# luosiallen/Diff-Foley

Hardware: AMD Instinct MI355X
Metric: UNet denoise steps/sec (8s audio latent, 25-step DDIM, CFG 4.5), aggregate over GPUs (higher is better)
Workload: dtype f16; 1 GPU; BASELINE.json configs[1]: single MI355X, batch=4 (UNet batch 8), 25-step DDIM, fp16 (16-bit MFMA operands at the bf16 rate; the operand type that meets mel MAE < 1e-3 -- the bf16 build is timed in `modes`) UNet, 32 CAVP context frames, latent 4x16x64, guidance 4.5; batch_per_gpu=4, global_batch=4, parallelism=batch-shard x1, no step-loop collectives

## Files before the change

### diff_foley_amd/csrc/attention.hip

```cpp
#include <stdlib.h>
#include "common.h"
#include "kernels.h"

namespace {

template <int KS> struct AttnGeo {
  static constexpr int KT = 32 * KS;
  static constexpr int VROW = KT + 4;
};

template <int D, int NW, int KS = 1>
__global__ __launch_bounds__(NW * 64) void attention_kernel(const bf16_t* __restrict__ Q, int ldq,
                                                            const bf16_t* __restrict__ K, int ldk,
                                                            const bf16_t* __restrict__ Vt, int ldvt, int heads, int Tq,
                                                            int Tk, float scale_log2e, bf16_t* __restrict__ O, int ldo) {
  constexpr int DKC = (D + 15) / 16;
  constexpr int DKP = DKC * 16;
  constexpr int DT = (D + 31) / 32;
  constexpr int KROW = DKP + 8;
  constexpr int KT = AttnGeo<KS>::KT, VROW = AttnGeo<KS>::VROW;
  constexpr bool ONES = (D % 32) != 0;
  constexpr int ONE_T = D / 32, ONE_R = ((D % 32) / 8) * 4 + (D % 4);
  static_assert(!ONES || (D % 8) == 0, "row D sits in half-wave 0");
  __shared__ __attribute__((aligned(16))) bf16_t sK[2 * KT * KROW];
  __shared__ __attribute__((aligned(16))) bf16_t sV[2 * DT * 32 * VROW];

  const int tid = threadIdx.x, lane = tid & 63, wid = tid >> 6;
  const int l31 = lane & 31, lh = lane >> 5;
  const int n = blockIdx.z, h = blockIdx.y;
  const int q0 = (blockIdx.x * NW + wid) * 32;
  const int q = q0 + l31;
  const bool qv = q < Tq;

  bf16x8 qf[DKC];
  {
    const bf16_t* qr = Q + ((long)n * Tq + (qv ? q : 0)) * ldq + h * D;
#pragma unroll
    for (int c = 0; c < DKC; ++c) {
      const int d0 = 16 * c + 8 * lh;
      const bool ok = qv && d0 < D;
      uint4 v = *reinterpret_cast<const uint4*>(qr + (ok ? d0 : 0));
      if (!ok) v = make_uint4(0, 0, 0, 0);
      qf[c] = *reinterpret_cast<bf16x8*>(&v);
    }
  }

  f32x16 o[DT];
#pragma unroll
  for (int t = 0; t < DT; ++t)
#pragma unroll
    for (int r = 0; r < 16; ++r) o[t][r] = 0.f;
  float m_run = -INFINITY, l_run = 0.f;

  const bf16_t* Kb = K + (long)n * Tk * ldk + h * D;
  const bf16_t* Vb = Vt + ((long)n * heads + h) * D * ldvt;
  const int ntiles = (Tk + KT - 1) / KT;

  constexpr int NT = NW * 64;
  constexpr int KCH = (KT * (DKP / 8) + NT - 1) / NT;
  constexpr int VCR = KT / 4;
  constexpr int VCH = (DT * 32 * VCR + NT - 1) / NT;
  uint4 kreg[KCH];
  uint2 vreg[VCH];
  constexpr unsigned OOB = 0x80000000u;
  const __amdgpu_buffer_rsrc_t rsK =
      __builtin_amdgcn_make_buffer_rsrc((void*)Kb, 0, (int)(((long)(Tk - 1) * ldk + D) * 2), 0x00020000);
  const __amdgpu_buffer_rsrc_t rsV =
      __builtin_amdgcn_make_buffer_rsrc((void*)Vb, 0, (int)(((long)(D - 1) * ldvt + ldvt) * 2), 0x00020000);
  unsigned k_off[KCH], v_off[VCH];
#pragma unroll
  for (int i = 0; i < KCH; ++i) {
    const int c = tid + i * NT;
    const int key = c / (DKP / 8), ch = c - key * (DKP / 8);
    const bool ok = (c < KT * (DKP / 8)) && (ch * 8 < D);
    k_off[i] = ok ? (unsigned)((key * ldk + ch * 8) * 2) : OOB;
  }
#pragma unroll
  for (int i = 0; i < VCH; ++i) {
    const int c = tid + i * NT;
    const int d = c / VCR, ch = c - d * VCR;
    const bool ok = (c < DT * 32 * VCR) && (d < D);
    v_off[i] = ok ? (unsigned)((d * ldvt + ch * 4) * 2) : OOB;
  }
  auto gfetch = [&](int k0) {
#pragma unroll
    for (int i = 0; i < KCH; ++i) {
      const u32x4 v = __builtin_amdgcn_raw_buffer_load_b128(rsK, (int)k_off[i], k0 * ldk * 2, 0);
      kreg[i] = make_uint4(v[0], v[1], v[2], v[3]);
    }
#pragma unroll
    for (int i = 0; i < VCH; ++i) {
      typedef __attribute__((ext_vector_type(2))) unsigned int u32x2;
      const u32x2 v = __builtin_amdgcn_raw_buffer_load_b64(rsV, (int)v_off[i], k0 * 2, 0);
      vreg[i] = make_uint2(v[0], v[1]);
    }
    if (k0 + KT > Tk) {
#pragma unroll
      for (int i = 0; i < VCH; ++i) {
        const int ch = (tid + i * NT) % VCR;
        const int nvalid = Tk - (k0 + ch * 4);
        uint2 v = vreg[i];
        if (nvalid < 4) {
          if (nvalid < 3) v.y = 0; else v.y &= 0xFFFFu;
          if (nvalid < 2) v.x &= 0xFFFFu;
          if (nvalid < 1) v.x = 0;
        }
        vreg[i] = v;
      }
    }
  };
  auto sstore = [&](int buf) {
    bf16_t* k_ = sK + buf * (KT * KROW);
    bf16_t* v_ = sV + buf * (DT * 32 * VROW);
#pragma unroll
    for (int i = 0; i < KCH; ++i) {
      const int c = tid + i * NT;
      const int key = c / (DKP / 8), ch = c - key * (DKP / 8);
      if (c < KT * (DKP / 8)) *reinterpret_cast<uint4*>(&k_[key * KROW + ch * 8]) = kreg[i];
    }
#pragma unroll
    for (int i = 0; i < VCH; ++i) {
      const int c = tid + i * NT;
      const int d = c / VCR, ch = c - d * VCR;
      if (c < DT * 32 * VCR && !(ONES && d == D)) *reinterpret_cast<uint2*>(&v_[d * VROW + ch * 4]) = vreg[i];
    }
  };

  gfetch(0);
  DfTouch code_touch = DfTouch();
  if constexpr (D >= 128) code_touch = df_entry_touch(0);
  sstore(0);
  if (ONES) {
#if defined(DF_OPERAND_F16)
    constexpr uint32_t ONE2 = 0x3C003C00u;
#else
    constexpr uint32_t ONE2 = 0x3F803F80u;
#endif
    for (int i = tid; i < 2 * (KT / 2); i += NT) {
      const int b = i / (KT / 2), k2 = i - b * (KT / 2);
      *reinterpret_cast<uint32_t*>(&sV[b * (DT * 32 * VROW) + D * VROW + 2 * k2]) = ONE2;
    }
  }
  __syncthreads();

  for (int kt = 0; kt < ntiles; ++kt) {
    const int k0 = kt * KT;
    const int buf = kt & 1;
    const bf16_t* cK = sK + buf * (KT * KROW);
    const bf16_t* cV = sV + buf * (DT * 32 * VROW);
    if (kt + 1 < ntiles) gfetch(k0 + KT);

    f32x16 s[KS];
#pragma unroll
    for (int u = 0; u < KS; ++u)
#pragma unroll
      for (int r = 0; r < 16; ++r) s[u][r] = 0.f;
#pragma unroll
    for (int c = 0; c < DKC; ++c)
#pragma unroll
      for (int u = 0; u < KS; ++u) {
        const bf16x8 kf = *reinterpret_cast<const bf16x8*>(&cK[(u * 32 + l31) * KROW + 16 * c + 8 * lh]);
        s[u] = DF_MFMA_32x32x16(kf, qf[c], s[u]);
      }
    if (k0 + KT > Tk) {
#pragma unroll
      for (int u = 0; u < KS; ++u)
#pragma unroll
        for (int r = 0; r < 16; ++r) {
          const int key = k0 + u * 32 + (r & 3) + 8 * (r >> 2) + 4 * lh;
          s[u][r] = (key < Tk) ? s[u][r] : -INFINITY;
        }
    }
    float mxu[KS];
#pragma unroll
    for (int u = 0; u < KS; ++u) {
      mxu[u] = -INFINITY;
#pragma unroll
      for (int r = 0; r < 16; ++r) mxu[u] = fmaxf(mxu[u], s[u][r]);
    }
    float mx = mxu[0];
#pragma unroll
    for (int u = 1; u < KS; ++u) mx = fmaxf(mx, mxu[u]);
    mx = half_max(mx) * scale_log2e;
    const float m_new = fmaxf(m_run, mx);
    float psu[KS];
    uint32_t pk[KS][8];
#pragma unroll
    for (int u = 0; u < KS; ++u) {
      psu[u] = 0.f;
#pragma unroll
      for (int r = 0; r < 16; r += 2) {
        const float p0 = __builtin_amdgcn_exp2f(__builtin_fmaf(s[u][r], scale_log2e, -m_new)),
                    p1 = __builtin_amdgcn_exp2f(__builtin_fmaf(s[u][r + 1], scale_log2e, -m_new));
        if (!ONES) psu[u] += p0 + p1;
        pk[u][r >> 1] = pack_bf2_bounded(p0, p1);
      }
    }
    float ps = psu[0];
#pragma unroll
    for (int u = 1; u < KS; ++u) ps += psu[u];
    if (__any(m_new != m_run)) {
      const float alpha = __builtin_amdgcn_exp2f(m_run - m_new);
      if (!ONES) l_run *= alpha;
#pragma unroll
      for (int t = 0; t < DT; ++t)
#pragma unroll
        for (int r = 0; r < 16; ++r) o[t][r] *= alpha;
      m_run = m_new;
    }
    if (!ONES) l_run += ps;
#pragma unroll
    for (int u = 0; u < KS; ++u)
#pragma unroll
      for (int c = 0; c < 2; ++c) {
        uint4 pv = make_uint4(pk[u][4 * c], pk[u][4 * c + 1], pk[u][4 * c + 2], pk[u][4 * c + 3]);
        const bf16x8 pf = *reinterpret_cast<bf16x8*>(&pv);
#pragma unroll
        for (int t = 0; t < DT; ++t) {
          const bf16_t* vr = &cV[(t * 32 + l31) * VROW + u * 32 + 16 * c + 4 * lh];
          const uint2 v0 = *reinterpret_cast<const uint2*>(vr);
          const uint2 v1 = *reinterpret_cast<const uint2*>(vr + 8);
          uint4 vv = make_uint4(v0.x, v0.y, v1.x, v1.y);
          const bf16x8 vf = *reinterpret_cast<bf16x8*>(&vv);
          o[t] = DF_MFMA_32x32x16(vf, pf, o[t]);
        }
      }
    if (kt + 1 < ntiles) sstore(buf ^ 1);
    __syncthreads();
  }

  float l_tot;
  if (ONES) {
    const float mine = o[ONE_T][ONE_R];
    const float other = __shfl_xor(mine, 32);
    l_tot = lh == 0 ? mine : other;
  } else {
    l_tot = l_run + __shfl_xor(l_run, 32);
  }
  const float inv = 1.0f / l_tot;
  if (qv) {
    bf16_t* orow = O + ((long)n * Tq + q) * ldo + h * D;
#pragma unroll
    for (int t = 0; t < DT; ++t)
#pragma unroll
      for (int g = 0; g < 4; ++g) {
        const int d0 = 32 * t + 8 * g + 4 * lh;
        if (d0 < D) {
          uint2 w;
          w.x = pack_bf2(o[t][4 * g] * inv, o[t][4 * g + 1] * inv);
          w.y = pack_bf2(o[t][4 * g + 2] * inv, o[t][4 * g + 3] * inv);
          *reinterpret_cast<uint2*>(orow + d0) = w;
        }
      }
  }
  if constexpr (D >= 128) df_entry_touch_end(code_touch);
}

template <int D>
hipError_t launch_d(const uint16_t* Q, int ldq, const uint16_t* K, int ldk, const uint16_t* Vt, int ldvt,
                    uint16_t* O, int ldo, int N, int heads, int Tq, int Tk, float scale, hipStream_t s) {
  const float sl2 = scale * 1.4426950408889634f;
  const int form = attention_form(D, Tq, Tk), nw = form >> 4;
  if (nw < 1) return hipErrorInvalidValue;
  const dim3 grid((Tq + 32 * nw - 1) / (32 * nw), heads, N), block(64 * nw);
#define DF_ATTN(...) hipLaunchKernelGGL((attention_kernel<D, __VA_ARGS__>), grid, block, 0, s, Q, ldq, K, ldk, Vt, ldvt, heads, Tq, Tk, sl2, O, ldo)
  switch (form) {
    case 4 * 16 + 2:
      if constexpr (D <= 80) { DF_ATTN(4, 2); break; }
      return hipErrorInvalidValue;
    case 4 * 16 + 1: DF_ATTN(4); break;
    case 2 * 16 + 1: DF_ATTN(2); break;
    case 1 * 16 + 1: DF_ATTN(1); break;
    default: return hipErrorInvalidValue;
  }
#undef DF_ATTN
  return hipGetLastError();
}

}

bool attention_supported(int D) {
  switch (D) {
    case 16: case 24: case 32: case 40: case 48: case 56: case 64: case 72: case 80: case 96: case 112: case 128: case 160: case 192:
      return true;
    default: return false;
  }
}

int attention_form(int D, int Tq, int Tk) {
  if (!attention_supported(D)) return 0;
  if (Tq >= 128) return 4 * 16 + (D <= 80 && Tk % 64 == 0 ? 2 : 1);
  return (Tq >= 64 ? 2 : 1) * 16 + 1;
}

hipError_t launch_attention(const uint16_t* Q, int ldq, const uint16_t* K, int ldk, const uint16_t* Vt, int ldvt,
                            uint16_t* O, int ldo, int N, int heads, int D, int Tq, int Tk, float scale,
                            hipStream_t s) {
  if (ldvt % 32 != 0 || ldvt < ((Tk + 31) / 32) * 32) return hipErrorInvalidValue;
  switch (D) {
    case 16:  return launch_d<16>(Q, ldq, K, ldk, Vt, ldvt, O, ldo, N, heads, Tq, Tk, scale, s);
    case 24:  return launch_d<24>(Q, ldq, K, ldk, Vt, ldvt, O, ldo, N, heads, Tq, Tk, scale, s);
    case 48:  return launch_d<48>(Q, ldq, K, ldk, Vt, ldvt, O, ldo, N, heads, Tq, Tk, scale, s);
    case 56:  return launch_d<56>(Q, ldq, K, ldk, Vt, ldvt, O, ldo, N, heads, Tq, Tk, scale, s);
    case 72:  return launch_d<72>(Q, ldq, K, ldk, Vt, ldvt, O, ldo, N, heads, Tq, Tk, scale, s);
    case 96:  return launch_d<96>(Q, ldq, K, ldk, Vt, ldvt, O, ldo, N, heads, Tq, Tk, scale, s);
    case 112: return launch_d<112>(Q, ldq, K, ldk, Vt, ldvt, O, ldo, N, heads, Tq, Tk, scale, s);
    case 192: return launch_d<192>(Q, ldq, K, ldk, Vt, ldvt, O, ldo, N, heads, Tq, Tk, scale, s);
    case 32:  return launch_d<32>(Q, ldq, K, ldk, Vt, ldvt, O, ldo, N, heads, Tq, Tk, scale, s);
    case 40:  return launch_d<40>(Q, ldq, K, ldk, Vt, ldvt, O, ldo, N, heads, Tq, Tk, scale, s);
    case 64:  return launch_d<64>(Q, ldq, K, ldk, Vt, ldvt, O, ldo, N, heads, Tq, Tk, scale, s);
    case 80:  return launch_d<80>(Q, ldq, K, ldk, Vt, ldvt, O, ldo, N, heads, Tq, Tk, scale, s);
    case 128: return launch_d<128>(Q, ldq, K, ldk, Vt, ldvt, O, ldo, N, heads, Tq, Tk, scale, s);
    case 160: return launch_d<160>(Q, ldq, K, ldk, Vt, ldvt, O, ldo, N, heads, Tq, Tk, scale, s);
    default:  return hipErrorInvalidValue;
  }
}
```

### diff_foley_amd/csrc/elementwise.hip

```cpp
#include <algorithm>
#include "common.h"
#include "kernels.h"

namespace {

struct GnSlabs {
  int n;
  long stride;
  const float* bias;
  const float* rowbias;
  int ld_rowbias;
  const float* own;
  int c_own;
  const float* res;
  int ldr;
  float* hout;
};
template <int PER>
__global__ void groupnorm_reg_kernel(const float* __restrict__ x, int ld, int HW, int cpg, int R, int sl_n, int nsamp,
                                     const float* __restrict__ sl_own, int sl_c_own, long sl_stride,
                                     bf16_t* __restrict__ out, int ldo, int silu, int C,
                                     const float* __restrict__ gamma, const float* __restrict__ beta, float eps,
                                     bf16_t* __restrict__ raw, GnSlabs sl) {
  df_fp16_hw_clamp();
// ... 851 lines not shown
}
}

static size_t conv3x3_fewout_lds(int C, int Cout) { return (size_t)(FO_TH + 2) * (FO_TW + 2) * (C * 2 + 16) + (size_t)Cout * 9 * C * 2; }

bool conv3x3_fewout_ok(int H, int W, int C, int Cout) {
  return Cout >= 1 && Cout <= 4 && C % 16 == 0 && C >= 16 && conv3x3_fewout_lds(C, Cout) <= 160 * 1024 && W % 4 == 0 && H > 0;
}

hipError_t launch_conv3x3_fewout(const uint16_t* X, const uint16_t* Wt, const float* bias, float* out, int NB, int H, int W, int C,
                                 int Cout, hipStream_t s) {
  if (!conv3x3_fewout_ok(H, W, C, Cout)) return hipErrorInvalidValue;
  const long blocks = (long)NB * ((H + FO_TH - 1) / FO_TH) * ((W + FO_TW - 1) / FO_TW);
  const size_t lds = conv3x3_fewout_lds(C, Cout);
  static size_t attr = 0;
  if (lds > attr) {
    hipError_t e = hipFuncSetAttribute(reinterpret_cast<const void*>(&conv3x3_fewout_kernel), hipFuncAttributeMaxDynamicSharedMemorySize, (int)lds);
    if (e != hipSuccess) return e;
    attr = lds;
  }
  hipLaunchKernelGGL(conv3x3_fewout_kernel, dim3((unsigned)blocks), dim3(256), lds, s, X, Wt, bias, out, NB, H, W, C, Cout);
  return hipGetLastError();
}

hipError_t launch_pack_conv_weight(const float* w, uint16_t* out, int O, int I, int KH, int KW, int Ipad,
                                   hipStream_t s) {
  const long n = (long)O * KH * KW * Ipad;
  hipLaunchKernelGGL(pack_conv_weight_kernel, dim3(grid_for(n)), dim3(256), 0, s, w, out, O, I, KH, KW, Ipad);
  return hipGetLastError();
}

namespace {
__global__ __launch_bounds__(256) void pack_ffproj_kernel(const float* __restrict__ Wp ,
                                                          const float* __restrict__ W2 , bf16_t* __restrict__ out ,
                                                          int C, int F) {
  __shared__ float sa[32][33], sb[32][33];
  const int tx = threadIdx.x & 31, ty = threadIdx.x >> 5;
  const int i0 = blockIdx.y * 32, j0 = blockIdx.x * 32;
  if (j0 >= F) {
#pragma unroll
    for (int r = 0; r < 4; ++r) out[(long)(i0 + ty + 8 * r) * (F + C) + j0 + tx] = f2bf(Wp[(long)(i0 + ty + 8 * r) * C + (j0 - F) + tx]);
    return;
  }
  float acc[4] = {0.f, 0.f, 0.f, 0.f};
  for (int k0 = 0; k0 < C; k0 += 32) {
#pragma unroll
    for (int r = 0; r < 4; ++r) {
      sa[ty + 8 * r][tx] = Wp[(long)(i0 + ty + 8 * r) * C + k0 + tx];
      sb[ty + 8 * r][tx] = W2[(long)(k0 + ty + 8 * r) * F + j0 + tx];
    }
    __syncthreads();
#pragma unroll
    for (int kk = 0; kk < 32; ++kk) {
      const float b = sb[kk][tx];
#pragma unroll
      for (int r = 0; r < 4; ++r) acc[r] += sa[ty + 8 * r][kk] * b;
    }
    __syncthreads();
  }
#pragma unroll
  for (int r = 0; r < 4; ++r) out[(long)(i0 + ty + 8 * r) * (F + C) + j0 + tx] = f2bf(acc[r]);
}
__global__ __launch_bounds__(256) void ffproj_bias_kernel(const float* __restrict__ Wp, const float* __restrict__ b2,
                                                          const float* __restrict__ bp, float* __restrict__ out, int C) {
  const int i = blockIdx.x * 4 + (threadIdx.x >> 6), lane = threadIdx.x & 63;
  if (i >= C) return;
  float a = 0.f;
  for (int k = lane; k < C; k += 64) a += Wp[(long)i * C + k] * b2[k];
#pragma unroll
  for (int o = 32; o > 0; o >>= 1) a += __shfl_xor(a, o);
  if (lane == 0) out[i] = a + bp[i];
}
}

hipError_t launch_pack_ffproj(const float* Wp, const float* bp, const float* W2, const float* b2, uint16_t* wout, float* bout,
                              int C, int F, hipStream_t s) {
  if (C % 32 != 0 || F % 32 != 0) return hipErrorInvalidValue;
  hipLaunchKernelGGL(pack_ffproj_kernel, dim3((F + C) / 32, C / 32), dim3(256), 0, s, Wp, W2, wout, C, F);
  hipLaunchKernelGGL(ffproj_bias_kernel, dim3((C + 3) / 4), dim3(256), 0, s, Wp, b2, bp, bout, C);
  return hipGetLastError();
}

namespace {
__global__ __launch_bounds__(256) void xattn_expand_kernel(const bf16_t* __restrict__ kv, bf16_t* __restrict__ Kexp,
                                                           bf16_t* __restrict__ Vexp, int Tc, int Tcp, int C, int H, long total8) {
  const int D = C / H, c8n = C / 8;
  for (long e = (long)blockIdx.x * 256 + threadIdx.x; e < total8; e += (long)gridDim.x * 256) {
    const int j8 = (int)(e % c8n);
    const long row = e / c8n;
    const int tp = (int)(row % Tcp), h = (int)((row / Tcp) % H);
    const long n = row / ((long)Tcp * H);
    uint4 k4 = make_uint4(0, 0, 0, 0), v4 = make_uint4(0, 0, 0, 0);
    if (tp < Tc) {
      const bf16_t* src = kv + ((n * Tc + tp) * 2l * C) + j8 * 8;
      k4 = *reinterpret_cast<const uint4*>(src);
      v4 = *reinterpret_cast<const uint4*>(src + C);
      const int hj = (j8 * 8) / D;
      if (hj != h) { k4 = make_uint4(0, 0, 0, 0); v4 = k4; }
    }
    *reinterpret_cast<uint4*>(Kexp + row * C + j8 * 8) = k4;
    *reinterpret_cast<uint4*>(Vexp + row * C + j8 * 8) = v4;
  }
}
__global__ __launch_bounds__(256) void pack_lnq_t_kernel(const float* __restrict__ Wq, const float* __restrict__ gamma,
                                                         bf16_t* __restrict__ out, int C, float scale) {
  __shared__ float t[32][33];
  const int tx = threadIdx.x & 31, ty = threadIdx.x >> 5;
  const int j0 = blockIdx.x * 32, c0 = blockIdx.y * 32;
#pragma unroll
  for (int r = 0; r < 4; ++r) t[ty + 8 * r][tx] = Wq[(long)(j0 + ty + 8 * r) * C + c0 + tx];
  __syncthreads();
#pragma unroll
  for (int r = 0; r < 4; ++r) {
    const int c = c0 + ty + 8 * r;
    out[(long)c * C + j0 + tx] = f2bf(scale * gamma[c] * t[tx][ty + 8 * r]);
  }
}
__global__ __launch_bounds__(256) void xattn_rowstats_kernel(const bf16_t* __restrict__ G, const bf16_t* __restrict__ Kexp,
                                                             const float* __restrict__ bq, float scale, int C, long rows,
                                                             float* __restrict__ cs, float* __restrict__ bb) {
  const long row = (long)blockIdx.x * 4 + (threadIdx.x >> 6);
  const int lane = threadIdx.x & 63;
  if (row >= rows) return;
  float a = 0.f, b = 0.f;
  for (int c = lane; c < C; c += 64) {
    a += bf2f(G[row * C + c]);
    b += bf2f(Kexp[row * C + c]) * bq[c];
  }
#pragma unroll
  for (int o = 32; o > 0; o >>= 1) { a += __shfl_xor(a, o); b += __shfl_xor(b, o); }
  if (lane == 0) { cs[row] = a; bb[row] = scale * b; }
}
}

hipError_t launch_xattn_expand(const uint16_t* kv, uint16_t* Kexp, uint16_t* Vexp, int NB, int Tc, int Tcp, int C, int H,
                               hipStream_t s) {
  if (C % H != 0 || (C / H) % 8 != 0 || C % 8 != 0) return hipErrorInvalidValue;
  const long total8 = (long)NB * H * Tcp * (C / 8);
  const int blocks = (int)std::min<long>((total8 + 255) / 256, 8192);
  hipLaunchKernelGGL(xattn_expand_kernel, dim3(blocks), dim3(256), 0, s, kv, Kexp, Vexp, Tc, Tcp, C, H, total8);
  return hipGetLastError();
}
hipError_t launch_pack_lnq_t(const float* Wq, const float* gamma, uint16_t* out, int C, float scale, hipStream_t s) {
  if (C % 32 != 0) return hipErrorInvalidValue;
  hipLaunchKernelGGL(pack_lnq_t_kernel, dim3(C / 32, C / 32), dim3(256), 0, s, Wq, gamma, out, C, scale);
  return hipGetLastError();
}
hipError_t launch_xattn_rowstats(const uint16_t* G, const uint16_t* Kexp, const float* bq, float scale, int C, long rows, float* cs,
                                 float* bb, hipStream_t s) {
  hipLaunchKernelGGL(xattn_rowstats_kernel, dim3((unsigned)((rows + 3) / 4)), dim3(256), 0, s, G, Kexp, bq, scale, C, rows, cs, bb);
  return hipGetLastError();
}

hipError_t launch_pack_conv_skip(const float* w, const float* ws, uint16_t* out, int O, int I, int I2, hipStream_t s) {
  const long n = (long)O * (9 * I + I2);
  hipLaunchKernelGGL(pack_conv_skip_kernel, dim3(grid_for(n)), dim3(256), 0, s, w, ws, out, O, I, I2);
  return hipGetLastError();
}

hipError_t launch_pack_geglu(const float* w, const float* b, uint16_t* wout, float* bout, int half_rows, int K,
                             hipStream_t s) {
  if (half_rows % 32 != 0) return hipErrorInvalidValue;
  const long n = (long)2 * half_rows * K;
  hipLaunchKernelGGL(pack_geglu_kernel, dim3(grid_for(n)), dim3(256), 0, s, w, b, wout, bout, half_rows, K);
  return hipGetLastError();
}
// ... 54 lines not shown
```

### diff_foley_amd/csrc/engine_builder.hip

```cpp
#include "engine_internal.h"

DFE_NAMESPACE {

static void choose_tile(int M, int N, int K, int batch, bool geglu, int* tile, int* splitk) {
  static const double eff[] = {1.0, 0.85, 0.85, 0.62, 0.55};
  constexpr int TILE_COUNT = sizeof(eff) / sizeof(eff[0]);
  static_assert(TILE_COUNT == TILE_32x128 + 1, "one efficiency per tile 128x128 .. 32x128");
  double best = 1e30;
  *tile = TILE_64x64;
  *splitk = 1;
  const int nk = K / 64;
  for (int c = 0; c < TILE_COUNT; ++c) {
    int bm, bn;
    gemm_tile_dims(c, &bm, &bn);
    if (bm > 64 && M <= bm / 2) continue;
    const long tiles = (long)cdiv(M, bm) * cdiv(N, bn) * batch;
    for (int sk = 1; sk <= 16; sk *= 2) {
      if (sk > 1 && (batch > 1 || nk / sk < 4)) break;
      const double work = (double)(bm / 32) * (bn / 32) * (double)cdiv(nk, sk) * 4.0 * 8.0 / eff[c] + 2500.0;
      const double rounds = (double)((tiles * sk + 255) / 256);
      double cost = rounds * work;
      if (sk > 1) cost += 9000.0 + (double)M * N * 8.0 * sk / 2000.0;
      if (cost < best) {
        best = cost;
// ... 185 lines not shown
  bf16_t* xraw = nullptr;
  bf16_t* a1 = groupnorm(x, NB, n1, eps, 1, has_skip ? &xraw : nullptr);
  float* h1 = buf<float>((size_t)M * cout);
  {
    GemmParams g = gp_conv3(a1, NB, H, Wd, cin, c->w_conv3(nm(c1 + ".weight"), cin), cout, 1, 0);
    out_f32(g, h1, cout);
    g.bias = c->f32(nm(c1 + ".bias"));
    if (emb) {
      g.rowbias = emb + emb_col; g.ld_rowbias = emb_ld; g.rows_per_sample = H * Wd; g.rowbias_mode = 1;
    }
    gemm(g, 1, "res.conv1");
  }
  pl->release(a1);
  const size_t ci = pl->ops.size() - 1;
  pl->ops[ci].defer = groupnorm_accepts_slabs(H * Wd, cout);
  bf16_t* a2 = buf<bf16_t>((size_t)M * cout);
  {
    Plan* plp = pl;
    const float* gm = c->f32(nm(n2 + ".weight"));
    const float* bt = c->f32(nm(n2 + ".bias"));
    const float* cb = c->f32(nm(c1 + ".bias"));
    const float* rb = emb ? emb + emb_col : nullptr;
    const int HW = H * Wd;
    const size_t sb = groupnorm_scratch_bytes(NB, HW, cout);
    float* scr = sb ? (float*)pl->alloc(sb) : nullptr;
    other("groupnorm", [=](hipStream_t s, const RunArgs&) {
      const Op& co = plp->ops[ci];
      if (co.defer && co.gp.splitk > 1)
        return launch_groupnorm_slabs(co.gp.partial, cout, NB, HW, cout, gm, bt, eps, 1, a2, cout, nullptr, co.gp.splitk,
                                      (long)M * cout, cb, rb, emb_ld, s);
      if (scr) return launch_groupnorm_chunked(h1, cout, NB, HW, cout, gm, bt, eps, 1, a2, cout, nullptr, scr, s);
      return launch_groupnorm(h1, cout, NB, HW, cout, gm, bt, eps, 1, a2, cout, nullptr, s);
    });
    emits(a2, M, cout, cout);
    pl->release(scr);
  }
  pl->release(h1);
  {
    GemmParams g = gp_conv3(a2, NB, H, Wd, cout, c->w_conv3(nm(c2 + ".weight"), cout), cout, 1, 0);
    out_f32(g, out.p, out.ld);
    g.bias = c->f32(nm(c2 + ".bias"));
    if (has_skip) {
      const bf16_t* w;
      const float* bsum;
      c->w_conv3_skip(nm(c2), nm(skip), &w, &bsum);
      g.W = w;
      g.bias = bsum;
      g.A2 = xraw; g.lda2 = cin; g.Cin2 = cin; g.a2_bytes = op_bytes((size_t)M * cin * 2);
      g.K = 9 * cout + cin;
      g.w_bytes = op_bytes((size_t)cout * g.K * 2);
    } else { g.res = x.p; g.ldr = x.ld; }
    attach_aux(g, M, cout);
    g.dup_rows = dup_rows;
    gemm(g, 1, "res.conv2");
  }
  if (has_skip) pl->release(xraw);
  pl->release(a2);
}

void Builder::spatial_transformer(const F32& x, const F32& out, int NB, int T, const std::string& p, int heads,
                                  const bf16_t* ctxK, const bf16_t* ctxVt, int Tc, int ldvtc, const PX* px,
                                  bool cfg_prefix) {
  const int C = x.C, M = x.rows, D = C / heads;
  if (cfg_prefix && (T % 4 != 0 || NB % 2 != 0)) fail("cfg prefix needs the fused QKV form");
  const int Mp = cfg_prefix ? M / 2 : M, NBp = cfg_prefix ? NB / 2 : NB;
  if (!attention_supported(D)) fail("unsupported attention head dim %d", D);
  const std::string tb = p + ".transformer_blocks.0";
  const float scale = 1.0f / sqrtf((float)D);
  bf16_t* a = groupnorm(F32{x.p, Mp, C, x.ld}, NBp, p + ".norm", 1e-6f, 0, nullptr);
  float* t0 = buf<float>((size_t)M * C);
  F32 t0v{t0, M, C, C};
  bf16_t* xb = buf<bf16_t>((size_t)M * C);
  const int slots = C / 64;
  float2* st = buf<float2>((size_t)M * slots);
  auto produces_t0 = [&](GemmParams& g) {
    out_f32(g, t0, C);
    g.aux = xb; g.ld_aux = C;
    g.stats = st; g.stats_slots = slots;
  };
  auto ln_fold = [&](GemmParams& g, const float* cs, const float* bb) {
    g.ln_stats = st; g.ln_slots = slots; g.ln_C = C; g.ln_eps = 1e-5f; g.ln_cs = cs;
    g.bias = bb;
  };
  {
    GemmParams g = gp_linear(a, Mp, C, c->w_linear(nm(p + ".proj_in.weight")), C);
    produces_t0(g);
    g.bias = c->f32(nm(p + ".proj_in.bias"));
    gemm(g, 1, "st.proj_in");
  }
  bf16_t* qk = buf<bf16_t>((size_t)M * 2 * C);
  const int ldvt = rup(T, 32);
  bf16_t* vt = buf<bf16_t>((size_t)NB * C * ldvt);
  const bool fuse_v = (T % 4 == 0);
  bf16_t* o_own = nullptr;
  if (!fuse_v) {
    layernorm(t0v, tb + ".norm1", a);
    {
      const bf16_t* w = c->w_stack(nm(tb + ".attn1.qk"), {nm(tb + ".attn1.to_q.weight"), nm(tb + ".attn1.to_k.weight")});
      GemmParams g = gp_linear(a, M, C, w, 2 * C);
      out_b16(g, qk, 2 * C);
      gemm(g, 1, "st.qk");
    }
    {
      GemmParams g = gp_linear(c->w_linear(nm(tb + ".attn1.to_v.weight")), C, C, a, T);
      g.w_bs = (long)T * C;
      out_b16(g, vt, ldvt);
      g.c_bs = (long)C * ldvt;
      gemm(g, NB, "st.vT");
    }
    o_own = buf<bf16_t>((size_t)M * C);
  } else {
    const bf16_t* w;
    const float *cs, *bb;
    c->w_ln_stack(nm(tb + ".attn1.qkv"), nm(tb + ".norm1"),
                  {nm(tb + ".attn1.to_q.weight"), nm(tb + ".attn1.to_k.weight"), nm(tb + ".attn1.to_v.weight")}, {}, false,
                  &w, &cs, &bb);
    GemmParams g = gp_linear(xb, Mp, C, w, 3 * C);
    out_b16(g, qk, 2 * C);
    ln_fold(g, cs, bb);
    g.vt = vt; g.vt_col0 = 2 * C; g.vt_T = T; g.ldvt = ldvt;
    gemm(g, 1, "st.qkv");
  }
  bf16_t* o = o_own ? o_own : a;
  other("attn.self", [=](hipStream_t s, const RunArgs&) {
    return launch_attention(qk, 2 * C, qk + C, 2 * C, vt, ldvt, o, C, NBp, heads, D, T, T, scale, s);
  });
  emits(o, Mp, C, C);
  {
    GemmParams g = gp_linear(o, Mp, C, c->w_linear(nm(tb + ".attn1.to_out.0.weight")), C);
    produces_t0(g);
    g.bias = c->f32(nm(tb + ".attn1.to_out.0.bias"));
    g.res = t0; g.ldr = C;
    g.dup_rows = cfg_prefix ? Mp : 0;
    gemm(g, 1, "st.attn1.out");
  }
  if (px && px->G) {
    const int HT = px->HT;
    bf16_t* pr = qk;
    if ((size_t)HT > (size_t)2 * C) fail("cross-attention: %d probability columns do not fit the q|k buffer", HT);
    {
      GemmParams g = gp_linear(xb, M, C, px->G, HT);
      g.w_bs = (long)HT * C; g.w_rows = T;
      g.w_bytes = op_bytes((size_t)HT * C * 2);
      out_b16(g, pr, HT);
      ln_fold(g, px->cs, px->bb);
      g.sm_w = 32; g.sm_valid = Tc;
      gemm(g, 1, "st.xs");
    }
    {
      GemmParams g = gp_linear(pr, M, HT, px->Vo, C);
      g.w_bs = (long)C * HT; g.w_rows = T;
      g.w_bytes = op_bytes((size_t)C * HT * 2);
      produces_t0(g);
      g.no_c_store = 1;
      g.bias = c->f32(nm(tb + ".attn2.to_out.0.bias"));
      g.res = t0; g.ldr = C;
      gemm(g, 1, "st.xo");
    }
  } else {
  bf16_t* q2 = qk;
  {
    const bf16_t* w;
    const float *cs, *bb;
    c->w_ln_stack(nm(tb + ".attn2.q"), nm(tb + ".norm2"), {nm(tb + ".attn2.to_q.weight")}, {}, false, &w, &cs, &bb);
    GemmParams g = gp_linear(xb, M, C, w, C);
    out_b16(g, q2, C);
    ln_fold(g, cs, bb);
    gemm(g, 1, "st.q2");
  }
  other("attn.cross", [=](hipStream_t s, const RunArgs&) {
    return launch_attention(q2, C, ctxK, C, ctxVt, ldvtc, o, C, NB, heads, D, T, Tc, scale, s);
  });
  emits(o, M, C, C);
  {
    GemmParams g = gp_linear(o, M, C, c->w_linear(nm(tb + ".attn2.to_out.0.weight")), C);
    produces_t0(g);
    g.bias = c->f32(nm(tb + ".attn2.to_out.0.bias"));
    g.res = t0; g.ldr = C;
    gemm(g, 1, "st.attn2.out");
  }
  }
  pl->release(qk);
  pl->release(vt);
  bf16_t* gl = buf<bf16_t>((size_t)M * 4 * C);
  {
    const bf16_t* w;
    const float *cs, *bb;
    c->w_ln_stack(nm(tb + ".ff.net.0.proj"), nm(tb + ".norm3"), {nm(tb + ".ff.net.0.proj.weight")},
                  {nm(tb + ".ff.net.0.proj.bias")}, true, &w, &cs, &bb);
    GemmParams g = gp_linear(xb, M, C, w, 8 * C);
    out_b16(g, gl, 4 * C);
    ln_fold(g, cs, bb);
    g.geglu = 1;
    if ((8 * C) % 320 == 0) {
      const bf16_t* w3;
      const float *cs3, *bb3;
      c->w_ln_w320(nm(tb + ".ff.net.0.proj"), 8 * C, C, &w3, &cs3, &bb3);
      g.W_w320 = w3; g.cs_w320 = cs3; g.bias_w320 = bb3;
    }
    gemm(g, 1, "st.ff1");
  }
  {
    const bf16_t* w;
    const float* bsum;
    c->w_ffproj(nm(tb + ".ff.net.2"), nm(p + ".proj_out"), &w, &bsum);
    GemmParams g = gp_linear(gl, M, 4 * C, w, C);
    g.K = 5 * C;
// ... 112 lines not shown
```

### diff_foley_amd/csrc/engine_internal.h

```cpp
#pragma once
#include <hip/hip_runtime.h>

#include <algorithm>
#include <array>
#include <cmath>
#include <cstdarg>
#include <cstdio>
#include <cstdlib>
#include <cstring>
#include <functional>
#include <map>
#include <mutex>
#include <memory>
#include <stdexcept>
#include <string>
#include <vector>

#include "../../include/df_engine.h"
#include "gemm.h"
#include "kernels.h"

typedef uint16_t bf16_t;

#define DFE_NAMESPACE namespace dfe __attribute__((visibility("hidden")))
// ... 150 lines not shown
  uint64_t tick = 0;
  dfe::Plan* last_unet = nullptr;
  bool last_unet_hoisted = false;
  int ctx_N = 0, ctx_T = 0;
  float* ctx_copy = nullptr;
  size_t ctx_copy_bytes = 0;
  bool autotune = false;
  bool reloaded = false;
  bool prof_on = false;
  std::vector<hipEvent_t> prof_ev;
  std::vector<int> prof_fam;
  std::vector<const void*> prof_op;
  size_t prof_used = 0;
  hipStream_t pack_stream = nullptr;
  bool chk_on = false;
  std::vector<std::string> rq_prefix;
  unsigned long long* chk_dev = nullptr;
  size_t chk_used = 0, chk_cap = 0;
  std::vector<std::string> chk_label;
  bool sat_on = false;
  unsigned long long* sat_dev = nullptr;
  size_t sat_used = 0, sat_cap = 0;
  std::vector<std::string> sat_label;

  ~df_ctx() {
    plans.clear();
    for (auto& kv : raw) (void)hipFree(kv.second.d);
    for (void* p : packed_blocks) (void)hipFree(p);
    for (hipEvent_t e : prof_ev) (void)hipEventDestroy(e);
    if (chk_dev) (void)hipFree(chk_dev);
    if (sat_dev) (void)hipFree(sat_dev);
    if (ctx_copy) (void)hipFree(ctx_copy);
  }

  const dfe::RawT& rt(const std::string& name) const {
    auto it = raw.find(name);
    if (it == raw.end()) dfe::fail("missing tensor '%s'", name.c_str());
    return it->second;
  }
  bool has(const std::string& name) const { return raw.count(name) != 0; }
  const float* f32(const std::string& name) const {
    const dfe::RawT& t = rt(name);
    if (!t.d) dfe::fail("tensor '%s' was imported shape-only (df_import_packed): its fp32 data is not on this rank", name.c_str());
    return t.d;
  }

  std::map<const void*, size_t> block_bytes;
  void* pmalloc(size_t bytes) {
    void* p = nullptr;
    HIPCHK(hipMalloc(&p, (bytes + 255) & ~(size_t)255));
    packed_blocks.push_back(p);
    block_bytes[p] = bytes;
    return p;
  }
  template <size_t N, class Make>
  std::array<void*, N> pack_once(const std::array<std::string, N>& keys, Make&& make) {
    if (!packed.count(keys[0])) {
      const std::array<void*, N> made = make();
      for (size_t i = 0; i < N; ++i) packed[keys[i]] = made[i];
    }
    std::array<void*, N> blk;
    for (size_t i = 0; i < N; ++i) blk[i] = packed[keys[i]];
    return blk;
  }
  template <class Make>
  void* pack_once(const std::string& key, Make&& make) {
    return pack_once<1>({key}, [&]() -> std::array<void*, 1> { return {make()}; })[0];
  }
  const bf16_t* w_linear(const std::string& name);
  const bf16_t* w_stack(const std::string& key, const std::vector<std::string>& names);
  const float* b_stack(const std::string& key, const std::vector<std::string>& names);
  const bf16_t* w_conv3(const std::string& name, int ipad);
  const bf16_t* w_conv3_ups4(const std::string& name, int ipad);
  void w_conv3_skip(const std::string& conv, const std::string& skip, const bf16_t** w, const float** b);
  void w_ffproj(const std::string& ff2, const std::string& po, const bf16_t** w, const float** b);
  const bf16_t* w_lnq_t(const std::string& wq, const std::string& norm, float scale);
  const bf16_t* w_stack_t(const std::string& key, const std::vector<std::string>& names);
  const bf16_t* w_conv3_bwd(const std::string& name);
  void w_conv3d_bn(const std::string& p, int kp, const bf16_t** w, const float** b);
  void w_ln_stack(const std::string& key, const std::string& norm, const std::vector<std::string>& names,
                  const std::vector<std::string>& biases, bool geglu, const bf16_t** w, const float** cs, const float** bb);
  void w_ln_w320(const std::string& key, int rows, int K, const bf16_t** w, const float** cs, const float** bb);
  void w_geglu(const std::string& prefix, const bf16_t** w, const float** b);
};

DFE_NAMESPACE {

struct BlockDesc {
  enum Kind { CONV_IN, RES, ST, DOWN, UP } kind;
  std::string prefix;
  int cin, cout;
  int ds = 1;
};
struct UNetTopo {
  std::vector<std::vector<BlockDesc>> input, output;
  std::vector<BlockDesc> middle;
  std::vector<int> in_ch;
  std::vector<int> in_ds;
  std::vector<int> out_ds;
  int final_ch = 0;
};

UNetTopo make_topo(const df_unet_config& u, bool encoder_only);
std::vector<std::string> topo_resblocks(const UNetTopo& t);
std::vector<BlockDesc> topo_sts(const UNetTopo& t);

struct Builder {
  df_ctx* c;
  Plan* pl;
  std::string pre;
  int which = 0;

  std::string nm(const std::string& s) const { return pre + s; }

  struct PX {
    const bf16_t* G = nullptr;
    const float* cs = nullptr;
    const float* bb = nullptr;
    const bf16_t* Vo = nullptr;
    int HT = 0;
  };

  bool want_aux = false;
  bf16_t* last_aux = nullptr;
  void attach_aux(GemmParams& g, int rows, int C);

  template <class T>
  T* buf(size_t n) {
    return (T*)pl->alloc(n * sizeof(T));
  }

  struct Pend { long op = -1; const float* p = nullptr; int ld = 0, C = 0, rows = 0; };
  Pend pend;

  void forget_pend();
  void other(const char* tag, std::function<hipError_t(hipStream_t, const RunArgs&)> fn);
  void emits(const bf16_t* p, long rows, int cols, int ld);
  Op& gemm(GemmParams gp, int batch, const char* tag);

  static unsigned op_bytes(size_t b);
  static GemmParams gp_linear(const bf16_t* A, int M, int K, const bf16_t* W, int N);
  static GemmParams gp_conv3(const bf16_t* A, int NB, int H, int Wd, int Cin, const bf16_t* W, int Cout, int stride,
                             int ups);
  static GemmParams gp_conv3_ups4(const bf16_t* A, int NB, int H, int Wd, int Cin, const bf16_t* W4, int Cout);
  static void out_f32(GemmParams& g, float* C, int ldc) { g.C = C; g.ldc = ldc; g.out_bf16 = 0; }
  static void out_b16(GemmParams& g, bf16_t* C, int ldc) { g.C = C; g.ldc = ldc; g.out_bf16 = 1; }

  bf16_t* groupnorm(const F32& x, int NB, const std::string& p, float eps, int silu, bf16_t** raw);
  void layernorm(const F32& x, const std::string& p, bf16_t* o);
  bf16_t* cast2d(const F32& x);

  void resblock(const F32& x, const F32& out, int NB, int H, int Wd, const std::string& n1, const std::string& c1,
                const std::string& n2, const std::string& c2, const std::string& skip, float eps,
                const float* emb, int emb_ld, int emb_col, int dup_rows = 0);

  void spatial_transformer(const F32& x, const F32& out, int NB, int T, const std::string& p, int heads,
                           const bf16_t* ctxK, const bf16_t* ctxVt, int Tc, int ldvtc, const PX* px = nullptr,
                           bool cfg_prefix = false);

  static bool px_ok(int C, int heads, int Tc, int tokens);
  PX context_px(const bf16_t* ctx, int NB, int Tc, int Dc, const std::string& st_prefix, int C, int heads);
  void context_kv(const bf16_t* ctx, int NB, int Tc, int Dc, const std::string& st_prefix, int C, bf16_t** K,
                  bf16_t** Vt, int ldvt);

  typedef std::map<std::string, std::pair<bf16_t*, bf16_t*>> KV;
  bf16_t* context_cast(int N, int Tc, int Dc);
// ... 40 lines not shown
```

### diff_foley_amd/csrc/engine_pack.hip

```cpp
#include "engine_internal.h"

using namespace dfe;

const bf16_t* df_ctx::w_linear(const std::string& name) {
  return (const bf16_t*)pack_once(name, [&] {
    const RawT& t = rt(name);
    (void)f32(name);
    bf16_t* o = (bf16_t*)pmalloc(t.n * 2);
    HIPCHK(launch_cast_bf16(t.d, o, (long)t.n, pack_stream));
    return o;
  });
}
const bf16_t* df_ctx::w_stack(const std::string& key, const std::vector<std::string>& names) {
  return (const bf16_t*)pack_once(key, [&] {
    size_t tot = 0;
    for (auto& n : names) tot += rt(n).n;
    bf16_t* o = (bf16_t*)pmalloc(tot * 2);
    size_t off = 0;
    for (auto& n : names) {
      const RawT& t = rt(n);
      HIPCHK(launch_cast_bf16(t.d, o + off, (long)t.n, pack_stream));
      off += t.n;
    }
    return o;
// ... 89 lines not shown
    return o;
  });
}
const bf16_t* df_ctx::w_conv3_bwd(const std::string& name) {
  return (const bf16_t*)pack_once(name + "#c3bwd", [&] {
    const RawT& t = rt(name);
    const int O = (int)t.shape[0], I = (int)t.shape[1], Opad = (O + 63) / 64 * 64;
    bf16_t* o = (bf16_t*)pmalloc((size_t)I * 9 * Opad * 2);
    HIPCHK(launch_pack_conv_bwd(t.d, o, O, I, Opad, pack_stream));
    return o;
  });
}
void df_ctx::w_conv3d_bn(const std::string& p, int kp, const bf16_t** w, const float** b) {
  const std::string kw = "c3d:" + p + ":" + std::to_string(kp);
  const auto blk = pack_once<2>({kw, kw + ":b"}, [&]() -> std::array<void*, 2> {
    const RawT& t = rt(p + ".conv.weight");
    if (t.shape.size() != 5) fail("%s.conv.weight: expected a 5-D Conv3d weight", p.c_str());
    const int O = (int)t.shape[0], I = (int)t.shape[1], KT = (int)t.shape[2], KH = (int)t.shape[3], KW = (int)t.shape[4];
    bf16_t* wo = (bf16_t*)pmalloc((size_t)O * kp * 2);
    float* bo = (float*)pmalloc((size_t)O * 4);
    HIPCHK(launch_pack_conv3d_bn(t.d, f32(p + ".bn.weight"), f32(p + ".bn.bias"), f32(p + ".bn.running_mean"),
                                 f32(p + ".bn.running_var"), 1e-5f, wo, bo, O, I, KT, KH, KW, kp, pack_stream));
    return {wo, bo};
  });
  *w = (const bf16_t*)blk[0];
  *b = (const float*)blk[1];
}

void df_ctx::w_ln_stack(const std::string& key, const std::string& norm, const std::vector<std::string>& names,
                        const std::vector<std::string>& biases, bool geglu, const bf16_t** w, const float** cs, const float** bb) {
  const auto blk = pack_once<3>({key + "#lnw", key + "#lncs", key + "#lnbb"}, [&]() -> std::array<void*, 3> {
    int rows = 0;
    const int K = (int)rt(names[0]).shape[1];
    for (auto& n : names) rows += (int)rt(n).shape[0];
    bf16_t* wo = (bf16_t*)pmalloc((size_t)rows * K * 2);
    float* co = (float*)pmalloc((size_t)rows * 4);
    float* bo = (float*)pmalloc((size_t)rows * 4);
    const float* g = f32(norm + ".weight");
    const float* be = f32(norm + ".bias");
    int off = 0;
    for (size_t i = 0; i < names.size(); ++i) {
      const RawT& t = rt(names[i]);
      if ((int)t.shape[1] != K) fail("w_ln_stack %s: input dims differ", key.c_str());
      const float* bias = (i < biases.size() && !biases[i].empty()) ? f32(biases[i]) : nullptr;
      const int r = (int)t.shape[0];
      HIPCHK(launch_pack_ln_linear(t.d, bias, g, be, wo, co, bo, r, K, off, geglu ? r / 2 : 0, pack_stream));
      off += r;
    }
    return {wo, co, bo};
  });
  *w = (const bf16_t*)blk[0];
  *cs = (const float*)blk[1];
  *bb = (const float*)blk[2];
}

void df_ctx::w_ln_w320(const std::string& key, int rows, int K, const bf16_t** w, const float** cs, const float** bb) {
  const std::string kw = key + "#lnw", kc = key + "#lncs", kb = key + "#lnbb";
  const auto blk = pack_once<3>({key + "#lnw320", key + "#lncs320", key + "#lnbb320"}, [&]() -> std::array<void*, 3> {
    if (!packed.count(kw) || !packed.count(kc) || !packed.count(kb)) fail("w_ln_w320 %s: the (32 | 32) packing does not exist", key.c_str());
    bf16_t* wo = (bf16_t*)pmalloc((size_t)rows * K * 2);
    float* co = (float*)pmalloc((size_t)rows * 4);
    float* bo = (float*)pmalloc((size_t)rows * 4);
    HIPCHK(launch_pack_w320((const bf16_t*)packed[kw], (const float*)packed[kc], (const float*)packed[kb], wo, co, bo, rows, K, pack_stream));
    return {wo, co, bo};
  });
  *w = (const bf16_t*)blk[0];
  *cs = (const float*)blk[1];
  *bb = (const float*)blk[2];
}

void df_ctx::w_geglu(const std::string& prefix, const bf16_t** w, const float** b) {
  const auto blk = pack_once<2>({prefix + ".weight#geglu", prefix + ".bias#geglu"}, [&]() -> std::array<void*, 2> {
    const RawT& tw = rt(prefix + ".weight");
    const RawT& tb = rt(prefix + ".bias");
    const int rows = (int)tw.shape[0], K = (int)tw.shape[1];
    bf16_t* wo = (bf16_t*)pmalloc((size_t)rows * K * 2);
    float* bo = (float*)pmalloc((size_t)rows * 4);
    HIPCHK(launch_pack_geglu(tw.d, tb.d, wo, bo, rows / 2, K, pack_stream));
    return {wo, bo};
  });
  *w = (const bf16_t*)blk[0];
  *b = (const float*)blk[1];
}
```

### diff_foley_amd/csrc/engine_run.hip

```cpp
#include "engine_internal.h"

DFE_NAMESPACE {

void finish_plan(df_ctx* c, Plan* pl) {
  if (pl->partial_bytes) {
    HIPCHK(hipMalloc((void**)&pl->partial, pl->partial_bytes));
    for (auto& o : pl->ops)
      if (o.is_gemm && o.gp.splitk > 1) o.gp.partial = pl->partial;
  }
  HIPCHK(hipStreamSynchronize(c->pack_stream));
}

namespace {

int op_family(const Op& o) {
  if (o.is_gemm) return 0;
  if (!strncmp(o.tag, "attn", 4)) return 1;
  if (!strcmp(o.tag, "groupnorm")) return 2;
  if (!strcmp(o.tag, "layernorm")) return 3;
  return 4;
}

struct ChkBuf { const uint32_t* p; unsigned long long words; };
__global__ __launch_bounds__(256) void checksum_kernel(const ChkBuf* list, unsigned long long* slot) {
  const ChkBuf b = list[blockIdx.y];
  unsigned long long acc = 0;
  for (unsigned long long i = (unsigned long long)blockIdx.x * 256 + threadIdx.x; i < b.words; i += (unsigned long long)gridDim.x * 256)
    acc += (unsigned long long)b.p[i] * (unsigned long long)((i & 1023u) + 1u);
#pragma unroll
  for (int o = 32; o > 0; o >>= 1) acc += __shfl_xor(acc, o);
  if ((threadIdx.x & 63) == 0) atomicAdd(slot, acc);
}

void checksum_after_op(df_ctx* c, Plan* pl, size_t op_index, hipStream_t s) {
  if (!pl->chk_list) {
    std::vector<ChkBuf> v;
    for (auto& b : pl->owned) v.push_back({(const uint32_t*)b.p, (unsigned long long)(b.bytes / 4)});
    if (pl->partial) v.push_back({(const uint32_t*)pl->partial, (unsigned long long)(pl->partial_bytes / 4)});
    pl->chk_n = (int)v.size();
    if (!v.empty()) {
      HIPCHK(hipMalloc(&pl->chk_list, v.size() * sizeof(ChkBuf)));
      HIPCHK(hipMemcpy(pl->chk_list, v.data(), v.size() * sizeof(ChkBuf), hipMemcpyHostToDevice));
    }
  }
  if (c->chk_used >= c->chk_cap || pl->chk_n == 0) return;
  hipLaunchKernelGGL(checksum_kernel, dim3(64, pl->chk_n), dim3(256), 0, s, (const ChkBuf*)pl->chk_list, c->chk_dev + c->chk_used);
  char lab[160];
  snprintf(lab, sizeof lab, "%s#%zu:%s", pl->name.c_str(), op_index, pl->ops[op_index].tag);
  if (pl->ops[op_index].is_gemm) {
    const Op& o = pl->ops[op_index];
    const size_t n = strlen(lab);
    snprintf(lab + n, sizeof lab - n, " %dx%dx%d taps%d tile%d sk%d", o.gp.M, o.gp.N, o.gp.K, o.gp.taps, o.tile, o.gp.splitk);
  }
  c->chk_label.push_back(lab);
  ++c->chk_used;
}

std::vector<OutBuf> operand_outputs(const Op& o) {
  std::vector<OutBuf> outs = o.outs;
  if (o.is_gemm) {
    const GemmParams& g = o.gp;
    const long rows = (long)g.M * (g.taps == 4 ? 4 : 1) + g.dup_rows;
    const int cols = g.geglu ? g.N / 2 : (g.vt ? g.vt_col0 : g.N);
    if (g.out_bf16 && g.C && !o.c_ext && !g.store_nchw)
      for (int z = 0; z < (g.splitk > 1 ? 1 : o.batch); ++z) outs.push_back({(const uint16_t*)g.C + (long)z * g.c_bs, rows, cols, g.ldc});
    if (g.aux) outs.push_back({g.aux, rows, g.N, g.ld_aux});
    if (g.vt) outs.push_back({g.vt, (long)(g.M / g.vt_T) * (g.N - g.vt_col0), g.vt_T, g.ldvt});
  }
  return outs;
}

__global__ __launch_bounds__(256) void sat_count_kernel(const uint16_t* p, long rows, int cols, int ld, unsigned long long* slot) {
  const long total = rows * (long)cols;
  unsigned long long acc = 0;
  for (long e = (long)blockIdx.x * 256 + threadIdx.x; e < total; e += (long)gridDim.x * 256) {
    const long r = e / cols;
    const uint16_t v = p[r * ld + (e - r * cols)];
#if defined(DF_OPERAND_F16)
    acc += (v & 0x7FFFu) == 0x7BFFu;
#else
    acc += (v & 0x7F80u) == 0x7F80u;
#endif
  }
#pragma unroll
  for (int o = 32; o > 0; o >>= 1) acc += __shfl_xor(acc, o);
  if ((threadIdx.x & 63) == 0 && acc) atomicAdd(slot, acc);
}

void saturations_after_op(df_ctx* c, Plan* pl, size_t op_index, hipStream_t s) {
  if (c->sat_used >= c->sat_cap) return;
  const Op& o = pl->ops[op_index];
  const std::vector<OutBuf> outs = operand_outputs(o);
  for (auto& b : outs) {
    const long total = b.rows * (long)b.cols;
    if (total <= 0) continue;
    const int blocks = (int)std::min<long>((total + 255) / 256, 1024);
    hipLaunchKernelGGL(sat_count_kernel, dim3(blocks), dim3(256), 0, s, b.p, b.rows, b.cols, b.ld, c->sat_dev + c->sat_used);
  }
  char lab[160];
  snprintf(lab, sizeof lab, "%s#%zu:%s", pl->name.c_str(), op_index, o.tag);
  c->sat_label.push_back(lab);
  ++c->sat_used;
}

__global__ __launch_bounds__(256) void requant_bf16_kernel(uint16_t* p, long rows, int cols, int ld) {
#if defined(DF_OPERAND_F16)
  const long total = rows * (long)cols;
  for (long e = (long)blockIdx.x * 256 + threadIdx.x; e < total; e += (long)gridDim.x * 256) {
    const long r = e / cols;
    uint16_t* q = p + r * ld + (e - r * cols);
    const uint16_t v = *q;
    if ((v & 0x7C00u) == 0x7C00u) continue;
    const uint16_t lsb = (v >> 3) & 1u;
    *q = (uint16_t)((v + 3u + lsb) & 0xFFF8u);
  }
#endif
}

void requant_after_op(df_ctx* c, Plan* pl, size_t op_index, hipStream_t s) {
  const Op& o = pl->ops[op_index];
  bool hit = false;
  for (auto& pre : c->rq_prefix)
    if (pre == "*" || !strncmp(o.tag, pre.c_str(), pre.size())) hit = true;
  if (!hit) return;
  const std::vector<OutBuf> outs = operand_outputs(o);
  for (auto& b : outs) {
    const long total = b.rows * (long)b.cols;
    if (total <= 0) continue;
    const int blocks = (int)std::min<long>((total + 255) / 256, 2048);
    hipLaunchKernelGGL(requant_bf16_kernel, dim3(blocks), dim3(256), 0, s, const_cast<uint16_t*>(b.p), b.rows, b.cols, b.ld);
  }
}

}

void run_ops(df_ctx* c, Plan* pl, size_t begin, size_t end, hipStream_t s, const RunArgs& a) {
  for (size_t i = begin; i < end; ++i) {
    Op& o = pl->ops[i];
    hipError_t e;
    (void)hipGetLastError();
    if (c->prof_on) {
      if (c->prof_used + 2 > c->prof_ev.size()) {
        hipEvent_t e0, e1;
        HIPCHK(hipEventCreate(&e0));
        HIPCHK(hipEventCreate(&e1));
        c->prof_ev.push_back(e0);
// ... 85 lines not shown
```

### diff_foley_amd/csrc/engine_test_api.hip

```cpp
#include "engine_internal.h"

using namespace dfe;

extern "C" {

static float* test_partial(size_t bytes) {
  static float* buf = nullptr;
  static size_t cap = 0;
  if (bytes > cap) {
    if (buf) {
      (void)hipDeviceSynchronize();
      (void)hipFree(buf);
    }
    HIPCHK(hipMalloc((void**)&buf, bytes));
    cap = bytes;
  }
  return buf;
}

int df_test_gemm(const uint16_t* A, const uint16_t* W, float* C, int M, int N, int K, int tile, int splitk, void* stream) {
  return guard([&] {
    GemmParams g = Builder::gp_linear(A, M, K, W, N);
    Builder::out_f32(g, C, N);
    g.dbg = getenv("DF_GEMM_DBG") ? atoi(getenv("DF_GEMM_DBG")) : 0;
    g.splitk = splitk;
    if (splitk > 1) g.partial = test_partial((size_t)splitk * M * N * 4);
    else if (g.dbg & 64) g.partial = test_partial((size_t)4096 * 32 * 8);
    HIPCHK(launch_gemm(g, tile, 1, (hipStream_t)stream));
  });
}

int df_test_gemm_epi(const uint16_t* A, const uint16_t* W, const float* bias, const float* res, void* C, int M, int N, int K,
                     int act, int out_operand, int tile, int splitk, void* stream) {
  return guard([&] {
    GemmParams g = Builder::gp_linear(A, M, K, W, N);
    if (out_operand) Builder::out_b16(g, (bf16_t*)C, N);
    else Builder::out_f32(g, (float*)C, N);
    g.bias = bias;
    if (res) { g.res = res; g.ldr = N; }
    g.silu = act == 1;
    g.relu = act == 2;
    g.splitk = splitk;
    if (splitk > 1) g.partial = test_partial((size_t)splitk * M * N * 4);
    if (!gemm_tile_valid(g, tile, 1, splitk)) fail("tile %d / split-K %d refused this problem", tile, splitk);
    HIPCHK(launch_gemm(g, tile, 1, (hipStream_t)stream));
  });
}

int df_test_gemm_dual(const uint16_t* A, const uint16_t* A2, const uint16_t* W, float* C, int M, int N, int K1, int K2, int tile,
                      int splitk, void* stream) {
  return guard([&] {
    GemmParams g = Builder::gp_linear(A, M, K1, W, N);
    g.K = K1 + K2;
    g.w_bytes = Builder::op_bytes((size_t)N * (K1 + K2) * 2);
    g.A2 = A2; g.lda2 = K2; g.Cin2 = K2; g.a2_bytes = Builder::op_bytes((size_t)M * K2 * 2);
    Builder::out_f32(g, C, N);
    g.splitk = splitk;
    if (splitk > 1) g.partial = test_partial((size_t)splitk * M * N * 4);
    if (!gemm_tile_valid(g, tile, 1, splitk)) fail("tile %d / split-K %d refused this problem", tile, splitk);
    HIPCHK(launch_gemm(g, tile, 1, (hipStream_t)stream));
  });
}

static void test_gemm_params(const df_test_gemm_desc* d, GemmParams& g) {
  if (!d) fail("df_test_gemm: null descriptor");
  if (d->size != (int64_t)sizeof(df_test_gemm_desc))
    fail("df_test_gemm: descriptor of %lld bytes, this build expects %zu (stale binding of df_test_gemm_desc?)", (long long)d->size,
         sizeof(df_test_gemm_desc));
  const bf16_t* A = (const bf16_t*)d->A;
  const bf16_t* W = (const bf16_t*)d->W;
  if (d->conv == 2) {
    if (d->ups || d->zstuff || d->stride > 1) fail("df_test_gemm: conv 2 takes neither ups / zstuff nor a stride");
    g = Builder::gp_conv3_ups4(A, d->NB, d->H, d->Wd, d->Cin, W, d->N);
  } else if (d->conv) {
    if (d->conv != 1) fail("df_test_gemm: conv %d", d->conv);
    if (d->stride != 1 && d->stride != 2) fail("df_test_gemm: conv stride %d", d->stride);
    if (d->zstuff && !d->ups) fail("df_test_gemm: zstuff without ups");
    if (d->ups && d->stride != 1) fail("df_test_gemm: ups with stride %d", d->stride);
    g = Builder::gp_conv3(A, d->NB, d->H, d->Wd, d->Cin, W, d->N, d->stride, d->ups ? 1 : 0);
    g.zstuff = d->zstuff ? 1 : 0;
  } else {
    if (d->ups || d->zstuff) fail("df_test_gemm: ups / zstuff on a linear GEMM");
    g = Builder::gp_linear(A, d->M, d->K, W, d->N);
    if (d->lda > 0) {
      g.lda = d->lda;
      g.a_bytes = Builder::op_bytes((size_t)d->M * d->lda * 2);
    }
  }
  if (d->Cin2 > 0 || d->A2) {
    if (d->Cin2 <= 0 || d->lda2 < d->Cin2) fail("df_test_gemm: A2 with Cin2 %d / lda2 %d", d->Cin2, d->lda2);
    g.A2 = (const bf16_t*)d->A2; g.lda2 = d->lda2; g.Cin2 = d->Cin2;
    g.a2_bytes = Builder::op_bytes(((size_t)(g.M - 1) * d->lda2 + d->Cin2) * 2);
    g.K += d->Cin2;
    g.w_bytes = Builder::op_bytes((size_t)g.N * g.K * 2);
  }
  g.geglu = d->geglu ? 1 : 0;
  g.vt = (bf16_t*)d->vt; g.vt_col0 = d->vt_col0; g.vt_T = d->vt_T; g.ldvt = d->ldvt;
  g.C = d->C; g.ldc = d->ldc > 0 ? d->ldc : (g.geglu ? g.N / 2 : g.N); g.out_bf16 = d->out_operand ? 1 : 0;
  g.a_bs = d->a_bs; g.c_bs = d->c_bs; g.res_bs = d->res_bs;
  if (d->conv != 2) g.w_bs = d->w_bs;
  g.alpha = d->alpha;
  g.bias = d->bias;
  g.rowbias = d->rowbias; g.ld_rowbias = d->ld_rowbias; g.rows_per_sample = d->rows_per_sample; g.rowbias_mode = d->rowbias_mode;
  g.res = d->res; g.ldr = d->ldr;
  g.relu = d->relu; g.silu = d->silu;
  g.aux = (bf16_t*)d->aux; g.ld_aux = d->ld_aux;
  g.stats = (float2*)d->stats; g.stats_slots = d->stats_slots;
  g.ln_stats = (const float2*)d->ln_stats; g.ln_slots = d->ln_slots; g.ln_C = d->ln_C; g.ln_eps = d->ln_eps; g.ln_cs = d->ln_cs;
  g.w_rows = d->w_rows; g.sm_w = d->sm_w; g.sm_valid = d->sm_valid;
  g.dup_rows = d->dup_rows; g.no_c_store = d->no_c_store; g.store_nchw = d->store_nchw; g.hw_out = d->hw_out;
  g.cfg_out = d->cfg_out; g.cfg_scale = d->cfg_scale;
  g.defer_reduce = d->defer_reduce;
  g.gm = d->gm;
  g.splitk = d->splitk > 1 ? d->splitk : 1;
  if (g.geglu && g.N % 320 == 0) { g.W_w320 = W; g.cs_w320 = g.ln_cs; g.bias_w320 = g.bias; }
}

int df_test_gemm_valid(const df_test_gemm_desc* d, int tile, int batch, int splitk) {
  std::lock_guard<std::recursive_mutex> hold(g_api_lock);
  try {
    GemmParams g;
    test_gemm_params(d, g);
    return gemm_tile_valid(g, tile, batch, splitk) ? 1 : 0;
  } catch (const std::exception& e) {
    g_err = e.what();
    return -1;
  }
}

int df_test_gemm_key(const df_test_gemm_desc* d, int batch, char* buf, int n) {
  std::lock_guard<std::recursive_mutex> hold(g_api_lock);
  try {
    GemmParams g;
    test_gemm_params(d, g);
    const std::string key = tune_key(g, batch > 1 ? batch : 1, d->defer_reduce != 0);
    if (!buf || n <= (int)key.size()) fail("df_test_gemm_key: buffer of %d bytes for a key of %zu", n, key.size());
    memcpy(buf, key.c_str(), key.size() + 1);
    return 0;
  } catch (const std::exception& e) {
    g_err = e.what();
    return -1;
  }
}

int df_test_gemm_tile_info(int tile, df_test_gemm_tile* out) {
  std::lock_guard<std::recursive_mutex> hold(g_api_lock);
  if (tile < 0 || tile >= TILE_ALL || !out || out->size != (int64_t)sizeof(df_test_gemm_tile)) {
    g_err = "df_test_gemm_tile_info: no tile " + std::to_string(tile) + ", or a df_test_gemm_tile of another size";
    return 1;
  }
  const GemmTileInfo& t = kGemmTiles[tile];
  out->name = t.name; out->family = t.family; out->modes = t.modes;
  out->bm = t.bm; out->bn = t.bn; out->dma_threads = gemm_halo_dma_threads(tile); out->ring = t.ring;
  return 0;
}

int df_test_gemm_ex(const df_test_gemm_desc* d, void* stream) {
  return guard([&] {
    GemmParams g;
    test_gemm_params(d, g);
    const int batch = d->batch > 1 ? d->batch : 1;
    if (g.K % 64 != 0) fail("df_test_gemm: K %d is not a multiple of 64", g.K);
    if (d->defer_reduce && g.splitk < 2) fail("df_test_gemm: defer_reduce needs split-K");
    const size_t slab_bytes = (size_t)g.splitk * g.M * g.N * 4 * (g.taps == 4 ? 4 : 1);
    if (g.splitk > 1) g.partial = test_partial(slab_bytes);
    if (gemm_tile_is_wgeglu(d->tile) && g.geglu) {
      if (g.N % 320 != 0 || !g.ln_cs || !g.bias) fail("tile %d: N = %d is not a multiple of 320, or no column sums / bias", d->tile, g.N);
      static void* buf = nullptr;
      static size_t cap = 0;
      const size_t wb = ((size_t)g.N * g.K * 2 + 255) & ~(size_t)255, need = wb + (size_t)g.N * 8 + 512;
      if (need > cap) {
        if (buf) {
          HIPCHK(hipDeviceSynchronize());
          HIPCHK(hipFree(buf));
          buf = nullptr; cap = 0;
        }
        HIPCHK(hipMalloc(&buf, need));
        cap = need;
      }
      uint16_t* w3 = (uint16_t*)buf;
// ... 233 lines not shown
    HIPCHK(launch_gemm(g, tile, 1, (hipStream_t)stream));
  });
}

int df_test_conv3x3_fewout(const uint16_t* A, const uint16_t* W, const float* bias, float* out_nchw, int NB, int H, int Wd, int Cin,
                           int Cout, void* stream) {
  return guard([&] { HIPCHK(launch_conv3x3_fewout(A, W, bias, out_nchw, NB, H, Wd, Cin, Cout, (hipStream_t)stream)); });
}

int df_test_conv3x3_skip(const uint16_t* A, const uint16_t* A2, const uint16_t* W, const float* bias, float* C, int NB, int H,
                         int Wd, int Cin, int Cin2, int Cout, int tile, int splitk, void* stream) {
  return guard([&] {
    GemmParams g = Builder::gp_conv3(A, NB, H, Wd, Cin, W, Cout, 1, 0);
    Builder::out_f32(g, C, Cout);
    g.bias = bias;
    g.A2 = A2; g.lda2 = Cin2; g.Cin2 = Cin2; g.a2_bytes = Builder::op_bytes((size_t)g.M * Cin2 * 2);
    g.K = 9 * Cin + Cin2;
    g.w_bytes = Builder::op_bytes((size_t)Cout * g.K * 2);
    g.splitk = splitk;
    if (splitk > 1) g.partial = test_partial((size_t)splitk * g.M * g.N * 4);
    if (!gemm_tile_valid(g, tile, 1, splitk)) fail("tile %d / split-K %d refused this problem", tile, splitk);
    HIPCHK(launch_gemm(g, tile, 1, (hipStream_t)stream));
  });
}

int df_test_conv3x3_ups4(const uint16_t* A, const float* W_oihw, const float* bias, float* C, uint16_t* w4_scratch, int NB, int H,
                         int Wd, int Cin, int Cout, int tile, int splitk, void* stream) {
  return guard([&] {
    HIPCHK(launch_pack_conv_ups4(W_oihw, w4_scratch, Cout, Cin, Cin, (hipStream_t)stream));
    GemmParams g = Builder::gp_conv3_ups4(A, NB, H, Wd, Cin, w4_scratch, Cout);
    Builder::out_f32(g, C, Cout);
    g.bias = bias;
    g.splitk = splitk;
    if (splitk > 1) g.partial = test_partial((size_t)splitk * 4 * g.M * g.N * 4);
    if (!gemm_tile_valid(g, tile, 1, splitk)) fail("tile %d / split-K %d refused this problem", tile, splitk);
    HIPCHK(launch_gemm(g, tile, 1, (hipStream_t)stream));
  });
}

int df_test_groupnorm_form(int N, int HW, int C, int nslab) { return groupnorm_form(N, HW, C, nslab); }
int df_test_attention_form(int D, int Tq, int Tk) { return attention_form(D, Tq, Tk); }

int df_test_groupnorm_ex(float* x, int ld, int N, int HW, int C, const float* gamma, const float* beta, float eps, int silu,
                         uint16_t* out, int ldo, uint16_t* raw_out, int nslab, int64_t slab_stride, const float* bias,
                         const float* rowbias, int ld_rowbias, const float* own_slabs, int c_own, const float* res, int ldr,
                         void* stream) {
  return guard([&] {
    hipStream_t s = (hipStream_t)stream;
    const int form = groupnorm_form(N, HW, C, nslab);
    if (form == GN_FORM_REFUSED) fail("groupnorm: %d x %d with %d slabs is refused", HW, C, nslab);
    if (own_slabs) {
      HIPCHK(launch_groupnorm_own_slabs(x, ld, N, HW, C, gamma, beta, eps, silu, out, ldo, raw_out, own_slabs, nslab, (long)slab_stride,
                                        c_own, bias, res, ldr, s));
    } else if (form == GN_FORM_CHUNKED) {
      float* scr = test_partial(groupnorm_scratch_bytes(N, HW, C));
      HIPCHK(launch_groupnorm_chunked(x, ld, N, HW, C, gamma, beta, eps, silu, out, ldo, raw_out, scr, s));
    } else {
      HIPCHK(launch_groupnorm_slabs(x, ld, N, HW, C, gamma, beta, eps, silu, out, ldo, raw_out, nslab, (long)slab_stride, bias, rowbias,
                                    ld_rowbias, s));
    }
  });
}
int df_test_groupnorm(const float* x, int ld, int N, int HW, int C, const float* gamma, const float* beta, float eps,
                      int silu, uint16_t* out, void* stream) {
  return df_test_groupnorm_ex(const_cast<float*>(x), ld, N, HW, C, gamma, beta, eps, silu, out, C, nullptr, 0, 0, nullptr, nullptr, 0,
                              nullptr, 0, nullptr, 0, stream);
}
int df_test_groupnorm_own_slabs(float* x, int ld, int N, int HW, int C, const float* gamma, const float* beta, float eps, int silu,
                                uint16_t* out, const float* slabs, int nslab, int c_own, const float* bias, const float* res,
                                int ldr, void* stream) {
  return df_test_groupnorm_ex(x, ld, N, HW, C, gamma, beta, eps, silu, out, C, nullptr, nslab, (int64_t)N * HW * c_own, bias, nullptr, 0,
                              slabs, c_own, res, ldr, stream);
}
int df_test_layernorm_ex(const float* x, int ld, int rows, int C, const float* gamma, const float* beta, uint16_t* out, void* stream) {
  return guard([&] { HIPCHK(launch_layernorm(x, ld, rows, C, gamma, beta, 1e-5f, out, (hipStream_t)stream)); });
}
int df_test_layernorm(const float* x, int rows, int C, const float* gamma, const float* beta, uint16_t* out, void* stream) {
  return df_test_layernorm_ex(x, C, rows, C, gamma, beta, out, stream);
}
int df_test_attention(const uint16_t* Q, int ldq, const uint16_t* K, int ldk, const uint16_t* Vt, int ldvt, uint16_t* O,
                      int ldo, int N, int heads, int D, int Tq, int Tk, float scale, void* stream) {
  return guard([&] { HIPCHK(launch_attention(Q, ldq, K, ldk, Vt, ldvt, O, ldo, N, heads, D, Tq, Tk, scale, (hipStream_t)stream)); });
}

int df_test_groupnorm_bwd(const float* x, int ld, int N, int HW, int C, const float* gamma, const float* beta, float eps, int silu,
                          const float* dy, int lddy, const float* addend, int ldadd, float* dx, int lddx, uint16_t* dx_b16,
                          void* stream) {
  return guard([&] {
    HIPCHK(launch_groupnorm_bwd(x, ld, N, HW, C, gamma, beta, eps, silu, dy, lddy, addend, ldadd, dx, lddx, dx_b16,
                                (hipStream_t)stream));
  });
}
int df_test_layernorm_bwd(const float* x, int rows, int C, const float* gamma, float eps, const float* dy, const float* addend,
                          float* dx, uint16_t* dx_b16, void* stream) {
  return guard([&] { HIPCHK(launch_layernorm_bwd(x, rows, C, gamma, eps, dy, addend, dx, dx_b16, (hipStream_t)stream)); });
}
int df_test_geglu_fwd(const uint16_t* u, uint16_t* y, int64_t rows, int H, void* stream) {
  return guard([&] { HIPCHK(launch_geglu_fwd(u, y, (long)rows, H, (hipStream_t)stream)); });
}
int df_test_geglu_bwd(const uint16_t* u, const float* dy, uint16_t* du, int64_t rows, int H, void* stream) {
  return guard([&] { HIPCHK(launch_geglu_bwd(u, dy, du, (long)rows, H, (hipStream_t)stream)); });
}
int df_test_attention_bwd(const uint16_t* Q, int ldq, const uint16_t* K, int ldk, const uint16_t* Vt, int ldvt, const float* dO,
                          int lddo, uint16_t* dQ, int lddq, uint16_t* dK, int lddk, uint16_t* dV, int lddv, int N, int heads, int D,
                          int Tq, int Tk, float scale, int form, void* stream) {
  return guard([&] {
    size_t nws = attention_bwd_ws_floats(N, heads, D, Tq, Tk, lddk, lddv, dK != nullptr);
    if (form == 2 && dK) nws = (size_t)N * heads * Tq * 3;
    float* ws = nws ? test_partial(nws * 4) : nullptr;
    HIPCHK(launch_attention_bwd(Q, ldq, K, ldk, Vt, ldvt, dO, lddo, dQ, lddq, dK, lddk, dV, lddv, N, heads, D, Tq, Tk, scale, ws,
                                form, (hipStream_t)stream));
  });
}
int df_test_cls_head_bwd(const float* prob, const float* w, float* dh, uint16_t* dh_b16, int N, int HW, int C, int Cp, void* stream) {
  return guard([&] { HIPCHK(launch_cls_head_bwd(prob, w, dh, dh_b16, N, HW, C, Cp, (hipStream_t)stream)); });
}
int df_test_pack_linear_t(const float* w, uint16_t* out, int O, int I, int ldo, int off, void* stream) {
  return guard([&] { HIPCHK(launch_pack_linear_t(w, out, O, I, ldo, off, (hipStream_t)stream)); });
}
int df_test_pack_conv_bwd(const float* w, uint16_t* out, int O, int I, int Opad, void* stream) {
  return guard([&] { HIPCHK(launch_pack_conv_bwd(w, out, O, I, Opad, (hipStream_t)stream)); });
}
int df_test_conv3x3_bwd_data(const uint16_t* dY, const float* W_oihw, uint16_t* w_scratch, float* dX, uint16_t* dX_op, int NB, int H,
                             int Wd, int I, int O, int stride, int tile, int splitk, void* stream) {
  return guard([&] {
    if (stride != 1 && stride != 2) fail("conv3x3 backward-data: stride %d", stride);
    if (stride == 2 && ((H | Wd) & 1)) fail("conv3x3 backward-data: stride 2 needs an even map, got %dx%d", H, Wd);
    const int Opad = (O + 63) / 64 * 64;
    HIPCHK(launch_pack_conv_bwd(W_oihw, w_scratch, O, I, Opad, (hipStream_t)stream));
    GemmParams g = stride == 1 ? Builder::gp_conv3(dY, NB, H, Wd, Opad, w_scratch, I, 1, 0)
                               : Builder::gp_conv3(dY, NB, H / 2, Wd / 2, Opad, w_scratch, I, 1, 1);
    if (stride == 2) g.zstuff = 1;
    Builder::out_f32(g, dX, I);
    if (dX_op) {
      g.aux = dX_op;
      g.ld_aux = I;
    }
    g.splitk = splitk;
    if (splitk > 1) g.partial = test_partial((size_t)splitk * g.M * g.N * 4);
    if (!gemm_tile_valid(g, tile, 1, splitk)) fail("tile %d / split-K %d refused this problem", tile, splitk);
    HIPCHK(launch_gemm(g, tile, 1, (hipStream_t)stream));
  });
}


#define DF_TEST_LAUNCH(call) return guard([&] { HIPCHK(call); })
int df_test_softmax_rows(const float* s, uint16_t* p, int rows, int T, int ldp, void* stream) {
  DF_TEST_LAUNCH(launch_softmax_rows(s, p, rows, T, ldp, (hipStream_t)stream));
}
int df_test_timestep_embedding(const float* t, float* out, int N, int dim, void* stream) {
  DF_TEST_LAUNCH(launch_timestep_embedding(t, out, N, dim, (hipStream_t)stream));
}
int df_test_timestep_embedding_b16(const float* t, int t_B, uint16_t* out, int N, int dim, void* stream) {
  DF_TEST_LAUNCH(launch_timestep_embedding_b16(t, t_B, out, N, dim, (hipStream_t)stream));
}
int df_test_pack_latent(const float* x, uint16_t* out, int B, int C, int HW, int cpad, int rep, float in_scale, const float* wpq,
                        const float* bpq, void* stream) {
  DF_TEST_LAUNCH(launch_pack_latent(x, out, B, C, HW, cpad, rep, in_scale, wpq, bpq, (hipStream_t)stream));
}
int df_test_pack_latent_bcast(const float* x, uint16_t* out, int B, int C, int HW, int cpad, int rep, const float* src, float* dst,
                              int rows, int n, void* stream) {
  DF_TEST_LAUNCH(launch_pack_latent_bcast(x, out, B, C, HW, cpad, rep, src, dst, rows, n, (hipStream_t)stream));
}
int df_test_bcast_rows(const float* src, float* dst, int rows, int n, void* stream) {
  DF_TEST_LAUNCH(launch_bcast_rows(src, dst, rows, n, (hipStream_t)stream));
}
// ... 51 lines not shown
```

### diff_foley_amd/csrc/engine_tune.hip

```cpp
#include "engine_internal.h"

DFE_NAMESPACE {

namespace {
struct TuneCand { int tile, sk; float iso_ms; double situ_ms; };

}

std::string tune_key(const GemmParams& g, int batch, bool defer) {
  char key[160];
  const int epi = (g.silu ? 128 : 0) | (g.ln_stats ? 1 : 0) | (g.stats ? 2 : 0) | (g.vt ? 4 : 0) | (g.aux ? 8 : 0) | (g.res ? 16 : 0) | (g.Cin2 ? 32 : 0) |
                  (defer ? 64 : 0) | (g.dup_rows ? 256 : 0);
  snprintf(key, sizeof key, "%d_%d_%d_%d_%d_%d_%d_%d_e%d", g.M, g.N, g.K, g.taps, g.stride, g.ups, batch, g.geglu, epi);
  return key;
}
static std::string tune_key(const Op& o) { return tune_key(o.gp, o.batch, o.defer); }

std::map<std::string, TuneChoice>& tune_cache() {
  static std::map<std::string, TuneChoice> m;
  static bool loaded = false;
  if (!loaded) {
    loaded = true;
    if (const char* path = getenv("DF_TUNE_CACHE")) {
      if (FILE* f = fopen(path, "r")) {
        char key[160];
        TuneChoice ch;
        while (fscanf(f, "%159s %d %d %d", key, &ch.tile, &ch.sk, &ch.gm) == 4) m[key] = ch;
        fclose(f);
      }
    }
  }
  return m;
}
static void tune_cache_save() {
  const char* path = getenv("DF_TUNE_CACHE");
  if (!path) return;
  FILE* f = fopen(path, "w");
  if (!f) return;
  for (auto& kv : tune_cache()) fprintf(f, "%s %d %d %d\n", kv.first.c_str(), kv.second.tile, kv.second.sk, kv.second.gm);
  fclose(f);
}

bool g_tune_imported = false;

static const TuneChoice* nearest_tune_choice(const std::string& key) {
  const size_t us = key.find('_');
  if (us == std::string::npos) return nullptr;
  const std::string suffix = key.substr(us);
  const double m = (double)atol(key.substr(0, us).c_str());
  if (m <= 0) return nullptr;
  const TuneChoice* best = nullptr;
  double bestd = 2.0001;
  for (auto& kv : tune_cache()) {
    const size_t u2 = kv.first.find('_');
    if (u2 == std::string::npos || kv.first.compare(u2, std::string::npos, suffix) != 0) continue;
    const double m2 = (double)atol(kv.first.substr(0, u2).c_str());
    if (m2 <= 0) continue;
    const double d = fabs(log2(m2 / m));
    if (d < bestd) {
      bestd = d;
      best = &kv.second;
    }
  }
  return best;
}

void apply_tune_cache(Plan* pl) {
  auto& tc = tune_cache();
  for (auto& o : pl->ops) {
    if (!o.is_gemm || o.c_ext) continue;
    const std::string key = tune_key(o);
    auto it = tc.find(key);
    const TuneChoice* chp = it != tc.end() ? &it->second : nearest_tune_choice(key);
    if (!chp) continue;
    const TuneChoice& ch = *chp;
    const size_t need = (size_t)ch.sk * o.gp.M * o.gp.N * 4 * (o.gp.taps == 4 ? 4 : 1);
    if (!gemm_tile_valid(o.gp, ch.tile, o.batch, ch.sk) || (ch.sk > 1 && need > pl->partial_bytes)) continue;
    o.tile = ch.tile;
    o.gp.splitk = ch.sk;
    o.gp.gm = ch.gm;
    o.gp.partial = pl->partial;
  }
}

void autotune_plan(df_ctx* c, Plan* pl, hipStream_t s) {
  {
    auto& tc = tune_cache();
    bool all = !tc.empty();
    for (auto& o : pl->ops)
      if (o.is_gemm && !o.c_ext && !tc.count(tune_key(o))) all = false;
    if (all) {
      apply_tune_cache(pl);
      tune_cache_save();
      return;
    }
// ... 161 lines not shown
```

### diff_foley_amd/csrc/gemm.h

```cpp
#pragma once
#include <hip/hip_runtime.h>
#include <stdint.h>
#include "common.h"

struct GemmParams {
  const uint16_t* A; long a_bs; int lda;
  const uint16_t* W; long w_bs;
  unsigned a_bytes, w_bytes;
  int M, N, K;
  const uint16_t* A2; int lda2; unsigned a2_bytes; int Cin2;
  int taps;
  int Cin;
  int H, Wd;
  int OH, OW;
  int stride;
  int ups;
  int zstuff;
  int th, tw;
  int halo_ring_bytes;
  void* C; long c_bs; int ldc; int out_bf16;
  float alpha;
  const float* bias;
  const float* rowbias; int ld_rowbias; int rows_per_sample; int rowbias_mode;
  const float* res; long res_bs; int ldr;
  int relu;
  int silu;
  uint16_t* aux; int ld_aux;
  int geglu;
  const float2* ln_stats; int ln_slots; int ln_C; float ln_eps;
  const float* ln_cs;
  const uint16_t* W_w320; const float* cs_w320; const float* bias_w320;
  int w_rows;
  int sm_w, sm_valid;
  float2* stats; int stats_slots;
  uint16_t* vt; int vt_col0; int vt_T; int ldvt;
  int dup_rows;
  int no_c_store;
  int store_nchw; int hw_out;
  int gm;
  int dbg;
  int splitk; float* partial;
  int defer_reduce;
  float* cfg_out; float cfg_scale;
};

#if defined(__HIP_DEVICE_COMPILE__)
__device__ __forceinline__ DfTouch gemm_kernarg_touch() { return df_entry_touch((int)sizeof(GemmParams)); }
__device__ __forceinline__ void gemm_kernarg_touch_end(const DfTouch& v) { df_entry_touch_end(v); }
#endif

enum GemmTileFamily { DF_FAM_GEN = 0, DF_FAM_HALO = 1, DF_FAM_PS = 2, DF_FAM_PGEGLU = 3, DF_FAM_WGEGLU = 4, DF_FAM_RETIRED = 5 };
enum GemmTile {
#define DF_TILE(ID, NAME, ...) NAME,
#include "gemm_tiles.def"
#undef DF_TILE
  TILE_ALL
};
struct GemmTileInfo {
  const char* name;
  int family, part;
  int modes;
  int bm, bn, wgm, wgn, ring, ps, lns;
};
inline constexpr GemmTileInfo kGemmTiles[TILE_ALL] = {
#define DF_TILE(ID, NAME, DISP, FAM, PART, M0, M1, M2, M3, BM, BN, WGM, WGN, RING, PS, LNS) \
  {DISP, DF_FAM_##FAM, PART, (M0) | (M1) << 1 | (M2) << 2 | (M3) << 3, BM, BN, WGM, WGN, RING, PS, LNS},
#include "gemm_tiles.def"
#undef DF_TILE
};
#define DF_TILE(ID, NAME, ...) static_assert(NAME == ID, "gemm_tiles.def: a tile id is its row's position (the ids are a file format)");
#include "gemm_tiles.def"
#undef DF_TILE

static inline int gemm_tile_family(int cfg) { return (cfg >= 0 && cfg < TILE_ALL) ? kGemmTiles[cfg].family : -1; }
static inline bool gemm_tile_is_halo(int cfg) { return gemm_tile_family(cfg) == DF_FAM_HALO; }
static inline bool gemm_tile_is_ps(int cfg) { return gemm_tile_family(cfg) == DF_FAM_PS; }
static inline bool gemm_tile_is_pgeglu(int cfg) { return gemm_tile_family(cfg) == DF_FAM_PGEGLU; }
static inline bool gemm_tile_is_wgeglu(int cfg) { return gemm_tile_family(cfg) == DF_FAM_WGEGLU; }
static inline bool gemm_tile_has_mode(int cfg, int mode) { return cfg >= 0 && cfg < TILE_ALL && ((kGemmTiles[cfg].modes >> mode) & 1); }
static inline int gemm_mode(const GemmParams& p) { return (p.taps == 4) ? 3 : (p.taps != 9) ? 0 : ((p.stride == 1 && !p.ups) ? 1 : 2); }
static inline int gemm_ln_max_slots() { return 20; }

static inline int gemm_halo_dma_threads(int cfg) {
  const GemmTileInfo& t = kGemmTiles[cfg];
  return 64 * t.wgm * t.wgn * (t.ps ? t.ps : 1);
}
static inline int gemm_halo_ring(int cfg) { return kGemmTiles[cfg].ring; }
static inline void gemm_tile_dims(int cfg, int* bm, int* bn) {
  *bm = kGemmTiles[cfg].bm;
  *bn = kGemmTiles[cfg].bn;
}

bool gemm_tile_valid(const GemmParams& p, int tile, int batch, int splitk);

hipError_t launch_gemm(const GemmParams& p, int tile_cfg, int batch, hipStream_t stream);
hipError_t launch_pack_w320(const uint16_t* w, const float* cs, const float* bb, uint16_t* wo, float* cso, float* bbo, int N, int K, hipStream_t s);
```

### diff_foley_amd/csrc/gemm.hip

```cpp
#include <algorithm>
#include <stdlib.h>

#include "gemm_impl.h"


hipError_t launch_gemm_m0a(int tile_cfg, int epi, const GemmParams& p, int zdim, hipStream_t stream);
hipError_t launch_gemm_m0b(int tile_cfg, int epi, const GemmParams& p, int zdim, hipStream_t stream);
hipError_t launch_gemm_m1(int tile_cfg, int epi, const GemmParams& p, int zdim, hipStream_t stream);
hipError_t launch_gemm_m2(int tile_cfg, int epi, const GemmParams& p, int zdim, hipStream_t stream);
hipError_t launch_gemm_halo(int tile_cfg, int epi, const GemmParams& p, int zdim, hipStream_t stream);
hipError_t launch_gemm_m3(int tile_cfg, int epi, const GemmParams& p, int zdim, hipStream_t stream);
hipError_t launch_gemm_ps(int mode, int tile_cfg, int epi, const GemmParams& p, int zdim, hipStream_t stream);
hipError_t launch_gemm_ps_small(int mode, int tile_cfg, int epi, const GemmParams& p, int zdim, hipStream_t stream);
hipError_t launch_gemm_pgeglu(int tile_cfg, const GemmParams& p, hipStream_t stream);
bool pgeglu_valid(const GemmParams& p, int tile, int batch, int splitk);
hipError_t launch_gemm_wgeglu(int tile_cfg, const GemmParams& p, hipStream_t stream);
bool wgeglu_valid(const GemmParams& p, int tile, int batch, int splitk);

namespace {

__global__ __launch_bounds__(256) void splitk_reduce_kernel(GemmParams p) {
  const int nout = p.geglu ? (p.N >> 1) : p.N;
  const long total = (long)p.M * nout;
  for (long e = (long)blockIdx.x * blockDim.x + threadIdx.x; e < total; e += (long)gridDim.x * blockDim.x) {
// ... 35 lines not shown
__global__ __launch_bounds__(256) void splitk_reduce_vec_kernel(GemmParams p) {
#if defined(__HIP_DEVICE_COMPILE__)
  const DfTouch ka = gemm_kernarg_touch();
#endif
  const int n4 = p.N >> 2;
  const long total = (long)p.M * n4;
  const long slab = (long)p.M * p.N;
  const bool has_bias = p.bias != nullptr, has_rb = p.rowbias != nullptr, has_res = p.res != nullptr;
  for (long e = (long)blockIdx.x * blockDim.x + threadIdx.x; e < total; e += (long)gridDim.x * blockDim.x) {
    const int row = (int)(e / n4), col = (int)(e - (long)row * n4) * 4;
    const float* src = p.partial + (long)row * p.N + col;
    float4 t[SK];
#pragma unroll
    for (int s = 0; s < SK; ++s) t[s] = *reinterpret_cast<const float4*>(src + s * slab);
    float4 v = t[0];
#pragma unroll
    for (int s = 1; s < SK; ++s) {
      v.x += t[s].x; v.y += t[s].y; v.z += t[s].z; v.w += t[s].w;
    }
    v.x *= p.alpha; v.y *= p.alpha; v.z *= p.alpha; v.w *= p.alpha;
    if (p.ln_stats) {
      const float2* sp = p.ln_stats + (long)row * p.ln_slots;
      float s1 = 0.f, s2 = 0.f;
      for (int i = 0; i < p.ln_slots; ++i) {
        const float2 t2 = sp[i];
        s1 += t2.x;
        s2 += t2.y;
      }
      const float inv = 1.0f / (float)p.ln_C;
      const float mean = s1 * inv, rstd = rsqrtf(fmaxf(s2 * inv - mean * mean, 0.f) + p.ln_eps);
      const float4 cs = *reinterpret_cast<const float4*>(&p.ln_cs[col]);
      v.x = rstd * (v.x - mean * cs.x); v.y = rstd * (v.y - mean * cs.y);
      v.z = rstd * (v.z - mean * cs.z); v.w = rstd * (v.w - mean * cs.w);
    }
    if (has_bias) {
      const float4 b = *reinterpret_cast<const float4*>(&p.bias[col]);
      v.x += b.x; v.y += b.y; v.z += b.z; v.w += b.w;
    }
    if (has_rb) {
      const int ri = (p.rowbias_mode == 1) ? (row / p.rows_per_sample) : (row % p.rows_per_sample);
      const float4 b = *reinterpret_cast<const float4*>(&p.rowbias[(long)ri * p.ld_rowbias + col]);
      v.x += b.x; v.y += b.y; v.z += b.z; v.w += b.w;
    }
    if (has_res) {
      const float4 b = *reinterpret_cast<const float4*>(&p.res[(long)row * p.ldr + col]);
      v.x += b.x; v.y += b.y; v.z += b.z; v.w += b.w;
    }
    if (p.silu && !p.ln_stats && !p.stats) {
      v.x = silu_f(v.x); v.y = silu_f(v.y); v.z = silu_f(v.z); v.w = silu_f(v.w);
    }
    if (p.relu) {
      v.x = fmaxf(v.x, 0.f); v.y = fmaxf(v.y, 0.f); v.z = fmaxf(v.z, 0.f); v.w = fmaxf(v.w, 0.f);
    }
    if (p.stats) {
      const float s1 = row16_sum((v.x + v.y) + (v.z + v.w));
      const float s2 = row16_sum((v.x * v.x + v.y * v.y) + (v.z * v.z + v.w * v.w));
      if ((threadIdx.x & 15) == 0) {
        p.stats[(long)row * p.stats_slots + (col >> 6)] = make_float2(s1, s2);
        if (p.dup_rows) p.stats[(long)(row + p.dup_rows) * p.stats_slots + (col >> 6)] = make_float2(s1, s2);
      }
    }
    for (int rep = 0; rep < (p.dup_rows ? 2 : 1); ++rep) {
      const long orow = row + (rep ? p.dup_rows : 0);
      const long idx = orow * p.ldc + col;
      if (p.no_c_store) {
      } else if (p.out_bf16)
        st_wt(reinterpret_cast<uint2*>(reinterpret_cast<bf16_t*>(p.C) + idx), make_uint2(pack_bf2(v.x, v.y), pack_bf2(v.z, v.w)));
      else
        st_wt(reinterpret_cast<float4*>(reinterpret_cast<float*>(p.C) + idx), v);
      if (p.aux) st_wt(reinterpret_cast<uint2*>(p.aux + orow * p.ld_aux + col), make_uint2(pack_bf2(v.x, v.y), pack_bf2(v.z, v.w)));
    }
  }
#if defined(__HIP_DEVICE_COMPILE__)
  gemm_kernarg_touch_end(ka);
#endif
}

}

bool gemm_tile_valid(const GemmParams& p, int tile, int batch, int splitk) {
  const int nk = p.K / 64;
  if (p.taps == 4) {
    if (!gemm_tile_has_mode(tile, 3) || batch > 1) return false;
    if (p.geglu || p.vt || p.ln_stats || p.stats || p.w_rows > 0 || p.sm_w > 0 || p.Cin2 > 0 || p.res || p.store_nchw) return false;
    if (splitk > 1 && (p.N & 3) != 0) return false;
    return splitk == 1 || nk / splitk >= 2;
  }
  if (gemm_tile_is_pgeglu(tile)) return pgeglu_valid(p, tile, batch, splitk);
  if (gemm_tile_is_wgeglu(tile)) return wgeglu_valid(p, tile, batch, splitk);
  if (!gemm_tile_has_mode(tile, gemm_mode(p))) return false;
  if (!gemm_tile_is_halo(tile)) {
    if (tile < 0 || tile >= TILE_ALL) return false;
    if (p.geglu && ((p.N & 63) != 0 || (p.ldc & 3) != 0)) return false;
    int bm_, bn_;
    gemm_tile_dims(tile, &bm_, &bn_);
    if (p.vt && (splitk > 1 || batch > 1 || p.vt_col0 % bn_ != 0)) return false;
    if (p.ln_stats && (batch > 1 || (p.geglu && splitk > 1))) return false;
    if (p.ln_stats && p.ln_slots > gemm_ln_max_slots()) return false;
    if (p.stats && batch > 1) return false;
    if (p.w_rows > 0 && (batch > 1 || p.taps != 1 || p.w_rows % bm_ != 0 || p.M % p.w_rows != 0)) return false;
    if (p.sm_w > 0 && (p.sm_w != 32 || splitk > 1 || !p.ln_stats || !p.out_bf16 || p.w_rows <= 0 || (p.N & 31) != 0 || p.geglu ||
                       p.vt || p.res || p.rowbias || p.aux || p.alpha != 1.f || !p.bias))
      return false;
    if (p.dup_rows > 0 && (batch > 1 || p.geglu || p.vt || p.sm_w > 0 || p.store_nchw || (p.N & 3) != 0 || (p.ldc & 3) != 0 ||
                           (p.ldr & 3) != 0 || (p.ld_rowbias & 3) != 0 || (p.ld_aux & 3) != 0))
      return false;
    if (p.Cin2 > 0 && (batch > 1 || (p.Cin2 & 63) != 0 || !p.A2)) return false;
    if (p.Cin2 > 0 && p.taps == 9 && (p.stride != 1 || p.ups)) return false;
    if (p.Cin2 > 0 && p.taps != 9 && (p.taps != 1 || p.Cin2 >= p.K)) return false;
    if (splitk > 1 && (p.N & 3) != 0) return false;
    return splitk == 1 || (batch <= 1 && nk / splitk >= 2);
  }
  if (splitk > 1 && (p.N & 3) != 0) return false;
  if (p.dup_rows > 0 && (p.store_nchw || (p.N & 3) != 0 || (p.ldc & 3) != 0 || (p.ldr & 3) != 0 || (p.ld_rowbias & 3) != 0 || (p.ld_aux & 3) != 0))
    return false;
  const bool halo_ps = tile >= TILE_HALO_PS_192x64 && tile <= TILE_HALO_PS_128x128;
  if (p.Cin2 > 0 && (!halo_ps || (p.Cin2 & 63) != 0 || !p.A2 || (p.lda2 & 7) != 0)) return false;
  if (p.taps != 9 || p.stride != 1 || p.ups != 0 || p.geglu || batch > 1) return false;
  int bm, bn, th, tw;
  gemm_tile_dims(tile, &bm, &bn);
  if (!halo_patch(p.H, p.Wd, bm, &th, &tw)) return false;
  const int threads = gemm_halo_dma_threads(tile), rpp = threads / 8;
  const int hr = (bm / (th * tw)) * (th + 2) * (tw + 2);
  const int apass = (hr + rpp - 1) / rpp, wpass = (bn + rpp - 1) / rpp;
  if (apass > 12) return false;
  if (p.Cin2 > 0 && 3 * bm > 2 * apass * rpp) return false;
  const int nstw = gemm_halo_ring(tile);
  if (((size_t)2 * apass * rpp + (size_t)nstw * wpass * rpp) * 128 + (size_t)std::max(bm, hr) * 4 > 160 * 1024) return false;
  if ((p.lda & 7) != 0) return false;
  const int nchunk = p.Cin / 64;
  return splitk == 1 || nchunk / splitk >= 1;
}

hipError_t launch_gemm(const GemmParams& p, int tile_cfg, int batch, hipStream_t stream) {
  if (gemm_tile_is_pgeglu(tile_cfg)) {
    if (!pgeglu_valid(p, tile_cfg, batch, p.splitk)) return hipErrorInvalidValue;
    return launch_gemm_pgeglu(tile_cfg, p, stream);
  }
  if (gemm_tile_is_wgeglu(tile_cfg)) {
    if (!wgeglu_valid(p, tile_cfg, batch, p.splitk)) return hipErrorInvalidValue;
    return launch_gemm_wgeglu(tile_cfg, p, stream);
  }
  const int zdim = (p.splitk > 1) ? p.splitk : (batch > 0 ? batch : 1);
  if (p.ln_stats || p.stats || p.vt) {
    const bool vec = !p.store_nchw && (p.N & 63) == 0 && (p.ldc & 3) == 0 && (p.ldr & 3) == 0 && (p.ld_rowbias & 3) == 0 &&
                     (p.ld_aux & 3) == 0;
    if (!vec || (p.vt && ((p.M & 3) != 0 || (p.vt_T & 3) != 0 || (p.ldvt & 3) != 0 || p.taps != 1))) return hipErrorInvalidValue;
    if (p.ln_stats && p.taps != 1) return hipErrorInvalidValue;
  }
  const bool vec = !p.store_nchw && (p.N & 3) == 0 && (p.ldc & 3) == 0 && (p.ldr & 3) == 0 && (p.ld_rowbias & 3) == 0 &&
                   (p.res_bs & 3) == 0 && (p.c_bs & 3) == 0 && (p.ld_aux & 3) == 0;
  int epi;
  if (p.splitk > 1) epi = EPI_SPLITK;
  else if (p.sm_w > 0) epi = EPI_XS;
  else if (p.geglu) epi = EPI_GEGLU;
  else if (p.ln_stats || p.vt) epi = EPI_LNC;
  else if (p.stats) epi = EPI_PROD;
  else if (!vec || p.relu || p.aux || p.alpha != 1.f) epi = EPI_ANY;
  else epi = EPI_LEAN;
  if ((epi == EPI_GEGLU || epi == EPI_LNC || epi == EPI_PROD) && (p.taps != 1 || p.alpha != 1.f || p.relu || p.silu || !vec))
    return hipErrorInvalidValue;
  if (epi == EPI_LNC && (!p.ln_stats || p.aux)) return hipErrorInvalidValue;
  if (epi == EPI_XS && (!p.ln_stats || p.taps != 1 || !vec || (p.N & 63) != 0)) return hipErrorInvalidValue;
  hipError_t e;
  const int mode = gemm_mode(p), part = (tile_cfg >= 0 && tile_cfg < TILE_ALL) ? kGemmTiles[tile_cfg].part : 0;
  if (mode == 3) {
    if (batch > 1 || gemm_tile_is_halo(tile_cfg) || p.OH != p.H || p.OW != p.Wd || p.K != 4 * p.Cin || p.w_bs != (long)p.N * p.K)
      return hipErrorInvalidValue;
    e = launch_gemm_m3(tile_cfg, epi, p, zdim, stream);
  } else if (gemm_tile_is_halo(tile_cfg)) e = launch_gemm_halo(tile_cfg, epi, p, zdim, stream);
  else if (gemm_tile_is_ps(tile_cfg)) e = part ? launch_gemm_ps_small(mode, tile_cfg, epi, p, zdim, stream) : launch_gemm_ps(mode, tile_cfg, epi, p, zdim, stream);
  else if (mode == 0) e = part ? launch_gemm_m0b(tile_cfg, epi, p, zdim, stream) : launch_gemm_m0a(tile_cfg, epi, p, zdim, stream);
  else if (mode == 1) e = launch_gemm_m1(tile_cfg, epi, p, zdim, stream);
  else e = launch_gemm_m2(tile_cfg, epi, p, zdim, stream);
  if (e != hipSuccess) return e;
  if (p.splitk > 1 && !p.defer_reduce && mode == 3) {
    GemmParams q = p;
    q.M = 4 * p.M;
    q.taps = 1;
    const long total = (long)q.M * (q.N >> 2);
    int blocks = (int)((total + 255) / 256);
    if (blocks > 4096) blocks = 4096;
    if ((q.N & 3) != 0 || (q.ldc & 3) != 0 || q.store_nchw) return hipErrorInvalidValue;
#define DF_RED3(SK) case SK: hipLaunchKernelGGL(splitk_reduce_vec_kernel<SK>, dim3(blocks), dim3(256), 0, stream, q); break;
    switch (p.splitk) {
      DF_RED3(2) DF_RED3(3) DF_RED3(4) DF_RED3(6) DF_RED3(8) DF_RED3(12) DF_RED3(16) DF_RED3(24) DF_RED3(32)
      default: hipLaunchKernelGGL(splitk_reduce_kernel, dim3(blocks), dim3(256), 0, stream, q); break;
    }
#undef DF_RED3
    return hipGetLastError();
  }
  if (p.splitk > 1 && p.dup_rows > 0 && p.defer_reduce) return hipErrorInvalidValue;
  if (p.splitk > 1 && !p.defer_reduce) {
    const bool vec = !p.geglu && !p.store_nchw && (p.N & 3) == 0 && (p.ldc & 3) == 0 && (p.ldr & 3) == 0 &&
                     (p.ld_rowbias & 3) == 0 && (p.ld_aux & 3) == 0;
    if (vec) {
      const long total = (long)p.M * (p.N >> 2);
      int blocks = (int)((total + 255) / 256);
      if (blocks > 4096) blocks = 4096;
#define DF_RED(SK) case SK: hipLaunchKernelGGL(splitk_reduce_vec_kernel<SK>, dim3(blocks), dim3(256), 0, stream, p); break;
      switch (p.splitk) {
        DF_RED(2) DF_RED(3) DF_RED(4) DF_RED(6) DF_RED(8) DF_RED(12) DF_RED(16) DF_RED(24) DF_RED(32)
        default: hipLaunchKernelGGL(splitk_reduce_kernel, dim3(blocks), dim3(256), 0, stream, p); break;
      }
#undef DF_RED
    } else if (p.cfg_out) {
      if (!p.store_nchw || p.geglu || p.res || p.aux || p.silu || p.relu || (p.M & 1) || p.hw_out <= 0 || (p.M >> 1) % p.hw_out != 0)
        return hipErrorInvalidValue;
      const long total = (long)(p.M >> 1) * p.N;
      int blocks = (int)((total + 255) / 256);
      if (blocks > 2048) blocks = 2048;
      hipLaunchKernelGGL(splitk_reduce_cfg_kernel, dim3(blocks), dim3(256), 0, stream, p);
    } else {
      const int nout = p.geglu ? (p.N >> 1) : p.N;
      const long total = (long)p.M * nout;
      int blocks = (int)((total + 255) / 256);
      if (blocks > 2048) blocks = 2048;
      hipLaunchKernelGGL(splitk_reduce_kernel, dim3(blocks), dim3(256), 0, stream, p);
    }
    e = hipGetLastError();
  }
  return e;
}
```

### diff_foley_amd/csrc/gemm_impl.h

```cpp
#include <algorithm>

#pragma once
#include "common.h"
#include "gemm.h"

namespace {

constexpr int BK = 64;

enum { EPI_LEAN = 0, EPI_SPLITK = 1, EPI_GEGLU = 2, EPI_PROD = 3, EPI_LNC = 4, EPI_ANY = 5, EPI_XS = 6 };

bool halo_patch(int H, int W, int BM, int* th, int* tw) {
  const int w = (W % 16 == 0) ? 16 : W;
  if (w <= 0 || BM % w != 0) return false;
  int h = BM / w;
  if (h > H) h = H;
  while (h > 1 && (H % h != 0 || BM % (h * w) != 0)) --h;
  if (h <= 0 || H % h != 0 || BM % (h * w) != 0) return false;
  *th = h;
  *tw = w;
  return true;
}

__device__ __forceinline__ float row16_sum(float v) {
// ... 85 lines not shown
#pragma unroll
          for (int r = 0; r < 16; ++r)
            if (rowv[r] < p.M) epi_store(p, batch, rowv[r], ocol, nout, v[r]);
        }
      }
      continue;
    }
    const int col = col0 + j * 32 + l31;
    const int cc = min(col, p.N - 1);
    const float b0 = has_bias ? p.bias[cc] : 0.f;
    float v[16];
#pragma unroll
    for (int r = 0; r < 16; ++r) v[r] = acc[j][r] * p.alpha + b0;
    if (has_rb) {
      float rb_[16];
#pragma unroll
      for (int r = 0; r < 16; ++r) {
        const int ri = (p.rowbias_mode == 1) ? (rowc[r] / p.rows_per_sample) : (rowc[r] % p.rows_per_sample);
        rb_[r] = p.rowbias[(long)ri * p.ld_rowbias + cc];
      }
#pragma unroll
      for (int r = 0; r < 16; ++r) v[r] += rb_[r];
    }
    if (has_res) {
      float rr[16];
#pragma unroll
      for (int r = 0; r < 16; ++r) rr[r] = p.res[(long)batch * p.res_bs + (long)rowc[r] * p.ldr + cc];
#pragma unroll
      for (int r = 0; r < 16; ++r) v[r] += rr[r];
    }
    if (col < p.N) {
#pragma unroll
      for (int r = 0; r < 16; ++r)
        if (rowv[r] < p.M) epi_store(p, batch, rowv[r], col, nout, v[r]);
    }
  }
}

struct EpiVec { float4 hb0, hb1, hc0, hc1; };
template <int BN, int NT, int EPI>
__device__ __forceinline__ EpiVec epi_prefetch(const GemmParams& p, int n0, int tid) {
  EpiVec ev;
  ev.hb0 = ev.hb1 = ev.hc0 = ev.hc1 = make_float4(0.f, 0.f, 0.f, 0.f);
  if (p.store_nchw || (p.N & 3)) return ev;
  if constexpr (EPI == EPI_GEGLU) {
    static_assert(NT % (BN / 8) == 0, "invariant column per thread");
    const int oc = (tid % (BN / 8)) * 4, xc = (oc >> 5) * 64 + (oc & 31);
    const int gx = min(n0 + xc, p.N - 36);
    if (p.ln_stats) {
      ev.hc0 = *reinterpret_cast<const float4*>(&p.ln_cs[gx]);
      ev.hc1 = *reinterpret_cast<const float4*>(&p.ln_cs[gx + 32]);
    }
    if (p.bias) {
      ev.hb0 = *reinterpret_cast<const float4*>(&p.bias[gx]);
      ev.hb1 = *reinterpret_cast<const float4*>(&p.bias[gx + 32]);
    }
  } else if constexpr (EPI != EPI_SPLITK && EPI != EPI_XS) {
    static_assert(NT % (BN / 4) == 0, "invariant column per thread");
    const int cch = min(n0 + (tid % (BN / 4)) * 4, p.N - 4);
    if (p.bias) ev.hb0 = *reinterpret_cast<const float4*>(&p.bias[cch]);
    if constexpr (EPI == EPI_LNC)
      if (p.ln_stats) ev.hc0 = *reinterpret_cast<const float4*>(&p.ln_cs[cch]);
  }
  return ev;
}

__device__ __forceinline__ void epilogue_block_idle() {
  __builtin_amdgcn_s_barrier();
  __builtin_amdgcn_s_barrier();
}
template <int BM, int BN, int NT, int TM, int TN, int EPI, bool PARK = true, class RowMap>
__device__ __forceinline__ void epilogue_block(const GemmParams& p, int z, int batch, float* sC,
                                               f32x16 (&acc)[TM][TN], int wrow0, int wcol0, int n0, int tid,
                                               RowMap rowmap, const EpiVec& ev, float2 ln_mr = make_float2(0.f, 1.f)) {
  constexpr int LDC = BN + 4;
  const int lane = tid & 63, l31 = lane & 31, lh = lane >> 5;
  float2* sRow = reinterpret_cast<float2*>(sC + BM * LDC);
  const float4 hb0 = ev.hb0, hb1 = ev.hb1, hc0 = ev.hc0, hc1 = ev.hc1;
#define DF_EPI_STAMP(K) \
  if ((p.dbg & 64) && p.splitk <= 1 && p.partial && tid == 0) \
    reinterpret_cast<unsigned long long*>(p.partial)[(long)blockIdx.x * 32 + 24 + (K)] = __builtin_amdgcn_s_memtime();
  DF_EPI_STAMP(0)
  __builtin_amdgcn_s_barrier();
  if ((EPI == EPI_LNC || EPI == EPI_GEGLU || EPI == EPI_XS) && p.ln_stats && tid < BM) sRow[tid] = ln_mr;
  if constexpr (PARK) {
#pragma unroll
    for (int i = 0; i < TM; ++i)
#pragma unroll
      for (int j = 0; j < TN; ++j)
#pragma unroll
        for (int r = 0; r < 16; ++r)
          sC[(wrow0 + i * 32 + (r & 3) + 8 * (r >> 2) + 4 * lh) * LDC + wcol0 + j * 32 + l31] = acc[i][j][r];
  }
  __syncthreads();
  DF_EPI_STAMP(1)
  const bool has_bias = p.bias != nullptr, has_rb = p.rowbias != nullptr, has_res = p.res != nullptr;
  if constexpr (EPI == EPI_SPLITK) {
    float* part = p.partial + (long)z * p.M * p.N;
    constexpr int CPR = BN / 4;
#pragma unroll 4
    for (int e = tid; e < BM * CPR; e += NT) {
      const int r = e / CPR, c4 = (e - r * CPR) * 4;
      const int row = rowmap(r), col = n0 + c4;
      const float4 v = *reinterpret_cast<const float4*>(&sC[r * LDC + c4]);
      if (row < p.M && col < p.N) st_wt(reinterpret_cast<float4*>(&part[(long)row * p.N + col]), v);
    }
    return;
  } else if constexpr (EPI == EPI_XS) {
    constexpr int CPR = BN / 4;
#pragma unroll 2
    for (int ei = 0; ei < BM * CPR / NT; ++ei) {
      const int e = tid + ei * NT;
      const int r = e / CPR, c4 = (e - r * CPR) * 4;
      const int row = rowmap(r), col = n0 + c4;
      const int rc = min(row, p.M - 1), cc = min(col, p.N - 4);
      float4 v = *reinterpret_cast<const float4*>(&sC[r * LDC + c4]);
      const float2 mr = sRow[r];
      const long so = (long)(rc / p.w_rows) * p.N + cc;
      const float4 cs = *reinterpret_cast<const float4*>(&p.ln_cs[so]);
      const float4 bb = *reinterpret_cast<const float4*>(&p.bias[so]);
      v.x = mr.y * (v.x - mr.x * cs.x) + bb.x; v.y = mr.y * (v.y - mr.x * cs.y) + bb.y;
      v.z = mr.y * (v.z - mr.x * cs.z) + bb.z; v.w = mr.y * (v.w - mr.x * cs.w) + bb.w;
      const int g0 = col & 31;
      const float NEG = -3.0e38f;
      if (g0 + 0 >= p.sm_valid) v.x = NEG;
      if (g0 + 1 >= p.sm_valid) v.y = NEG;
      if (g0 + 2 >= p.sm_valid) v.z = NEG;
      if (g0 + 3 >= p.sm_valid) v.w = NEG;
      float mx = fmaxf(fmaxf(v.x, v.y), fmaxf(v.z, v.w));
      mx = fmaxf(mx, dpp_xor1(mx));
      mx = fmaxf(mx, dpp_xor2(mx));
      mx = fmaxf(mx, dpp_half_mirror(mx));
      v.x = g0 + 0 < p.sm_valid ? __expf(v.x - mx) : 0.f;
      v.y = g0 + 1 < p.sm_valid ? __expf(v.y - mx) : 0.f;
      v.z = g0 + 2 < p.sm_valid ? __expf(v.z - mx) : 0.f;
      v.w = g0 + 3 < p.sm_valid ? __expf(v.w - mx) : 0.f;
      float sm = (v.x + v.y) + (v.z + v.w);
      sm += dpp_xor1(sm);
      sm += dpp_xor2(sm);
      sm += dpp_half_mirror(sm);
      const float inv = 1.0f / sm;
      if (row < p.M && col < p.N)
        st_wt(reinterpret_cast<uint2*>(reinterpret_cast<bf16_t*>(p.C) + (long)row * p.ldc + col),
              make_uint2(pack_bf2(v.x * inv, v.y * inv), pack_bf2(v.z * inv, v.w * inv)));
    }
    return;
  } else if constexpr (EPI == EPI_GEGLU) {
    constexpr int CPR = BN / 8;
    const int nout = p.N >> 1;
#pragma unroll 2
    for (int e = tid; e < BM * CPR; e += NT) {
      const int r = e / CPR, oc = (e - r * CPR) * 4;
      const int xc = (oc >> 5) * 64 + (oc & 31);
      const int row = rowmap(r), ocol = (n0 >> 1) + oc;
      float4 x = *reinterpret_cast<const float4*>(&sC[r * LDC + xc]);
      float4 g = *reinterpret_cast<const float4*>(&sC[r * LDC + xc + 32]);
      if (p.ln_stats) {
        const float2 mr = sRow[r];
        const float4 cx = hc0, cg = hc1;
        x.x = mr.y * (x.x - mr.x * cx.x); x.y = mr.y * (x.y - mr.x * cx.y); x.z = mr.y * (x.z - mr.x * cx.z); x.w = mr.y * (x.w - mr.x * cx.w);
        g.x = mr.y * (g.x - mr.x * cg.x); g.y = mr.y * (g.y - mr.x * cg.y); g.z = mr.y * (g.z - mr.x * cg.z); g.w = mr.y * (g.w - mr.x * cg.w);
      }
      if (has_bias) {
        const float4 bx = hb0, bg = hb1;
        x.x = x.x * p.alpha + bx.x; x.y = x.y * p.alpha + bx.y; x.z = x.z * p.alpha + bx.z; x.w = x.w * p.alpha + bx.w;
        g.x = g.x * p.alpha + bg.x; g.y = g.y * p.alpha + bg.y; g.z = g.z * p.alpha + bg.z; g.w = g.w * p.alpha + bg.w;
      }
      float4 v = make_float4(x.x * gelu_erf(g.x), x.y * gelu_erf(g.y), x.z * gelu_erf(g.z), x.w * gelu_erf(g.w));
      if (row < p.M && ocol < nout) {
        const long idx = (long)batch * p.c_bs + (long)row * p.ldc + ocol;
        if (p.out_bf16)
          st_wt(reinterpret_cast<uint2*>(reinterpret_cast<bf16_t*>(p.C) + idx), make_uint2(pack_bf2(v.x, v.y), pack_bf2(v.z, v.w)));
        else
          st_wt(reinterpret_cast<float4*>(reinterpret_cast<float*>(p.C) + idx), v);
      }
    }
    return;
  } else {
  constexpr int CPR = BN / 4;
  const int rps_sh = (has_rb && p.rows_per_sample > 0 && (p.rows_per_sample & (p.rows_per_sample - 1)) == 0)
                         ? (31 - __builtin_clz(p.rows_per_sample)) : -1;
  if (EPI == EPI_LNC && p.vt && n0 >= p.vt_col0) {
    constexpr int RG = BM / 4, CG = BN / 4;
    const int cv = p.N - p.vt_col0;
#pragma unroll 2
    for (int e = tid; e < CG * RG; e += NT) {
      const int cg = e / RG, r = (e - cg * RG) * 4, c4 = cg * 4;
      const int row = rowmap(r), col = n0 + c4;
      const int cc = min(col, p.N - 4);
      float4 v[4];
#pragma unroll
      for (int j = 0; j < 4; ++j) {
        v[j] = *reinterpret_cast<const float4*>(&sC[(r + j) * LDC + c4]);
        v[j].x *= p.alpha; v[j].y *= p.alpha; v[j].z *= p.alpha; v[j].w *= p.alpha;
      }
      if (p.ln_stats) {
        const float4 cs = *reinterpret_cast<const float4*>(&p.ln_cs[cc]);
#pragma unroll
        for (int j = 0; j < 4; ++j) {
          const float2 mr = sRow[r + j];
          v[j].x = mr.y * (v[j].x - mr.x * cs.x); v[j].y = mr.y * (v[j].y - mr.x * cs.y);
          v[j].z = mr.y * (v[j].z - mr.x * cs.z); v[j].w = mr.y * (v[j].w - mr.x * cs.w);
        }
      }
      if (has_bias) {
        const float4 b = *reinterpret_cast<const float4*>(&p.bias[cc]);
#pragma unroll
        for (int j = 0; j < 4; ++j) { v[j].x += b.x; v[j].z += b.z; v[j].w += b.w; }
        pk_add_hi(v[0].y, v[1].y, b.x, b.y);
        pk_add_hi(v[2].y, v[3].y, b.x, b.y);
      }
      if (row < p.M && col < p.N) {
        const int smp = row / p.vt_T, t = row - smp * p.vt_T;
        bf16_t* dst = p.vt + ((long)smp * cv + (col - p.vt_col0)) * p.ldvt + t;
        st_wt(reinterpret_cast<uint2*>(dst), make_uint2(pack_bf2(v[0].x, v[1].x), pack_bf2(v[2].x, v[3].x)));
        st_wt(reinterpret_cast<uint2*>(dst + p.ldvt), make_uint2(pack_bf2(v[0].y, v[1].y), pack_bf2(v[2].y, v[3].y)));
        st_wt(reinterpret_cast<uint2*>(dst + 2 * p.ldvt), make_uint2(pack_bf2(v[0].z, v[1].z), pack_bf2(v[2].z, v[3].z)));
        st_wt(reinterpret_cast<uint2*>(dst + 3 * p.ldvt), make_uint2(pack_bf2(v[0].w, v[1].w), pack_bf2(v[2].w, v[3].w)));
      }
    }
    return;
  }
#define DF_EPI_LOOP(FL)                                                                                             \
  _Pragma("unroll 4") for (int ei = 0; ei < BM * CPR / NT; ++ei) {                                                  \
    const int e = tid + ei * NT;                                                                                    \
    const int r = e / CPR, c4 = (e - r * CPR) * 4;                                                                  \
    const int row = rowmap(r), col = n0 + c4;                                                                       \
    const int rc = min(row, p.M - 1), cc = min(col, p.N - 4);                                                       \
    float4 v = *reinterpret_cast<const float4*>(&sC[r * LDC + c4]);                                                 \
    if ((FL) & 16) { v.x *= p.alpha; v.y *= p.alpha; v.z *= p.alpha; v.w *= p.alpha; }                              \
    if ((FL) & 2) {                                                                                                 \
      const float2 mr = sRow[r];                                                                                    \
      const float4 cs = hc0;                                                                                        \
      v.x = mr.y * (v.x - mr.x * cs.x); v.y = mr.y * (v.y - mr.x * cs.y);                                           \
      v.z = mr.y * (v.z - mr.x * cs.z); v.w = mr.y * (v.w - mr.x * cs.w);                                           \
    }                                                                                                               \
    if (has_bias_l) {                                                                                               \
      const float4 b = hb0;                                                                                         \
      v.x += b.x; v.y += b.y; v.z += b.z; v.w += b.w;                                                               \
    }                                                                                                               \
    if (has_rb_l) {                                                                                                 \
      const int ri = (rps_sh >= 0) ? ((p.rowbias_mode == 1) ? (rc >> rps_sh) : (rc & (p.rows_per_sample - 1)))      \
                                   : ((p.rowbias_mode == 1) ? (rc / p.rows_per_sample) : (rc % p.rows_per_sample)); \
      const float4 b = *reinterpret_cast<const float4*>(&p.rowbias[(long)ri * p.ld_rowbias + cc]);                  \
      v.x += b.x; v.y += b.y; v.z += b.z; v.w += b.w;                                                               \
    }                                                                                                               \
    if (has_res_l) {                                                                                                \
      const float4 b = *reinterpret_cast<const float4*>(&p.res[(long)batch * p.res_bs + (long)rc * p.ldr + cc]);    \
      v.x += b.x; v.y += b.y; v.z += b.z; v.w += b.w;                                                               \
    }                                                                                                               \
    if (!((FL) & (2 | 4)) && p.silu) {                                                                              \
      v.x = silu_f(v.x); v.y = silu_f(v.y); v.z = silu_f(v.z); v.w = silu_f(v.w);                                   \
    }                                                                                                               \
    if (((FL) & 1) && p.relu) {                                                                                     \
      v.x = fmaxf(v.x, 0.f); v.y = fmaxf(v.y, 0.f); v.z = fmaxf(v.z, 0.f); v.w = fmaxf(v.w, 0.f);                   \
    }                                                                                                               \
    const bool ok = row < p.M && col < p.N;                                                                         \
    if ((FL) & 4) {                                                                                                 \
      const float s1 = row16_sum(ok ? (v.x + v.y) + (v.z + v.w) : 0.f);                                             \
      const float s2 = row16_sum(ok ? (v.x * v.x + v.y * v.y) + (v.z * v.z + v.w * v.w) : 0.f);                     \
      if (ok && (tid & 15) == 0) {                                                                                  \
        st_wt(&p.stats[(long)row * p.stats_slots + (col >> 6)], make_float2(s1, s2));                                      \
        if (p.dup_rows) st_wt(&p.stats[(long)(row + p.dup_rows) * p.stats_slots + (col >> 6)], make_float2(s1, s2));       \
      }                                                                                                             \
    }                                                                                                               \
    if (ok) {                                                                                                       \
      const long idx = (long)batch * p.c_bs + (long)row * p.ldc + col;                                              \
      if (((FL) & 4) && p.no_c_store) {  \
      } else if (p.out_bf16)                                                                                        \
        st_wt(reinterpret_cast<uint2*>(reinterpret_cast<bf16_t*>(p.C) + idx), make_uint2(pack_bf2(v.x, v.y), pack_bf2(v.z, v.w))); \
      else                                                                                                          \
        st_wt(reinterpret_cast<float4*>(reinterpret_cast<float*>(p.C) + idx), v);                                        \
      if (((FL) & 1) && p.aux)                                                                                      \
        st_wt(reinterpret_cast<uint2*>(p.aux + (long)row * p.ld_aux + col), make_uint2(pack_bf2(v.x, v.y), pack_bf2(v.z, v.w))); \
      if (p.dup_rows) {                              \
        const long idx2 = idx + (long)p.dup_rows * p.ldc;                                                           \
        if (((FL) & 4) && p.no_c_store) {                                                                            \
        } else if (p.out_bf16)                                                                                      \
          st_wt(reinterpret_cast<uint2*>(reinterpret_cast<bf16_t*>(p.C) + idx2), make_uint2(pack_bf2(v.x, v.y), pack_bf2(v.z, v.w))); \
        else                                                                                                        \
          st_wt(reinterpret_cast<float4*>(reinterpret_cast<float*>(p.C) + idx2), v);                                     \
        if (((FL) & 1) && p.aux)                                                                                    \
          st_wt(reinterpret_cast<uint2*>(p.aux + (long)(row + p.dup_rows) * p.ld_aux + col), make_uint2(pack_bf2(v.x, v.y), pack_bf2(v.z, v.w))); \
      }                                                                                                             \
    }                                                                                                               \
  }
  bool pre_added = false;
  if constexpr (EPI == EPI_PROD || EPI == EPI_LEAN) {
    constexpr int ITERS = BM * CPR / NT;
    if (has_rb || has_res) {
      float4 rbv[ITERS], rsv[ITERS];
      if (has_rb) {
#pragma unroll
        for (int ei = 0; ei < ITERS; ++ei) {
          const int e = tid + ei * NT, r = e / CPR, c4 = (e - r * CPR) * 4;
          const int rc = min(rowmap(r), p.M - 1), cc = min(n0 + c4, p.N - 4);
          const int ri = (rps_sh >= 0) ? ((p.rowbias_mode == 1) ? (rc >> rps_sh) : (rc & (p.rows_per_sample - 1)))
                                       : ((p.rowbias_mode == 1) ? (rc / p.rows_per_sample) : (rc % p.rows_per_sample));
          rbv[ei] = *reinterpret_cast<const float4*>(&p.rowbias[(long)ri * p.ld_rowbias + cc]);
        }
      }
      if (has_res) {
#pragma unroll
        for (int ei = 0; ei < ITERS; ++ei) {
          const int e = tid + ei * NT, r = e / CPR, c4 = (e - r * CPR) * 4;
          const int rc = min(rowmap(r), p.M - 1), cc = min(n0 + c4, p.N - 4);
          rsv[ei] = *reinterpret_cast<const float4*>(&p.res[(long)batch * p.res_bs + (long)rc * p.ldr + cc]);
        }
      }
#pragma unroll
      for (int ei = 0; ei < ITERS; ++ei) {
        const int e = tid + ei * NT, r = e / CPR, c4 = (e - r * CPR) * 4;
        float4 v = *reinterpret_cast<const float4*>(&sC[r * LDC + c4]);
        if (has_bias) { v.x += hb0.x; v.y += hb0.y; v.z += hb0.z; v.w += hb0.w; }
        if (has_rb) { v.x += rbv[ei].x; v.y += rbv[ei].y; v.z += rbv[ei].z; v.w += rbv[ei].w; }
        if (has_res) { v.x += rsv[ei].x; v.y += rsv[ei].y; v.z += rsv[ei].z; v.w += rsv[ei].w; }
        *reinterpret_cast<float4*>(&sC[r * LDC + c4]) = v;
      }
      pre_added = true;
    }
  }
  DF_EPI_STAMP(2)
  const bool has_bias_l = has_bias && !pre_added, has_rb_l = has_rb && !pre_added, has_res_l = has_res && !pre_added;
  if constexpr (EPI == EPI_LEAN || EPI == EPI_PROD) {
    constexpr int ITERS = BM * CPR / NT, RSTEP = NT / CPR;
    const bool plain = !p.dup_rows && !p.silu && !p.relu && (EPI == EPI_PROD || (!p.out_bf16 && !p.aux));
    if (plain) {
      const int rb0 = tid / CPR, c4 = (tid - rb0 * CPR) * 4, col = n0 + c4;
      const bool colok = col < p.N;
      const long cbase = (long)batch * p.c_bs + col;
#pragma unroll
      for (int ei = 0; ei < ITERS; ++ei) {
        const int r = rb0 + ei * RSTEP;
        const int row = rowmap(r);
        float4 v = *reinterpret_cast<const float4*>(&sC[r * LDC + c4]);
        if (has_bias_l) { v.x += hb0.x; v.y += hb0.y; v.z += hb0.z; v.w += hb0.w; }
        const bool ok = colok && row < p.M;
        if constexpr (EPI == EPI_PROD) {
          const float s1 = row16_sum(ok ? (v.x + v.y) + (v.z + v.w) : 0.f);
          const float s2 = row16_sum(ok ? (v.x * v.x + v.y * v.y) + (v.z * v.z + v.w * v.w) : 0.f);
          if (ok) {
            if ((tid & 15) == 0) st_wt(&p.stats[(long)row * p.stats_slots + (col >> 6)], make_float2(s1, s2));
            if (!p.no_c_store) {
              if (p.out_bf16)
                st_wt(reinterpret_cast<uint2*>(reinterpret_cast<bf16_t*>(p.C) + cbase + (long)row * p.ldc), make_uint2(pack_bf2(v.x, v.y), pack_bf2(v.z, v.w)));
              else
                st_wt(reinterpret_cast<float4*>(reinterpret_cast<float*>(p.C) + cbase + (long)row * p.ldc), v);
            }
            if (p.aux) st_wt(reinterpret_cast<uint2*>(p.aux + (long)row * p.ld_aux + col), make_uint2(pack_bf2(v.x, v.y), pack_bf2(v.z, v.w)));
          }
// ... 1078 lines not shown
```

### diff_foley_amd/csrc/kernels.h

```cpp
#pragma once
#include <hip/hip_runtime.h>
#include <stdint.h>

hipError_t launch_groupnorm(const float* x, int ld, int N, int HW, int C, const float* gamma, const float* beta,
                            float eps, int silu, uint16_t* out, int ldo, uint16_t* raw_out, hipStream_t s);

hipError_t launch_groupnorm_slabs(const float* x, int ld, int N, int HW, int C, const float* gamma, const float* beta,
                                  float eps, int silu, uint16_t* out, int ldo, uint16_t* raw_out, int nslab,
                                  long slab_stride, const float* bias, const float* rowbias, int ld_rowbias, hipStream_t s);
bool groupnorm_accepts_slabs(int HW, int C);
enum { GN_FORM_STREAMING = -1, GN_FORM_CHUNKED = -2, GN_FORM_REFUSED = -3 };
int groupnorm_form(int N, int HW, int C, int nslab);
hipError_t launch_groupnorm_own_slabs(float* x, int ld, int N, int HW, int C, const float* gamma, const float* beta, float eps,
                                      int silu, uint16_t* out, int ldo, uint16_t* raw_out, const float* slab0, int nslab,
                                      long slab_stride, int c_own, const float* bias, const float* res, int ldr, hipStream_t s);

size_t groupnorm_scratch_bytes(int N, int HW, int C);
hipError_t launch_groupnorm_chunked(const float* x, int ld, int N, int HW, int C, const float* gamma, const float* beta,
                                    float eps, int silu, uint16_t* out, int ldo, uint16_t* raw_out, float* scratch,
                                    hipStream_t s);

hipError_t launch_layernorm(const float* x, int ld, int rows, int C, const float* gamma, const float* beta,
                            float eps, uint16_t* out, hipStream_t s);

hipError_t launch_attention(const uint16_t* Q, int ldq, const uint16_t* K, int ldk, const uint16_t* Vt, int ldvt,
                            uint16_t* O, int ldo, int N, int heads, int D, int Tq, int Tk, float scale,
                            hipStream_t s);
bool attention_supported(int D);
int attention_form(int D, int Tq, int Tk);

bool conv3x3_fewout_ok(int H, int W, int C, int Cout);
hipError_t launch_conv3x3_fewout(const uint16_t* X, const uint16_t* Wt , const float* bias, float* out, int NB, int H, int W,
                                 int C, int Cout, hipStream_t s);

hipError_t launch_softmax_rows(const float* s, uint16_t* p, int rows, int T, int ldp, hipStream_t st);

hipError_t launch_linear_rows(const float* a, int lda, const uint16_t* W, const float* bias, float* out, int ldo,
                              int M, int N, int K, int act_out , hipStream_t s);

hipError_t launch_timestep_embedding(const float* t, float* out, int N, int dim, hipStream_t s);

hipError_t launch_timestep_embedding_b16(const float* t, int t_B, uint16_t* out, int N, int dim, hipStream_t s);

hipError_t launch_pack_latent(const float* x, uint16_t* out, int B, int C, int HW, int cpad, int rep, float in_scale,
                              const float* wpq, const float* bpq, hipStream_t s);

hipError_t launch_cast_bf16(const float* x, uint16_t* out, long n, hipStream_t s);

hipError_t launch_cast_bf16_2d(const float* x, int ld, uint16_t* out, long rows, int C, hipStream_t s);

hipError_t launch_pack_conv_weight(const float* w, uint16_t* out, int O, int I, int KH, int KW, int Ipad, hipStream_t s);
hipError_t launch_pack_conv_ups4(const float* w, uint16_t* out, int O, int I, int Ipad, hipStream_t s);
hipError_t launch_pack_ln_linear(const float* w, const float* bias, const float* gamma, const float* beta,
                                 uint16_t* wout, float* cs, float* bb, int rows, int K, int row_off, int geglu_half,
                                 hipStream_t s);
hipError_t launch_pack_conv_skip(const float* w, const float* ws, uint16_t* out, int O, int I, int I2, hipStream_t s);
hipError_t launch_xattn_expand(const uint16_t* kv, uint16_t* Kexp, uint16_t* Vexp, int NB, int Tc, int Tcp, int C, int H,
                               hipStream_t s);
hipError_t launch_pack_lnq_t(const float* Wq, const float* gamma, uint16_t* out, int C, float scale, hipStream_t s);
hipError_t launch_xattn_rowstats(const uint16_t* G, const uint16_t* Kexp, const float* bq, float scale, int C, long rows, float* cs,
                                 float* bb, hipStream_t s);
hipError_t launch_pack_ffproj(const float* Wp, const float* bp, const float* W2, const float* b2, uint16_t* wout, float* bout,
                              int C, int F, hipStream_t s);
hipError_t launch_pack_geglu(const float* w, const float* b, uint16_t* wout, float* bout, int half_rows, int K,
                             hipStream_t s);

hipError_t launch_bcast_rows(const float* src, float* dst, int rows, int n, hipStream_t s);
hipError_t launch_pack_latent_bcast(const float* x, uint16_t* out, int B, int C, int HW, int cpad, int rep, const float* src,
                                    float* dst, int rows, int n, hipStream_t s);
hipError_t launch_cfg_combine(const float* e2, float* e, long n, float scale, hipStream_t s);
hipError_t launch_lincomb(float* out, const float* const* in, const float* coef, int nterms, long n, hipStream_t s);
hipError_t launch_q_sample_blend(const float* img, const float* x0, const float* noise, const float* mask, float* out, long n,
                                 long chw, long hw, int mask_c, float a, float b, hipStream_t s);
hipError_t launch_ddim_update(const float* x, const float* e, const float* noise, float* x_prev, float* pred_x0,
                              long n, float sqrt_at, float s1m, float sqrt_aprev, float dir_coef, float sigma,
                              hipStream_t s);
hipError_t launch_avgpool(const float* x, float* out, int N, int HW, int C, hipStream_t s);

hipError_t launch_groupnorm_bwd(const float* x, int ld, int N, int HW, int C, const float* gamma, const float* beta,
                                float eps, int silu, const float* dy, int lddy, const float* addend, int ldadd,
                                float* dx, int lddx, uint16_t* dx_b16, hipStream_t s);
hipError_t launch_layernorm_bwd(const float* x, int rows, int C, const float* gamma, float eps, const float* dy,
                                const float* addend, float* dx, uint16_t* dx_b16, hipStream_t s);
hipError_t launch_geglu_fwd(const uint16_t* u, uint16_t* y, long rows, int H, hipStream_t s);
hipError_t launch_geglu_bwd(const uint16_t* u, const float* dy, uint16_t* du, long rows, int H, hipStream_t s);
size_t attention_bwd_ws_floats(int N, int heads, int D, int Tq, int Tk, int lddk, int lddv, bool want_dkv);
hipError_t launch_attention_bwd(const uint16_t* Q, int ldq, const uint16_t* K, int ldk, const uint16_t* Vt, int ldvt,
                                const float* dO, int lddo, uint16_t* dQ, int lddq, uint16_t* dK, int lddk, uint16_t* dV,
                                int lddv, int N, int heads, int D, int Tq, int Tk, float scale, float* ws, hipStream_t s);
hipError_t launch_attention_bwd(const uint16_t* Q, int ldq, const uint16_t* K, int ldk, const uint16_t* Vt, int ldvt,
                                const float* dO, int lddo, uint16_t* dQ, int lddq, uint16_t* dK, int lddk, uint16_t* dV,
                                int lddv, int N, int heads, int D, int Tq, int Tk, float scale, float* ws, int form, hipStream_t s);
hipError_t launch_cls_head_bwd(const float* prob, const float* w, float* dh, uint16_t* dh_b16, int N, int HW, int C, int Cp,
                               hipStream_t s);
hipError_t launch_grad_scale_per_sample(float* x, const float* prob, int N, long per, hipStream_t s);
hipError_t launch_pack_linear_t(const float* w, uint16_t* out, int O, int I, int ldo, int off, hipStream_t s);
hipError_t launch_pack_conv_bwd(const float* w, uint16_t* out, int O, int I, int Opad, hipStream_t s);

hipError_t launch_stem_im2col(const float* x, uint16_t* out, int F, int H, int W, int OH, int OW, int KP, hipStream_t s);
hipError_t launch_maxpool3x3s2(const uint16_t* x, uint16_t* out, int F, int H, int W, int OH, int OW, int C, hipStream_t s);
hipError_t launch_subsample2(const uint16_t* x, uint16_t* out, int F, int H, int W, int C, hipStream_t s);
hipError_t launch_tcat3(const uint16_t* x, uint16_t* out, int F, int T, int HW, int C, hipStream_t s);
hipError_t launch_pack_conv3d_bn(const float* w, const float* gamma, const float* beta, const float* mean,
                                 const float* var, float eps, uint16_t* out, float* bias, int O, int I, int KT, int KH,
                                 int KW, int KP, hipStream_t s);
hipError_t launch_maxpool_time(const float* x, float* out, int B, int T, int C, int k, hipStream_t s);
hipError_t launch_l2norm_rows(float* x, int rows, int C, hipStream_t s);

hipError_t launch_frames_to_tensor(const uint8_t* frames, float* out, uint8_t* tmp, int T, int H, int W, int OH, int OW,
                                   const int* bounds_w, const int* coef_w, int ksize_w, const int* bounds_h,
                                   const int* coef_h, int ksize_h, hipStream_t s);

hipError_t launch_mel_to_stft(const float* mel, int B, int NM, int T, const float* A, const float* At, const float* Pt,
                              float inv_L, int iters, float* S, hipStream_t s);
hipError_t launch_griffinlim(const float* S, const float* phase0, int B, int T, int n_iter, float momentum, const float2* tw,
                             const float* window, const float* wss, float2* angles, float2* reb0, float2* reb1, float* frames,
                             float* y, hipStream_t s);
```

### diff_foley_amd/engine.py

```python
import ctypes as C
import itertools
import os

import torch

_HERE = os.path.dirname(os.path.abspath(__file__))
LIB_PATH = os.path.join(_HERE, "libdfengine.so")
LIB_PATHS = {"bf16": LIB_PATH, "fp16": os.path.join(_HERE, "libdfengine_f16.so")}
OPERAND_DTYPE = {"bf16": torch.bfloat16, "fp16": torch.float16}


def default_precision():
    p = os.environ.get("DF_PRECISION", "fp16")
    if p not in LIB_PATHS:
        raise RuntimeError(f"DF_PRECISION={p!r}: expected one of {sorted(LIB_PATHS)}")
    return p


class GemmDesc(C.Structure):
    _fields_ = [("size", C.c_int64), ("A", C.c_void_p), ("W", C.c_void_p), ("C", C.c_void_p)] + [
        (n, C.c_int) for n in ("M", "N", "K", "lda", "ldc", "out_operand", "conv", "NB", "H", "Wd", "Cin", "stride", "batch", "tile",
                               "splitk", "gm")] + [
        (n, C.c_int64) for n in ("a_bs", "w_bs", "c_bs", "res_bs")] + [
        ("alpha", C.c_float), ("bias", C.c_void_p), ("rowbias", C.c_void_p), ("ld_rowbias", C.c_int), ("rows_per_sample", C.c_int),
        ("rowbias_mode", C.c_int), ("res", C.c_void_p), ("ldr", C.c_int), ("relu", C.c_int), ("silu", C.c_int), ("aux", C.c_void_p),
        ("ld_aux", C.c_int), ("stats", C.c_void_p), ("stats_slots", C.c_int), ("ln_stats", C.c_void_p), ("ln_slots", C.c_int),
        ("ln_C", C.c_int), ("ln_eps", C.c_float), ("ln_cs", C.c_void_p), ("w_rows", C.c_int), ("sm_w", C.c_int),
        ("sm_valid", C.c_int), ("dup_rows", C.c_int), ("no_c_store", C.c_int), ("store_nchw", C.c_int), ("hw_out", C.c_int),
        ("cfg_out", C.c_void_p), ("cfg_scale", C.c_float), ("defer_reduce", C.c_int), ("slabs_out", C.c_void_p),
        ("ups", C.c_int), ("zstuff", C.c_int), ("A2", C.c_void_p), ("lda2", C.c_int), ("Cin2", C.c_int), ("geglu", C.c_int),
        ("vt", C.c_void_p), ("vt_col0", C.c_int), ("vt_T", C.c_int), ("ldvt", C.c_int)]

    def __init__(self, **kw):
        kw.setdefault("alpha", 1.0)
        super().__init__(size=C.sizeof(GemmDesc), **kw)


class GemmTile(C.Structure):
    _fields_ = [("size", C.c_int64), ("name", C.c_char_p)] + [(n, C.c_int) for n in ("family", "bm", "bn", "dma_threads", "ring", "modes")]


TILE_FAMILIES = ("generic", "halo", "ps", "pgeglu", "wgeglu", "retired")


def gemm_tiles(L=None):
    L = L or lib()
    out, t = {}, GemmTile(size=C.sizeof(GemmTile))
    while L.df_test_gemm_tile_info(len(out), C.byref(t)) == 0:
        out[len(out)] = dict(name=t.name.decode(), family=TILE_FAMILIES[t.family], bm=t.bm, bn=t.bn, dma_threads=t.dma_threads,
                             ring=t.ring, modes=tuple(m for m in range(4) if t.modes >> m & 1))
    return out


class UNetConfig(C.Structure):
    _fields_ = [("in_channels", C.c_int), ("out_channels", C.c_int), ("model_channels", C.c_int),
                ("num_res_blocks", C.c_int), ("channel_mult", C.c_int * 8), ("n_mult", C.c_int),
                ("attention_resolutions", C.c_int * 8), ("n_attn", C.c_int), ("num_heads", C.c_int),
                ("context_dim", C.c_int)]


class VaeConfig(C.Structure):
    _fields_ = [("z_channels", C.c_int), ("embed_dim", C.c_int), ("ch", C.c_int), ("num_res_blocks", C.c_int),
                ("out_ch", C.c_int), ("ch_mult", C.c_int * 8), ("n_mult", C.c_int), ("scale_factor", C.c_float)]


class CondConfig(C.Structure):
    _fields_ = [("origin_dim", C.c_int), ("embed_dim", C.c_int), ("seq_len", C.c_int)]


class CavpConfig(C.Structure):
    _fields_ = [("stage_blocks", C.c_int * 4), ("base_channels", C.c_int), ("embed_dim", C.c_int)]


_libs = {}

_SIGS = {
    "df_create": [C.c_int, C.POINTER(C.c_void_p)],
    "df_config_unet": [C.c_void_p, C.POINTER(UNetConfig)],
    "df_config_vae": [C.c_void_p, C.POINTER(VaeConfig)],
    "df_config_cond": [C.c_void_p, C.POINTER(CondConfig)],
    "df_config_cavp": [C.c_void_p, C.POINTER(CavpConfig)],
    "df_cavp_encode": [C.c_void_p, C.c_void_p, C.c_void_p, C.c_int, C.c_int, C.c_int, C.c_int, C.c_int, C.c_void_p],
    "df_cavp_pool": [C.c_void_p, C.c_void_p, C.c_int, C.c_int, C.c_int, C.c_int, C.c_int, C.c_void_p],
    "df_config_classifier": [C.c_void_p, C.POINTER(UNetConfig)],
    "df_load_tensor": [C.c_void_p, C.c_char_p, C.c_void_p, C.POINTER(C.c_int64), C.c_int],
    "df_load_tensor_dev": [C.c_void_p, C.c_char_p, C.c_void_p, C.POINTER(C.c_int64), C.c_int],
    "df_finalize": [C.c_void_p],
    "df_autotune": [C.c_void_p, C.c_int],
    "df_cond_encode": [C.c_void_p, C.c_void_p, C.c_void_p, C.c_int, C.c_int, C.c_void_p],
    "df_unet_set_context": [C.c_void_p, C.c_void_p, C.c_int, C.c_int, C.c_void_p],
    "df_unet_forward": [C.c_void_p, C.c_void_p, C.c_void_p, C.c_void_p, C.c_int, C.c_int, C.c_int, C.c_void_p],
    "df_unet_forward_cfg": [C.c_void_p, C.c_void_p, C.c_void_p, C.c_void_p, C.c_int, C.c_int, C.c_int, C.c_float,
                            C.c_void_p],
    "df_unet_set_timesteps": [C.c_void_p, C.c_void_p, C.c_int, C.c_int, C.c_int, C.c_int, C.c_int, C.c_void_p],
    "df_unet_forward_ts": [C.c_void_p, C.c_void_p, C.c_int, C.c_void_p, C.c_int, C.c_int, C.c_int, C.c_void_p],
    "df_unet_forward_cfg_ts": [C.c_void_p, C.c_void_p, C.c_int, C.c_void_p, C.c_int, C.c_int, C.c_int, C.c_float,
                               C.c_void_p],
    "df_vae_decode": [C.c_void_p, C.c_void_p, C.c_void_p, C.c_int, C.c_int, C.c_int, C.c_void_p],
    "df_classifier_forward": [C.c_void_p, C.c_void_p, C.c_void_p, C.c_void_p, C.c_void_p, C.c_int, C.c_int, C.c_int,
                              C.c_int, C.c_void_p],
    "df_classifier_grad": [C.c_void_p, C.c_void_p, C.c_void_p, C.c_void_p, C.c_void_p, C.c_void_p, C.c_int, C.c_int,
                           C.c_int, C.c_int, C.c_void_p],
    "df_classifier_grad_cached": [C.c_void_p, C.c_void_p, C.c_void_p, C.c_void_p, C.c_void_p, C.c_void_p, C.c_int, C.c_int,
                                  C.c_int, C.c_int, C.c_uint64, C.c_void_p],
    "df_prepack": [C.c_void_p, C.c_int, C.c_int, C.c_int, C.c_int],
    "df_packed_size": [C.c_void_p, C.POINTER(C.c_size_t), C.POINTER(C.c_size_t)],
    "df_export_packed": [C.c_void_p, C.c_void_p, C.c_void_p, C.c_void_p],
    "df_import_packed": [C.c_void_p, C.c_void_p, C.c_size_t, C.c_void_p, C.c_size_t, C.c_void_p],
    "df_frames_to_tensor": [C.c_void_p, C.c_void_p, C.c_void_p] + [C.c_int] * 5 + [C.c_void_p, C.c_void_p, C.c_int, C.c_void_p,
                                                                                  C.c_void_p, C.c_int, C.c_void_p],
    "df_mel_to_stft": [C.c_void_p, C.c_int, C.c_int, C.c_int, C.c_void_p, C.c_void_p, C.c_void_p, C.c_float, C.c_int, C.c_void_p,
                       C.c_void_p],
    "df_griffinlim": [C.c_void_p, C.c_void_p, C.c_int, C.c_int, C.c_int, C.c_float] + [C.c_void_p] * 9,
    "df_cfg_combine": [C.c_void_p, C.c_void_p, C.c_int64, C.c_float, C.c_void_p],
    "df_lincomb": [C.c_void_p, C.POINTER(C.c_void_p), C.POINTER(C.c_float), C.c_int, C.c_int64, C.c_void_p],
    "df_q_sample_blend": [C.c_void_p, C.c_void_p, C.c_void_p, C.c_void_p, C.c_void_p, C.c_int64, C.c_int64, C.c_int64, C.c_int,
                          C.c_float, C.c_float, C.c_void_p],
    "df_ddim_update": [C.c_void_p, C.c_void_p, C.c_void_p, C.c_void_p, C.c_void_p, C.c_int64, C.c_float, C.c_float,
                       C.c_float, C.c_float, C.c_void_p],
    "df_plan_count": [C.c_void_p, C.POINTER(C.c_int64), C.POINTER(C.c_int64)],
    "df_unet_plan_stats": [C.c_void_p, C.POINTER(C.c_int64), C.POINTER(C.c_double), C.POINTER(C.c_double)],
    "df_profile_begin": [C.c_void_p],
    "df_profile_end": [C.c_void_p, C.POINTER(C.c_double), C.POINTER(C.c_int64)],
    "df_profile_dump": [C.c_void_p, C.c_char_p],
    "df_tune_cache_export": [C.c_char_p, C.c_int64, C.POINTER(C.c_int64)],
    "df_tune_cache_import": [C.c_char_p, C.c_int64],
    "df_debug_checksums": [C.c_void_p, C.c_int, C.c_int64],
    "df_debug_checksums_read": [C.c_void_p, C.POINTER(C.c_uint64), C.c_int64, C.POINTER(C.c_int64)],
    "df_debug_checksum_label": [C.c_void_p, C.c_int64, C.c_char_p, C.c_int64],
    "df_test_geglu": [C.c_void_p, C.c_void_p, C.c_void_p, C.c_void_p, C.c_void_p, C.c_void_p, C.c_int, C.c_int, C.c_int, C.c_int,
                      C.c_int, C.c_void_p],
    "df_test_scratch_read": [C.c_void_p, C.c_int64],
    "df_test_conv3x3_fewout": [C.c_void_p, C.c_void_p, C.c_void_p, C.c_void_p] + [C.c_int] * 5 + [C.c_void_p],
    "df_debug_saturations": [C.c_void_p, C.c_int, C.c_int64],
    "df_debug_saturations_read": [C.c_void_p, C.POINTER(C.c_uint64), C.c_int64, C.POINTER(C.c_int64)],
    "df_debug_saturation_label": [C.c_void_p, C.c_int64, C.c_char_p, C.c_int64],
    "df_debug_requant": [C.c_void_p, C.c_char_p],
    "df_test_gemm_epi": [C.c_void_p, C.c_void_p, C.c_void_p, C.c_void_p, C.c_void_p, C.c_int, C.c_int, C.c_int, C.c_int,
                         C.c_int, C.c_int, C.c_int, C.c_void_p],
    "df_test_gemm_dual": [C.c_void_p, C.c_void_p, C.c_void_p, C.c_void_p, C.c_int, C.c_int, C.c_int, C.c_int, C.c_int, C.c_int,
                          C.c_void_p],
    "df_test_gemm": [C.c_void_p, C.c_void_p, C.c_void_p, C.c_int, C.c_int, C.c_int, C.c_int, C.c_int, C.c_void_p],
    "df_test_ln_chain": [C.c_void_p] * 11 + [C.c_int] * 10 + [C.c_void_p],
    "df_test_linear_rows": [C.c_void_p, C.c_int, C.c_void_p, C.c_void_p, C.c_void_p] + [C.c_int] * 5 + [C.c_void_p],
    "df_test_unet_block": [C.c_void_p, C.c_char_p, C.c_int, C.c_void_p, C.c_void_p, C.c_void_p, C.c_void_p] + [C.c_int] * 6
                          + [C.c_void_p],
    "df_test_conv3x3": [C.c_void_p, C.c_void_p, C.c_void_p, C.c_void_p] + [C.c_int] * 9 + [C.c_void_p],
    "df_test_conv3x3_skip": [C.c_void_p, C.c_void_p, C.c_void_p, C.c_void_p, C.c_void_p] + [C.c_int] * 8 + [C.c_void_p],
    "df_test_conv3x3_ups4": [C.c_void_p, C.c_void_p, C.c_void_p, C.c_void_p, C.c_void_p, C.c_int, C.c_int, C.c_int, C.c_int, C.c_int,
                             C.c_int, C.c_int, C.c_void_p],
    "df_test_groupnorm": [C.c_void_p, C.c_int, C.c_int, C.c_int, C.c_int, C.c_void_p, C.c_void_p, C.c_float, C.c_int,
                          C.c_void_p, C.c_void_p],
    "df_test_groupnorm_own_slabs": [C.c_void_p, C.c_int, C.c_int, C.c_int, C.c_int, C.c_void_p, C.c_void_p, C.c_float, C.c_int,
                                    C.c_void_p, C.c_void_p, C.c_int, C.c_int, C.c_void_p, C.c_void_p, C.c_int, C.c_void_p],
    "df_test_groupnorm_form": [C.c_int] * 4,
    "df_test_attention_form": [C.c_int] * 3,
    "df_test_groupnorm_ex": [C.c_void_p, C.c_int, C.c_int, C.c_int, C.c_int, C.c_void_p, C.c_void_p, C.c_float, C.c_int, C.c_void_p,
                             C.c_int, C.c_void_p, C.c_int, C.c_int64, C.c_void_p, C.c_void_p, C.c_int, C.c_void_p, C.c_int, C.c_void_p,
                             C.c_int, C.c_void_p],
    "df_test_layernorm": [C.c_void_p, C.c_int, C.c_int, C.c_void_p, C.c_void_p, C.c_void_p, C.c_void_p],
    "df_test_layernorm_ex": [C.c_void_p, C.c_int, C.c_int, C.c_int, C.c_void_p, C.c_void_p, C.c_void_p, C.c_void_p],
    "df_test_attention": [C.c_void_p, C.c_int, C.c_void_p, C.c_int, C.c_void_p, C.c_int, C.c_void_p, C.c_int, C.c_int,
                          C.c_int, C.c_int, C.c_int, C.c_int, C.c_float, C.c_void_p],
    "df_test_groupnorm_bwd": [C.c_void_p, C.c_int, C.c_int, C.c_int, C.c_int, C.c_void_p, C.c_void_p, C.c_float, C.c_int,
                              C.c_void_p, C.c_int, C.c_void_p, C.c_int, C.c_void_p, C.c_int, C.c_void_p, C.c_void_p],
    "df_test_layernorm_bwd": [C.c_void_p, C.c_int, C.c_int, C.c_void_p, C.c_float, C.c_void_p, C.c_void_p, C.c_void_p, C.c_void_p,
                              C.c_void_p],
    "df_test_geglu_fwd": [C.c_void_p, C.c_void_p, C.c_int64, C.c_int, C.c_void_p],
    "df_test_geglu_bwd": [C.c_void_p, C.c_void_p, C.c_void_p, C.c_int64, C.c_int, C.c_void_p],
    "df_test_attention_bwd": [C.c_void_p, C.c_int] * 7 + [C.c_int] * 5 + [C.c_float, C.c_int, C.c_void_p],
    "df_test_cls_head_bwd": [C.c_void_p] * 4 + [C.c_int] * 4 + [C.c_void_p],
    "df_test_pack_linear_t": [C.c_void_p, C.c_void_p] + [C.c_int] * 4 + [C.c_void_p],
    "df_test_pack_conv_bwd": [C.c_void_p, C.c_void_p] + [C.c_int] * 3 + [C.c_void_p],
    "df_test_conv3x3_bwd_data": [C.c_void_p] * 5 + [C.c_int] * 8 + [C.c_void_p],
    "df_test_gemm_ex": [C.POINTER(GemmDesc), C.c_void_p],
    "df_test_gemm_valid": [C.POINTER(GemmDesc), C.c_int, C.c_int, C.c_int],
    "df_test_gemm_key": [C.POINTER(GemmDesc), C.c_int, C.c_char_p, C.c_int],
    "df_test_gemm_tile_info": [C.c_int, C.POINTER(GemmTile)],
    "df_test_xattn_chain": [C.c_void_p] * 10 + [C.c_int] * 6 + [C.c_void_p] * 10 + [C.c_int, C.c_int, C.c_void_p],
    "df_test_pack_ffproj": [C.c_void_p] * 6 + [C.c_int, C.c_int, C.c_void_p],
    "df_test_softmax_rows": [C.c_void_p, C.c_void_p, C.c_int, C.c_int, C.c_int, C.c_void_p],
    "df_test_timestep_embedding": [C.c_void_p, C.c_void_p, C.c_int, C.c_int, C.c_void_p],
    "df_test_timestep_embedding_b16": [C.c_void_p, C.c_int, C.c_void_p, C.c_int, C.c_int, C.c_void_p],
    "df_test_pack_latent": [C.c_void_p, C.c_void_p] + [C.c_int] * 5 + [C.c_float, C.c_void_p, C.c_void_p, C.c_void_p],
    "df_test_pack_latent_bcast": [C.c_void_p, C.c_void_p] + [C.c_int] * 5 + [C.c_void_p, C.c_void_p, C.c_int, C.c_int, C.c_void_p],
    "df_test_bcast_rows": [C.c_void_p, C.c_void_p, C.c_int, C.c_int, C.c_void_p],
    "df_test_cast_bf16": [C.c_void_p, C.c_void_p, C.c_int64, C.c_void_p],
    "df_test_cast_bf16_2d": [C.c_void_p, C.c_int, C.c_void_p, C.c_int64, C.c_int, C.c_void_p],
    "df_test_avgpool": [C.c_void_p, C.c_void_p, C.c_int, C.c_int, C.c_int, C.c_void_p],
    "df_test_pack_conv_weight": [C.c_void_p, C.c_void_p] + [C.c_int] * 5 + [C.c_void_p],
    "df_test_pack_conv_skip": [C.c_void_p, C.c_void_p, C.c_void_p] + [C.c_int] * 3 + [C.c_void_p],
    "df_test_pack_geglu": [C.c_void_p] * 4 + [C.c_int, C.c_int, C.c_void_p],
    "df_test_pack_ln_linear": [C.c_void_p] * 7 + [C.c_int] * 4 + [C.c_void_p],
    "df_test_grad_scale_per_sample": [C.c_void_p, C.c_void_p, C.c_int, C.c_int64, C.c_void_p],
    "df_test_stem_im2col": [C.c_void_p, C.c_void_p] + [C.c_int] * 6 + [C.c_void_p],
    "df_test_maxpool3x3s2": [C.c_void_p, C.c_void_p] + [C.c_int] * 6 + [C.c_void_p],
    "df_test_subsample2": [C.c_void_p, C.c_void_p] + [C.c_int] * 4 + [C.c_void_p],
    "df_test_tcat3": [C.c_void_p, C.c_void_p] + [C.c_int] * 4 + [C.c_void_p],
    "df_test_pack_conv3d_bn": [C.c_void_p] * 5 + [C.c_float, C.c_void_p, C.c_void_p] + [C.c_int] * 6 + [C.c_void_p],
    "df_test_maxpool_time": [C.c_void_p, C.c_void_p] + [C.c_int] * 4 + [C.c_void_p],
    "df_test_l2norm_rows": [C.c_void_p, C.c_int, C.c_int, C.c_void_p],
    "df_test_peak": [C.c_int, C.c_void_p, C.c_void_p, C.c_size_t, C.c_int, C.c_void_p],
    "df_test_fill": [C.c_int, C.c_void_p, C.c_void_p, C.c_size_t, C.c_size_t, C.c_int, C.c_int, C.c_void_p],
}


def lib(precision=None):
    if precision is None and _libs:
        return next(iter(_libs.values()))
    precision = precision or default_precision()
    if precision not in _libs:
        path = os.environ.get("DF_LIB_OVERRIDE") or LIB_PATHS[precision]
        if not os.path.exists(path):
            raise RuntimeError(f"{path} not found: build it with diff_foley_amd/csrc/build.sh "
                               "(there is no CPU/torch fallback for the sampling path)")
        L = C.CDLL(path)
        for name, args in _SIGS.items():
            if os.environ.get("DF_LIB_OVERRIDE") and not hasattr(L, name):
                continue
            fn = getattr(L, name)
            fn.argtypes = args
            fn.restype = C.c_int
        L.df_last_error.restype = C.c_char_p
        L.df_destroy.argtypes = [C.c_void_p]
        L.df_destroy.restype = None
        L.df_abi_version.restype = C.c_int
        L.df_operand_dtype.restype = C.c_char_p
        want = {"bf16": b"bf16", "fp16": b"f16"}[precision]
        if L.df_operand_dtype() != want:
            raise RuntimeError(f"{path} was built for {L.df_operand_dtype()!r} operands, expected {want!r}")
        _libs[precision] = L
    return _libs[precision]


def exported_symbols():
    return list(_SIGS.keys()) + ["df_last_error", "df_destroy", "df_abi_version", "df_operand_dtype"]


def _chk(rc, L=None):
    if rc != 0:
        raise RuntimeError("libdfengine: " + (L or lib()).df_last_error().decode())


def _stream():
    return C.c_void_p(torch.cuda.current_stream().cuda_stream)


def _ptr(t):
    return C.c_void_p(t.data_ptr())


def _dev_f32(t, device):
    if t.device != device or t.dtype != torch.float32 or not t.is_contiguous():
        t = t.to(device=device, dtype=torch.float32).contiguous()
    return t


def _want_dim(what, got, want):
    if want is not None and int(got) != int(want):
        raise RuntimeError(f"{what}: last dimension is {got}, the loaded model expects {want}")


def _want_nchw(what, x, channels):
# ... 424 lines not shown
```

### include/df_engine.h

```cpp
#ifndef DF_ENGINE_H
#define DF_ENGINE_H
#include <stddef.h>
#include <stdint.h>

#ifdef __cplusplus
extern "C" {
#endif

typedef struct df_ctx df_ctx;

typedef struct {
  int in_channels, out_channels, model_channels, num_res_blocks;
  int channel_mult[8];
  int n_mult;
  int attention_resolutions[8];
  int n_attn;
  int num_heads;
  int context_dim;
} df_unet_config;

typedef struct {
  int z_channels, embed_dim, ch, num_res_blocks, out_ch;
  int ch_mult[8];
  int n_mult;
// ... 120 lines not shown
                         int NB, int H, int Wd, int Cin, int Cout, int tile, int splitk, void* stream);
int df_test_groupnorm(const float* x_dev, int ld, int N, int HW, int C, const float* gamma, const float* beta, float eps,
                      int silu, uint16_t* out_dev, void* stream);
int df_test_groupnorm_own_slabs(float* x_dev, int ld, int N, int HW, int C, const float* gamma, const float* beta, float eps,
                                int silu, uint16_t* out_dev, const float* slabs_dev, int nslab, int c_own,
                                const float* bias_dev, const float* res_dev, int ldr, void* stream);
int df_test_groupnorm_form(int N, int HW, int C, int nslab);
int df_test_attention_form(int D, int Tq, int Tk);
int df_test_groupnorm_ex(float* x_dev, int ld, int N, int HW, int C, const float* gamma, const float* beta, float eps, int silu,
                         uint16_t* out_dev, int ldo, uint16_t* raw_out_dev, int nslab, int64_t slab_stride, const float* bias_dev,
                         const float* rowbias_dev, int ld_rowbias, const float* own_slabs_dev, int c_own, const float* res_dev,
                         int ldr, void* stream);
int df_test_layernorm(const float* x_dev, int rows, int C, const float* gamma, const float* beta, uint16_t* out_dev,
                      void* stream);
int df_test_layernorm_ex(const float* x_dev, int ld, int rows, int C, const float* gamma, const float* beta, uint16_t* out_dev,
                         void* stream);
int df_test_attention(const uint16_t* Q, int ldq, const uint16_t* K, int ldk, const uint16_t* Vt, int ldvt, uint16_t* O,
                      int ldo, int N, int heads, int D, int Tq, int Tk, float scale, void* stream);
int df_test_groupnorm_bwd(const float* x_dev, int ld, int N, int HW, int C, const float* gamma, const float* beta, float eps,
                          int silu, const float* dy_dev, int lddy, const float* addend_dev, int ldadd, float* dx_dev, int lddx,
                          uint16_t* dx_b16_dev, void* stream);
int df_test_layernorm_bwd(const float* x_dev, int rows, int C, const float* gamma, float eps, const float* dy_dev,
                          const float* addend_dev, float* dx_dev, uint16_t* dx_b16_dev, void* stream);
int df_test_geglu_fwd(const uint16_t* u_dev, uint16_t* y_dev, int64_t rows, int H, void* stream);
int df_test_geglu_bwd(const uint16_t* u_dev, const float* dy_dev, uint16_t* du_dev, int64_t rows, int H, void* stream);
int df_test_attention_bwd(const uint16_t* Q, int ldq, const uint16_t* K, int ldk, const uint16_t* Vt, int ldvt, const float* dO,
                          int lddo, uint16_t* dQ, int lddq, uint16_t* dK, int lddk, uint16_t* dV, int lddv, int N, int heads, int D,
                          int Tq, int Tk, float scale, int form, void* stream);
int df_test_cls_head_bwd(const float* prob_dev, const float* w_dev, float* dh_dev, uint16_t* dh_b16_dev, int N, int HW, int C, int Cp,
                         void* stream);
int df_test_pack_linear_t(const float* w_dev, uint16_t* out_dev, int O, int I, int ldo, int off, void* stream);
int df_test_pack_conv_bwd(const float* w_dev, uint16_t* out_dev, int O, int I, int Opad, void* stream);
int df_test_conv3x3_bwd_data(const uint16_t* dY_dev, const float* W_oihw_dev, uint16_t* w_scratch_dev, float* dX_dev,
                             uint16_t* dX_op_dev, int NB, int H, int Wd, int I, int O, int stride, int tile, int splitk,
                             void* stream);
int df_test_softmax_rows(const float* s_dev, uint16_t* p_dev, int rows, int T, int ldp, void* stream);
int df_test_timestep_embedding(const float* t_dev, float* out_dev, int N, int dim, void* stream);
int df_test_timestep_embedding_b16(const float* t_dev, int t_B, uint16_t* out_dev, int N, int dim, void* stream);
int df_test_pack_latent(const float* x_dev, uint16_t* out_dev, int B, int C, int HW, int cpad, int rep, float in_scale,
                        const float* wpq_dev, const float* bpq_dev, void* stream);
int df_test_pack_latent_bcast(const float* x_dev, uint16_t* out_dev, int B, int C, int HW, int cpad, int rep, const float* src_dev,
                              float* dst_dev, int rows, int n, void* stream);
int df_test_bcast_rows(const float* src_dev, float* dst_dev, int rows, int n, void* stream);
int df_test_cast_bf16(const float* x_dev, uint16_t* out_dev, int64_t n, void* stream);
int df_test_cast_bf16_2d(const float* x_dev, int ld, uint16_t* out_dev, int64_t rows, int C, void* stream);
int df_test_avgpool(const float* x_dev, float* out_dev, int N, int HW, int C, void* stream);
int df_test_pack_conv_weight(const float* w_dev, uint16_t* out_dev, int O, int I, int KH, int KW, int Ipad, void* stream);
int df_test_pack_conv_skip(const float* w_dev, const float* ws_dev, uint16_t* out_dev, int O, int I, int I2, void* stream);
int df_test_pack_geglu(const float* w_dev, const float* b_dev, uint16_t* wout_dev, float* bout_dev, int half_rows, int K, void* stream);
int df_test_pack_ln_linear(const float* w_dev, const float* bias_dev, const float* gamma_dev, const float* beta_dev, uint16_t* wout_dev,
                           float* cs_dev, float* bb_dev, int rows, int K, int row_off, int geglu_half, void* stream);
int df_test_grad_scale_per_sample(float* x_dev, const float* prob_dev, int N, int64_t per, void* stream);
int df_test_stem_im2col(const float* x_dev, uint16_t* out_dev, int F, int H, int W, int OH, int OW, int KP, void* stream);
int df_test_maxpool3x3s2(const uint16_t* x_dev, uint16_t* out_dev, int F, int H, int W, int OH, int OW, int C, void* stream);
int df_test_subsample2(const uint16_t* x_dev, uint16_t* out_dev, int F, int H, int W, int C, void* stream);
int df_test_tcat3(const uint16_t* x_dev, uint16_t* out_dev, int F, int T, int HW, int C, void* stream);
int df_test_pack_conv3d_bn(const float* w_dev, const float* gamma_dev, const float* beta_dev, const float* mean_dev, const float* var_dev,
                           float eps, uint16_t* out_dev, float* bias_dev, int O, int I, int KT, int KH, int KW, int KP, void* stream);
int df_test_maxpool_time(const float* x_dev, float* out_dev, int B, int T, int C, int k, void* stream);
int df_test_l2norm_rows(float* x_dev, int rows, int C, void* stream);
typedef struct df_test_gemm_desc {
  int64_t size;
  const void* A; const void* W; void* C;
  int M, N, K, lda, ldc, out_operand;
  int conv, NB, H, Wd, Cin, stride;
  int batch, tile, splitk, gm;
  int64_t a_bs, w_bs, c_bs, res_bs;
  float alpha;
  const float* bias;
  const float* rowbias; int ld_rowbias, rows_per_sample, rowbias_mode;
  const float* res; int ldr;
  int relu, silu;
  void* aux; int ld_aux;
  void* stats; int stats_slots;
  const void* ln_stats; int ln_slots, ln_C; float ln_eps; const float* ln_cs;
  int w_rows, sm_w, sm_valid;
  int dup_rows, no_c_store, store_nchw, hw_out;
  float* cfg_out; float cfg_scale;
  int defer_reduce; float* slabs_out;
  int ups, zstuff;
  const void* A2; int lda2, Cin2;
  int geglu;
  void* vt; int vt_col0, vt_T, ldvt;
} df_test_gemm_desc;
int df_test_gemm_ex(const df_test_gemm_desc* d, void* stream);
int df_test_gemm_valid(const df_test_gemm_desc* d, int tile, int batch, int splitk);
int df_test_gemm_key(const df_test_gemm_desc* d, int batch, char* buf, int n);
typedef struct df_test_gemm_tile {
  int64_t size;
  const char* name;
  int family, bm, bn, dma_threads, ring, modes;
} df_test_gemm_tile;
int df_test_gemm_tile_info(int tile, df_test_gemm_tile* out);
int df_test_xattn_chain(const uint16_t* ctx_dev, const uint16_t* Wkv_dev, const float* Wq_dev, const float* gamma_dev,
                        const float* bq_dev, const uint16_t* Wo_dev, const float* bo_dev, const float* x_dev, const uint16_t* xb_dev,
                        const void* xstats_dev, int NB, int T, int Tc, int Dc, int C, int heads, uint16_t* kv_dev, uint16_t* Kexp_dev,
                        uint16_t* Vexp_dev, uint16_t* WqT_dev, uint16_t* G_dev, float* cs_dev, float* bb_dev, uint16_t* Vo_dev,
                        uint16_t* P_dev, float* out_dev, int tile_xs, int tile_xo, void* stream);
int df_test_pack_ffproj(const float* Wp_dev, const float* bp_dev, const float* W2_dev, const float* b2_dev, uint16_t* wout_dev,
                        float* bout_dev, int C, int F, void* stream);
int df_test_peak(int kind, const void* src_dev, void* dst_dev, size_t n, int blocks, void* stream);
int df_test_fill(int kind, const void* src_dev, void* dst_dev, size_t span, size_t stride_blk, int n, int blocks,
                 void* stream);


#ifdef __cplusplus
}
#endif
#endif
```

Baseline: 284.2 denoise_steps/s.

## Fold proj_in and norm1 into the fused QKV GEMM, normalising inside attention

Within each spatial transformer, the proj_in linear and the norm1 LayerNorm are folded algebraically into the QKV weights: proj_in weights are mean-centred and multiplied through gamma, and the offset terms become bias and e-vectors. One GEMM now writes t0 for the residual, the per-row LN statistics, QK and transposed V. The per-token rstd is applied to Q, K and V inside the attention kernel, and the e_v offset is added at output. This removes a separate GEMM launch and its activation round trip, at the cost of extra per-element scaling work in attention and a bounded token count (2048) that needs shared memory for the row scales.

New measurement: 274.3 denoise_steps/s. 0.965x the previous value.

```diff
diff --git a/diff_foley_amd/csrc/attention.hip b/diff_foley_amd/csrc/attention.hip
--- a/diff_foley_amd/csrc/attention.hip
+++ b/diff_foley_amd/csrc/attention.hip
@@ -9,11 +9,22 @@
   static constexpr int VROW = KT + 4;
 };
 
-template <int D, int NW, int KS = 1>
+struct AttnPreNorm {
+  const float2* stats; int slots; float inv_c, eps;
+  const float* e_q; const float* e_v;
+};
+constexpr int ATTN_PN_MAX_T = 2048;
+
+__device__ __forceinline__ uint32_t scale_op2(uint32_t v, float s0, float s1) {
+  return pack_bf2_hw(bf2f((uint16_t)(v & 0xFFFFu)) * s0, bf2f((uint16_t)(v >> 16)) * s1);
+}
+
+template <int D, int NW, int KS = 1, bool PN = false>
 __global__ __launch_bounds__(NW * 64) void attention_kernel(const bf16_t* __restrict__ Q, int ldq,
                                                             const bf16_t* __restrict__ K, int ldk,
                                                             const bf16_t* __restrict__ Vt, int ldvt, int heads, int Tq,
-                                                            int Tk, float scale_log2e, bf16_t* __restrict__ O, int ldo) {
+                                                            int Tk, float scale_log2e, bf16_t* __restrict__ O, int ldo,
+                                                            AttnPreNorm pn) {
   constexpr int DKC = (D + 15) / 16;
   constexpr int DKP = DKC * 16;
   constexpr int DT = (D + 31) / 32;
@@ -24,6 +35,8 @@
   static_assert(!ONES || (D % 8) == 0, "row D sits in half-wave 0");
   __shared__ __attribute__((aligned(16))) bf16_t sK[2 * KT * KROW];
   __shared__ __attribute__((aligned(16))) bf16_t sV[2 * DT * 32 * VROW];
+  __shared__ __attribute__((aligned(16))) float sR[PN ? ATTN_PN_MAX_T : 4];
+  if constexpr (PN) df_fp16_hw_clamp();
 
   const int tid = threadIdx.x, lane = tid & 63, wid = tid >> 6;
   const int l31 = lane & 31, lh = lane >> 5;
@@ -109,19 +122,27 @@
       }
     }
   };
-  auto sstore = [&](int buf) {
+  auto sstore = [&](int buf, int k0) {
     bf16_t* k_ = sK + buf * (KT * KROW);
     bf16_t* v_ = sV + buf * (DT * 32 * VROW);
 #pragma unroll
     for (int i = 0; i < KCH; ++i) {
       const int c = tid + i * NT;
       const int key = c / (DKP / 8), ch = c - key * (DKP / 8);
+      if constexpr (PN) {
+        const float r = sR[min(k0 + key, Tk - 1)];
+        kreg[i] = make_uint4(scale_op2(kreg[i].x, r, r), scale_op2(kreg[i].y, r, r), scale_op2(kreg[i].z, r, r), scale_op2(kreg[i].w, r, r));
+      }
       if (c < KT * (DKP / 8)) *reinterpret_cast<uint4*>(&k_[key * KROW + ch * 8]) = kreg[i];
     }
 #pragma unroll
     for (int i = 0; i < VCH; ++i) {
       const int c = tid + i * NT;
       const int d = c / VCR, ch = c - d * VCR;
+      if constexpr (PN) {
+        const float4 r = *reinterpret_cast<const float4*>(&sR[min(k0 + ch * 4, Tk - 4)]);
+        vreg[i] = make_uint2(scale_op2(vreg[i].x, r.x, r.y), scale_op2(vreg[i].y, r.z, r.w));
+      }
       if (c < DT * 32 * VCR && !(ONES && d == D)) *reinterpret_cast<uint2*>(&v_[d * VROW + ch * 4]) = vreg[i];
     }
   };
@@ -129,7 +150,37 @@
   gfetch(0);
   DfTouch code_touch = DfTouch();
   if constexpr (D >= 128) code_touch = df_entry_touch(0);
-  sstore(0);
+  if constexpr (PN) {
+    for (int t = tid; t < Tk; t += NT) {
+      const float2* sp = pn.stats + ((long)n * Tk + t) * pn.slots;
+      float s1 = 0.f, s2 = 0.f;
+#pragma unroll 5
+      for (int i = 0; i < pn.slots; ++i) {
+        const float2 t2 = sp[i];
+        s1 += t2.x;
+        s2 += t2.y;
+      }
+      const float mean = s1 * pn.inv_c;
+      sR[t] = rsqrtf(fmaxf(s2 * pn.inv_c - mean * mean, 0.f) + pn.eps);
+    }
+    __syncthreads();
+    const float rq = sR[qv ? q : 0];
+#pragma unroll
+    for (int c = 0; c < DKC; ++c) {
+      const int d0 = 16 * c + 8 * lh;
+      if (qv && d0 < D) {
+        const float4 e0 = *reinterpret_cast<const float4*>(pn.e_q + h * D + d0);
+        const float4 e1 = *reinterpret_cast<const float4*>(pn.e_q + h * D + d0 + 4);
+        const uint4 v = *reinterpret_cast<const uint4*>(&qf[c]);
+        auto fix = [&](uint32_t w, float a, float b) {
+          return pack_bf2_hw(bf2f((uint16_t)(w & 0xFFFFu)) * rq + a, bf2f((uint16_t)(w >> 16)) * rq + b);
+        };
+        const uint4 f = make_uint4(fix(v.x, e0.x, e0.y), fix(v.y, e0.z, e0.w), fix(v.z, e1.x, e1.y), fix(v.w, e1.z, e1.w));
+        qf[c] = *reinterpret_cast<const bf16x8*>(&f);
+      }
+    }
+  }
+  sstore(0, 0);
   if (ONES) {
 #if defined(DF_OPERAND_F16)
     constexpr uint32_t ONE2 = 0x3C003C00u;
@@ -225,7 +276,7 @@
           o[t] = DF_MFMA_32x32x16(vf, pf, o[t]);
         }
       }
-    if (kt + 1 < ntiles) sstore(buf ^ 1);
+    if (kt + 1 < ntiles) sstore(buf ^ 1, k0 + KT);
     __syncthreads();
   }
 
@@ -246,9 +297,11 @@
       for (int g = 0; g < 4; ++g) {
         const int d0 = 32 * t + 8 * g + 4 * lh;
         if (d0 < D) {
+          float4 ev = make_float4(0.f, 0.f, 0.f, 0.f);
+          if constexpr (PN) ev = *reinterpret_cast<const float4*>(pn.e_v + h * D + d0);
           uint2 w;
-          w.x = pack_bf2(o[t][4 * g] * inv, o[t][4 * g + 1] * inv);
-          w.y = pack_bf2(o[t][4 * g + 2] * inv, o[t][4 * g + 3] * inv);
+          w.x = pack_bf2(o[t][4 * g] * inv + ev.x, o[t][4 * g + 1] * inv + ev.y);
+          w.y = pack_bf2(o[t][4 * g + 2] * inv + ev.z, o[t][4 * g + 3] * inv + ev.w);
           *reinterpret_cast<uint2*>(orow + d0) = w;
         }
       }
@@ -256,25 +309,38 @@
   if constexpr (D >= 128) df_entry_touch_end(code_touch);
 }
 
-template <int D>
+template <int D, bool PN>
 hipError_t launch_d(const uint16_t* Q, int ldq, const uint16_t* K, int ldk, const uint16_t* Vt, int ldvt,
-                    uint16_t* O, int ldo, int N, int heads, int Tq, int Tk, float scale, hipStream_t s) {
+                    uint16_t* O, int ldo, int N, int heads, int Tq, int Tk, float scale, const AttnPreNorm& pn, hipStream_t s) {
   const float sl2 = scale * 1.4426950408889634f;
   const int form = attention_form(D, Tq, Tk), nw = form >> 4;
   if (nw < 1) return hipErrorInvalidValue;
   const dim3 grid((Tq + 32 * nw - 1) / (32 * nw), heads, N), block(64 * nw);
-#define DF_ATTN(...) hipLaunchKernelGGL((attention_kernel<D, __VA_ARGS__>), grid, block, 0, s, Q, ldq, K, ldk, Vt, ldvt, heads, Tq, Tk, sl2, O, ldo)
+#define DF_ATTN(NW_, KS_) hipLaunchKernelGGL((attention_kernel<D, NW_, KS_, PN>), grid, block, 0, s, Q, ldq, K, ldk, Vt, ldvt, heads, Tq, Tk, sl2, O, ldo, pn)
   switch (form) {
     case 4 * 16 + 2:
       if constexpr (D <= 80) { DF_ATTN(4, 2); break; }
       return hipErrorInvalidValue;
-    case 4 * 16 + 1: DF_ATTN(4); break;
-    case 2 * 16 + 1: DF_ATTN(2); break;
-    case 1 * 16 + 1: DF_ATTN(1); break;
+    case 4 * 16 + 1: DF_ATTN(4, 1); break;
+    case 2 * 16 + 1: DF_ATTN(2, 1); break;
+    case 1 * 16 + 1: DF_ATTN(1, 1); break;
     default: return hipErrorInvalidValue;
   }
 #undef DF_ATTN
   return hipGetLastError();
+}
+
+template <bool PN>
+hipError_t launch_any_d(const uint16_t* Q, int ldq, const uint16_t* K, int ldk, const uint16_t* Vt, int ldvt, uint16_t* O, int ldo,
+                        int N, int heads, int D, int Tq, int Tk, float scale, const AttnPreNorm& pn, hipStream_t s) {
+  if (ldvt % 32 != 0 || ldvt < ((Tk + 31) / 32) * 32) return hipErrorInvalidValue;
+#define DF_ATTN_D(D_) case D_: return launch_d<D_, PN>(Q, ldq, K, ldk, Vt, ldvt, O, ldo, N, heads, Tq, Tk, scale, pn, s);
+  switch (D) {
+    DF_ATTN_D(16) DF_ATTN_D(24) DF_ATTN_D(48) DF_ATTN_D(56) DF_ATTN_D(72) DF_ATTN_D(96) DF_ATTN_D(112) DF_ATTN_D(192)
+    DF_ATTN_D(32) DF_ATTN_D(40) DF_ATTN_D(64) DF_ATTN_D(80) DF_ATTN_D(128) DF_ATTN_D(160)
+    default: return hipErrorInvalidValue;
+  }
+#undef DF_ATTN_D
 }
 
 }
@@ -296,22 +362,16 @@
 hipError_t launch_attention(const uint16_t* Q, int ldq, const uint16_t* K, int ldk, const uint16_t* Vt, int ldvt,
                             uint16_t* O, int ldo, int N, int heads, int D, int Tq, int Tk, float scale,
                             hipStream_t s) {
-  if (ldvt % 32 != 0 || ldvt < ((Tk + 31) / 32) * 32) return hipErrorInvalidValue;
-  switch (D) {
-    case 16:  return launch_d<16>(Q, ldq, K, ldk, Vt, ldvt, O, ldo, N, heads, Tq, Tk, scale, s);
-    case 24:  return launch_d<24>(Q, ldq, K, ldk, Vt, ldvt, O, ldo, N, heads, Tq, Tk, scale, s);
-    case 48:  return launch_d<48>(Q, ldq, K, ldk, Vt, ldvt, O, ldo, N, heads, Tq, Tk, scale, s);
-    case 56:  return launch_d<56>(Q, ldq, K, ldk, Vt, ldvt, O, ldo, N, heads, Tq, Tk, scale, s);
-    case 72:  return launch_d<72>(Q, ldq, K, ldk, Vt, ldvt, O, ldo, N, heads, Tq, Tk, scale, s);
-    case 96:  return launch_d<96>(Q, ldq, K, ldk, Vt, ldvt, O, ldo, N, heads, Tq, Tk, scale, s);
-    case 112: return launch_d<112>(Q, ldq, K, ldk, Vt, ldvt, O, ldo, N, heads, Tq, Tk, scale, s);
-    case 192: return launch_d<192>(Q, ldq, K, ldk, Vt, ldvt, O, ldo, N, heads, Tq, Tk, scale, s);
-    case 32:  return launch_d<32>(Q, ldq, K, ldk, Vt, ldvt, O, ldo, N, heads, Tq, Tk, scale, s);
-    case 40:  return launch_d<40>(Q, ldq, K, ldk, Vt, ldvt, O, ldo, N, heads, Tq, Tk, scale, s);
-    case 64:  return launch_d<64>(Q, ldq, K, ldk, Vt, ldvt, O, ldo, N, heads, Tq, Tk, scale, s);
-    case 80:  return launch_d<80>(Q, ldq, K, ldk, Vt, ldvt, O, ldo, N, heads, Tq, Tk, scale, s);
-    case 128: return launch_d<128>(Q, ldq, K, ldk, Vt, ldvt, O, ldo, N, heads, Tq, Tk, scale, s);
-    case 160: return launch_d<160>(Q, ldq, K, ldk, Vt, ldvt, O, ldo, N, heads, Tq, Tk, scale, s);
-    default:  return hipErrorInvalidValue;
-  }
-}
+  return launch_any_d<false>(Q, ldq, K, ldk, Vt, ldvt, O, ldo, N, heads, D, Tq, Tk, scale, AttnPreNorm{}, s);
+}
+
+int attention_prenorm_max_tokens() { return ATTN_PN_MAX_T; }
+
+hipError_t launch_attention_prenorm(const uint16_t* Q, int ldq, const uint16_t* K, int ldk, const uint16_t* Vt, int ldvt,
+                                    uint16_t* O, int ldo, int N, int heads, int D, int T, float scale, const float2* stats,
+                                    int slots, int C, float eps, const float* e_q, const float* e_v, hipStream_t s) {
+  if (!stats || !e_q || !e_v || slots < 1 || C < 1 || T < 4 || T % 4 != 0 || T > ATTN_PN_MAX_T || D % 8 != 0 || (heads * D) % 4 != 0)
+    return hipErrorInvalidValue;
+  const AttnPreNorm pn{stats, slots, 1.0f / (float)C, eps, e_q, e_v};
+  return launch_any_d<true>(Q, ldq, K, ldk, Vt, ldvt, O, ldo, N, heads, D, T, T, scale, pn, s);
+}
diff --git a/diff_foley_amd/csrc/elementwise.hip b/diff_foley_amd/csrc/elementwise.hip
--- a/diff_foley_amd/csrc/elementwise.hip
+++ b/diff_foley_amd/csrc/elementwise.hip
@@ -957,6 +957,77 @@
 }
 
 namespace {
+__global__ __launch_bounds__(256) void proj_fold_colmean_kernel(const float* __restrict__ Wp, const float* __restrict__ bp,
+                                                                float* __restrict__ cm, int C) {
+  const int j = blockIdx.x * 4 + (threadIdx.x >> 6), lane = threadIdx.x & 63;
+  if (j > C) return;
+  double a = 0.0;
+  for (int c = lane; c < C; c += 64) a += (double)(j < C ? Wp[(long)c * C + j] : bp[c]);
+#pragma unroll
+  for (int o = 32; o > 0; o >>= 1) a += __shfl_xor(a, o);
+  if (lane == 0) cm[j] = (float)(a / (double)C);
+}
+__global__ __launch_bounds__(256) void pack_proj_fold_kernel(const float* __restrict__ W , const float* __restrict__ gamma,
+                                                             const float* __restrict__ Wp , const float* __restrict__ cm,
+                                                             bf16_t* __restrict__ out , int C) {
+  __shared__ float sa[32][33], sb[32][33];
+  const int tx = threadIdx.x & 31, ty = threadIdx.x >> 5;
+  const int i0 = blockIdx.y * 32, j0 = blockIdx.x * 32;
+  const float mj = cm[j0 + tx];
+  double acc[4] = {0.0, 0.0, 0.0, 0.0};
+  for (int k0 = 0; k0 < C; k0 += 32) {
+#pragma unroll
+    for (int r = 0; r < 4; ++r) {
+      sa[ty + 8 * r][tx] = W[(long)(i0 + ty + 8 * r) * C + k0 + tx] * gamma[k0 + tx];
+      sb[ty + 8 * r][tx] = Wp[(long)(k0 + ty + 8 * r) * C + j0 + tx] - mj;
+    }
+    __syncthreads();
+#pragma unroll
+    for (int kk = 0; kk < 32; ++kk) {
+      const double b = (double)sb[kk][tx];
+#pragma unroll
+      for (int r = 0; r < 4; ++r) acc[r] += (double)sa[ty + 8 * r][kk] * b;
+    }
+    __syncthreads();
+  }
+#pragma unroll
+  for (int r = 0; r < 4; ++r) out[(long)(i0 + ty + 8 * r) * C + j0 + tx] = f2bf((float)acc[r]);
+}
+__global__ __launch_bounds__(256) void proj_fold_bias_kernel(const float* __restrict__ W, const float* __restrict__ gamma,
+                                                             const float* __restrict__ beta, const float* __restrict__ bp,
+                                                             const float* __restrict__ cm, float* __restrict__ d,
+                                                             float* __restrict__ e, int R, int C) {
+  const int i = blockIdx.x * 4 + (threadIdx.x >> 6), lane = threadIdx.x & 63;
+  if (i >= R) return;
+  const float mb = cm[C];
+  double ad = 0.0, ae = 0.0;
+  for (int k = lane; k < C; k += 64) {
+    const float w = W[(long)i * C + k];
+    ad += (double)(w * gamma[k]) * (double)(bp[k] - mb);
+    ae += (double)w * (double)beta[k];
+  }
+#pragma unroll
+  for (int o = 32; o > 0; o >>= 1) {
+    ad += __shfl_xor(ad, o);
+    ae += __shfl_xor(ae, o);
+  }
+  if (lane == 0) {
+    d[i] = (float)ad;
+    e[i] = (float)ae;
+  }
+}
+}
+
+hipError_t launch_pack_proj_fold(const float* W, const float* gamma, const float* beta, const float* Wp, const float* bp, float* cm,
+                                 int fill_cm, uint16_t* wout, float* d, float* e, int R, int C, hipStream_t s) {
+  if (C % 32 != 0 || R % 32 != 0) return hipErrorInvalidValue;
+  if (fill_cm) hipLaunchKernelGGL(proj_fold_colmean_kernel, dim3((C + 1 + 3) / 4), dim3(256), 0, s, Wp, bp, cm, C);
+  hipLaunchKernelGGL(pack_proj_fold_kernel, dim3(C / 32, R / 32), dim3(256), 0, s, W, gamma, Wp, cm, wout, C);
+  hipLaunchKernelGGL(proj_fold_bias_kernel, dim3((R + 3) / 4), dim3(256), 0, s, W, gamma, beta, bp, cm, d, e, R, C);
+  return hipGetLastError();
+}
+
+namespace {
 __global__ __launch_bounds__(256) void xattn_expand_kernel(const bf16_t* __restrict__ kv, bf16_t* __restrict__ Kexp,
                                                            bf16_t* __restrict__ Vexp, int Tc, int Tcp, int C, int H, long total8) {
   const int D = C / H, c8n = C / 8;
diff --git a/diff_foley_amd/csrc/engine_builder.hip b/diff_foley_amd/csrc/engine_builder.hip
--- a/diff_foley_amd/csrc/engine_builder.hip
+++ b/diff_foley_amd/csrc/engine_builder.hip
@@ -291,7 +291,10 @@
     g.ln_stats = st; g.ln_slots = slots; g.ln_C = C; g.ln_eps = 1e-5f; g.ln_cs = cs;
     g.bias = bb;
   };
-  {
+  const bool fuse_v = (T % 4 == 0);
+  const bool no_fold = getenv("DF_NO_PROJ_FOLD") && atoi(getenv("DF_NO_PROJ_FOLD"));
+  const bool fold = fuse_v && !no_fold && C % 64 == 0 && T <= attention_prenorm_max_tokens();
+  if (!fold) {
     GemmParams g = gp_linear(a, Mp, C, c->w_linear(nm(p + ".proj_in.weight")), C);
     produces_t0(g);
     g.bias = c->f32(nm(p + ".proj_in.bias"));
@@ -300,8 +303,8 @@
   bf16_t* qk = buf<bf16_t>((size_t)M * 2 * C);
   const int ldvt = rup(T, 32);
   bf16_t* vt = buf<bf16_t>((size_t)NB * C * ldvt);
-  const bool fuse_v = (T % 4 == 0);
   bf16_t* o_own = nullptr;
+  const float* pn_e = nullptr;
   if (!fuse_v) {
     layernorm(t0v, tb + ".norm1", a);
     {
@@ -318,6 +321,18 @@
       gemm(g, NB, "st.vT");
     }
     o_own = buf<bf16_t>((size_t)M * C);
+  } else if (fold) {
+    const bf16_t* w;
+    const float* bb;
+    c->w_proj_fold(nm(tb + ".attn1.pqkv"), nm(p + ".proj_in"), nm(tb + ".norm1"),
+                   {nm(tb + ".attn1.to_q.weight"), nm(tb + ".attn1.to_k.weight"), nm(tb + ".attn1.to_v.weight")}, &w, &bb, &pn_e);
+    GemmParams g = gp_linear(a, Mp, C, w, 4 * C);
+    out_b16(g, qk, 2 * C);
+    g.bias = bb;
+    g.t0 = t0; g.t0_ld = C; g.t0_cols = C;
+    g.stats = st; g.stats_slots = slots;
+    g.vt = vt; g.vt_col0 = 3 * C; g.vt_T = T; g.ldvt = ldvt;
+    gemm(g, 1, "st.qkv");
   } else {
     const bf16_t* w;
     const float *cs, *bb;
@@ -332,6 +347,9 @@
   }
   bf16_t* o = o_own ? o_own : a;
   other("attn.self", [=](hipStream_t s, const RunArgs&) {
+    if (pn_e)
+      return launch_attention_prenorm(qk, 2 * C, qk + C, 2 * C, vt, ldvt, o, C, NBp, heads, D, T, scale, st, slots, C, 1e-5f, pn_e,
+                                      pn_e + 2 * C, s);
     return launch_attention(qk, 2 * C, qk + C, 2 * C, vt, ldvt, o, C, NBp, heads, D, T, T, scale, s);
   });
   emits(o, Mp, C, C);
diff --git a/diff_foley_amd/csrc/engine_internal.h b/diff_foley_amd/csrc/engine_internal.h
--- a/diff_foley_amd/csrc/engine_internal.h
+++ b/diff_foley_amd/csrc/engine_internal.h
@@ -256,6 +256,8 @@
                   const std::vector<std::string>& biases, bool geglu, const bf16_t** w, const float** cs, const float** bb);
   void w_ln_w320(const std::string& key, int rows, int K, const bf16_t** w, const float** cs, const float** bb);
   void w_geglu(const std::string& prefix, const bf16_t** w, const float** b);
+  void w_proj_fold(const std::string& key, const std::string& pin, const std::string& norm, const std::vector<std::string>& names,
+                   const bf16_t** w, const float** bias, const float** e);
 };
 
 DFE_NAMESPACE {
diff --git a/diff_foley_amd/csrc/engine_pack.hip b/diff_foley_amd/csrc/engine_pack.hip
--- a/diff_foley_amd/csrc/engine_pack.hip
+++ b/diff_foley_amd/csrc/engine_pack.hip
@@ -195,3 +195,36 @@
   *w = (const bf16_t*)blk[0];
   *b = (const float*)blk[1];
 }
+
+void df_ctx::w_proj_fold(const std::string& key, const std::string& pin, const std::string& norm, const std::vector<std::string>& names,
+                         const bf16_t** w, const float** bias, const float** e) {
+  const auto blk = pack_once<4>({key + "#pfw", key + "#pfb", key + "#pfe", key + "#pfcm"}, [&]() -> std::array<void*, 4> {
+    const RawT& tp = rt(pin + ".weight");
+    const int C = (int)tp.shape[0];
+    if ((int)tp.shape[1] != C) fail("w_proj_fold %s: proj_in is not square", key.c_str());
+    int rows = 0;
+    for (auto& n : names) {
+      if ((int)rt(n).shape[1] != C) fail("w_proj_fold %s: input dims differ", key.c_str());
+      rows += (int)rt(n).shape[0];
+    }
+    bf16_t* wo = (bf16_t*)pmalloc((size_t)(C + rows) * C * 2);
+    float* bo = (float*)pmalloc((size_t)(C + rows) * 4);
+    float* eo = (float*)pmalloc((size_t)rows * 4);
+    float* cm = (float*)pmalloc((size_t)(C + 1) * 4);
+    const float* wp = f32(pin + ".weight");
+    const float* bp = f32(pin + ".bias");
+    HIPCHK(launch_cast_bf16(wp, wo, (long)C * C, pack_stream));
+    HIPCHK(hipMemcpyAsync(bo, bp, (size_t)C * 4, hipMemcpyDeviceToDevice, pack_stream));
+    int off = 0;
+    for (auto& n : names) {
+      const int r = (int)rt(n).shape[0];
+      HIPCHK(launch_pack_proj_fold(f32(n), f32(norm + ".weight"), f32(norm + ".bias"), wp, bp, cm, off == 0, wo + (size_t)(C + off) * C,
+                                   bo + C + off, eo + off, r, C, pack_stream));
+      off += r;
+    }
+    return {wo, bo, eo, cm};
+  });
+  *w = (const bf16_t*)blk[0];
+  *bias = (const float*)blk[1];
+  *e = (const float*)blk[2];
+}
diff --git a/diff_foley_amd/csrc/engine_run.hip b/diff_foley_amd/csrc/engine_run.hip
--- a/diff_foley_amd/csrc/engine_run.hip
+++ b/diff_foley_amd/csrc/engine_run.hip
@@ -61,7 +61,7 @@
   if (o.is_gemm) {
     const GemmParams& g = o.gp;
     const long rows = (long)g.M * (g.taps == 4 ? 4 : 1) + g.dup_rows;
-    const int cols = g.geglu ? g.N / 2 : (g.vt ? g.vt_col0 : g.N);
+    const int cols = g.geglu ? g.N / 2 : (g.vt ? g.vt_col0 - g.t0_cols : g.N);
     if (g.out_bf16 && g.C && !o.c_ext && !g.store_nchw)
       for (int z = 0; z < (g.splitk > 1 ? 1 : o.batch); ++z) outs.push_back({(const uint16_t*)g.C + (long)z * g.c_bs, rows, cols, g.ldc});
     if (g.aux) outs.push_back({g.aux, rows, g.N, g.ld_aux});
diff --git a/diff_foley_amd/csrc/engine_test_api.hip b/diff_foley_amd/csrc/engine_test_api.hip
--- a/diff_foley_amd/csrc/engine_test_api.hip
+++ b/diff_foley_amd/csrc/engine_test_api.hip
@@ -96,6 +96,7 @@
   }
   g.geglu = d->geglu ? 1 : 0;
   g.vt = (bf16_t*)d->vt; g.vt_col0 = d->vt_col0; g.vt_T = d->vt_T; g.ldvt = d->ldvt;
+  g.t0 = d->t0; g.t0_ld = d->t0_ld; g.t0_cols = d->t0_cols;
   g.C = d->C; g.ldc = d->ldc > 0 ? d->ldc : (g.geglu ? g.N / 2 : g.N); g.out_bf16 = d->out_operand ? 1 : 0;
   g.a_bs = d->a_bs; g.c_bs = d->c_bs; g.res_bs = d->res_bs;
   if (d->conv != 2) g.w_bs = d->w_bs;
@@ -495,6 +496,20 @@
                       int ldo, int N, int heads, int D, int Tq, int Tk, float scale, void* stream) {
   return guard([&] { HIPCHK(launch_attention(Q, ldq, K, ldk, Vt, ldvt, O, ldo, N, heads, D, Tq, Tk, scale, (hipStream_t)stream)); });
 }
+int df_test_attention_prenorm(const uint16_t* Q, int ldq, const uint16_t* K, int ldk, const uint16_t* Vt, int ldvt, uint16_t* O,
+                              int ldo, int N, int heads, int D, int T, float scale, const void* stats, int slots, int C, float eps,
+                              const float* e_q, const float* e_v, void* stream) {
+  return guard([&] {
+    const hipError_t e = launch_attention_prenorm(Q, ldq, K, ldk, Vt, ldvt, O, ldo, N, heads, D, T, scale, (const float2*)stats, slots,
+                                                  C, eps, e_q, e_v, (hipStream_t)stream);
+    if (e == hipErrorInvalidValue) fail("launch_attention_prenorm refused D %d / T %d / %d slots", D, T, slots);
+    HIPCHK(e);
+  });
+}
+int df_test_pack_proj_fold(const float* W, const float* gamma, const float* beta, const float* Wp, const float* bp, float* cm,
+                           uint16_t* wout, float* d, float* e, int R, int C, void* stream) {
+  return guard([&] { HIPCHK(launch_pack_proj_fold(W, gamma, beta, Wp, bp, cm, 1, wout, d, e, R, C, (hipStream_t)stream)); });
+}
 
 int df_test_groupnorm_bwd(const float* x, int ld, int N, int HW, int C, const float* gamma, const float* beta, float eps, int silu,
                           const float* dy, int lddy, const float* addend, int ldadd, float* dx, int lddx, uint16_t* dx_b16,
diff --git a/diff_foley_amd/csrc/engine_tune.hip b/diff_foley_amd/csrc/engine_tune.hip
--- a/diff_foley_amd/csrc/engine_tune.hip
+++ b/diff_foley_amd/csrc/engine_tune.hip
@@ -9,8 +9,8 @@
 
 std::string tune_key(const GemmParams& g, int batch, bool defer) {
   char key[160];
-  const int epi = (g.silu ? 128 : 0) | (g.ln_stats ? 1 : 0) | (g.stats ? 2 : 0) | (g.vt ? 4 : 0) | (g.aux ? 8 : 0) | (g.res ? 16 : 0) | (g.Cin2 ? 32 : 0) |
-                  (defer ? 64 : 0) | (g.dup_rows ? 256 : 0);
+  const int epi = (g.silu ? 128 : 0) | ((g.ln_stats || g.t0_cols) ? 1 : 0) | ((g.stats && !g.t0_cols) ? 2 : 0) | (g.vt ? 4 : 0) |
+                  (g.aux ? 8 : 0) | (g.res ? 16 : 0) | (g.Cin2 ? 32 : 0) | (defer ? 64 : 0) | (g.dup_rows ? 256 : 0);
   snprintf(key, sizeof key, "%d_%d_%d_%d_%d_%d_%d_%d_e%d", g.M, g.N, g.K, g.taps, g.stride, g.ups, batch, g.geglu, epi);
   return key;
 }
diff --git a/diff_foley_amd/csrc/gemm.h b/diff_foley_amd/csrc/gemm.h
--- a/diff_foley_amd/csrc/gemm.h
+++ b/diff_foley_amd/csrc/gemm.h
@@ -34,6 +34,7 @@
   int sm_w, sm_valid;
   float2* stats; int stats_slots;
   uint16_t* vt; int vt_col0; int vt_T; int ldvt;
+  float* t0; int t0_ld; int t0_cols;
   int dup_rows;
   int no_c_store;
   int store_nchw; int hw_out;
diff --git a/diff_foley_amd/csrc/gemm.hip b/diff_foley_amd/csrc/gemm.hip
--- a/diff_foley_amd/csrc/gemm.hip
+++ b/diff_foley_amd/csrc/gemm.hip
@@ -141,10 +141,16 @@
   const int nk = p.K / 64;
   if (p.taps == 4) {
     if (!gemm_tile_has_mode(tile, 3) || batch > 1) return false;
-    if (p.geglu || p.vt || p.ln_stats || p.stats || p.w_rows > 0 || p.sm_w > 0 || p.Cin2 > 0 || p.res || p.store_nchw) return false;
+    if (p.geglu || p.vt || p.t0_cols > 0 || p.ln_stats || p.stats || p.w_rows > 0 || p.sm_w > 0 || p.Cin2 > 0 || p.res || p.store_nchw) return false;
     if (splitk > 1 && (p.N & 3) != 0) return false;
     return splitk == 1 || nk / splitk >= 2;
   }
+  if (p.t0_cols > 0 && (p.taps != 1 || !p.t0 || !p.stats || !p.vt || p.ln_stats || p.geglu || p.sm_w > 0 || p.res || p.rowbias ||
+                        p.aux || p.dup_rows || p.w_rows > 0 || p.Cin2 > 0 || !p.out_bf16 || batch > 1 || splitk > 1 ||
+                        (p.t0_cols & 63) != 0 || (p.t0_ld & 3) != 0 || p.t0_cols >= p.vt_col0 || p.stats_slots * 64 < p.t0_cols ||
+                        gemm_tile_family(tile) == DF_FAM_HALO || gemm_tile_family(tile) < 0 ||
+                        p.t0_cols % kGemmTiles[tile].bn != 0))
+    return false;
   if (gemm_tile_is_pgeglu(tile)) return pgeglu_valid(p, tile, batch, splitk);
   if (gemm_tile_is_wgeglu(tile)) return wgeglu_valid(p, tile, batch, splitk);
   if (!gemm_tile_has_mode(tile, gemm_mode(p))) return false;
@@ -219,7 +225,8 @@
   else epi = EPI_LEAN;
   if ((epi == EPI_GEGLU || epi == EPI_LNC || epi == EPI_PROD) && (p.taps != 1 || p.alpha != 1.f || p.relu || p.silu || !vec))
     return hipErrorInvalidValue;
-  if (epi == EPI_LNC && (!p.ln_stats || p.aux)) return hipErrorInvalidValue;
+  if (epi == EPI_LNC && ((!p.ln_stats && p.t0_cols <= 0) || p.aux)) return hipErrorInvalidValue;
+  if (p.t0_cols > 0 && !gemm_tile_valid(p, tile_cfg, batch, p.splitk)) return hipErrorInvalidValue;
   if (epi == EPI_XS && (!p.ln_stats || p.taps != 1 || !vec || (p.N & 63) != 0)) return hipErrorInvalidValue;
   hipError_t e;
   const int mode = gemm_mode(p), part = (tile_cfg >= 0 && tile_cfg < TILE_ALL) ? kGemmTiles[tile_cfg].part : 0;
diff --git a/diff_foley_amd/csrc/gemm_impl.h b/diff_foley_amd/csrc/gemm_impl.h
--- a/diff_foley_amd/csrc/gemm_impl.h
+++ b/diff_foley_amd/csrc/gemm_impl.h
@@ -191,7 +191,7 @@
     reinterpret_cast<unsigned long long*>(p.partial)[(long)blockIdx.x * 32 + 24 + (K)] = __builtin_amdgcn_s_memtime();
   DF_EPI_STAMP(0)
   __builtin_amdgcn_s_barrier();
-  if ((EPI == EPI_LNC || EPI == EPI_GEGLU || EPI == EPI_XS) && p.ln_stats && tid < BM) sRow[tid] = ln_mr;
+  if ((EPI == EPI_LNC || EPI == EPI_GEGLU || EPI == EPI_XS) && (p.ln_stats || EPI == EPI_LNC) && tid < BM) sRow[tid] = ln_mr;
   if constexpr (PARK) {
 #pragma unroll
     for (int i = 0; i < TM; ++i)
@@ -289,6 +289,27 @@
   constexpr int CPR = BN / 4;
   const int rps_sh = (has_rb && p.rows_per_sample > 0 && (p.rows_per_sample & (p.rows_per_sample - 1)) == 0)
                          ? (31 - __builtin_clz(p.rows_per_sample)) : -1;
+  if (EPI == EPI_LNC && p.t0_cols > 0 && n0 < p.t0_cols) {
+    constexpr int ITERS = BM * CPR / NT, RSTEP = NT / CPR;
+    const int rb0 = tid / CPR, c4 = (tid - rb0 * CPR) * 4, col = n0 + c4;
+    const bool colok = col < p.t0_cols;
+#pragma unroll
+    for (int ei = 0; ei < ITERS; ++ei) {
+      const int r = rb0 + ei * RSTEP;
+      const int row = rowmap(r);
+      float4 v = *reinterpret_cast<const float4*>(&sC[r * LDC + c4]);
+      if (has_bias) { v.x += hb0.x; v.y += hb0.y; v.z += hb0.z; v.w += hb0.w; }
+      const bool ok = colok && row < p.M;
+      const float s1 = row16_sum(ok ? (v.x + v.y) + (v.z + v.w) : 0.f);
+      const float s2 = row16_sum(ok ? (v.x * v.x + v.y * v.y) + (v.z * v.z + v.w * v.w) : 0.f);
+      if (ok) {
+        if ((tid & 15) == 0) st_wt(&p.stats[(long)row * p.stats_slots + (col >> 6)], make_float2(s1, s2));
+        st_wt(reinterpret_cast<float4*>(p.t0 + (long)row * p.t0_ld + col), v);
+      }
+    }
+    return;
+  }
+  const int c_col0 = (EPI == EPI_LNC) ? p.t0_cols : 0;
   if (EPI == EPI_LNC && p.vt && n0 >= p.vt_col0) {
     constexpr int RG = BM / 4, CG = BN / 4;
     const int cv = p.N - p.vt_col0;
@@ -374,7 +395,7 @@
       }                                                                                                             \
     }                                                                                                               \
     if (ok) {                                                                                                       \
-      const long idx = (long)batch * p.c_bs + (long)row * p.ldc + col;                                              \
+      const long idx = (long)batch * p.c_bs + (long)row * p.ldc + (col - c_col0);                                   \
       if (((FL) & 4) && p.no_c_store) {  \
       } else if (p.out_bf16)                                                                                        \
         st_wt(reinterpret_cast<uint2*>(reinterpret_cast<bf16_t*>(p.C) + idx), make_uint2(pack_bf2(v.x, v.y), pack_bf2(v.z, v.w))); \
diff --git a/diff_foley_amd/csrc/kernels.h b/diff_foley_amd/csrc/kernels.h
--- a/diff_foley_amd/csrc/kernels.h
+++ b/diff_foley_amd/csrc/kernels.h
@@ -26,6 +26,10 @@
 hipError_t launch_attention(const uint16_t* Q, int ldq, const uint16_t* K, int ldk, const uint16_t* Vt, int ldvt,
                             uint16_t* O, int ldo, int N, int heads, int D, int Tq, int Tk, float scale,
                             hipStream_t s);
+hipError_t launch_attention_prenorm(const uint16_t* Q, int ldq, const uint16_t* K, int ldk, const uint16_t* Vt, int ldvt,
+                                    uint16_t* O, int ldo, int N, int heads, int D, int T, float scale, const float2* stats,
+                                    int slots, int C, float eps, const float* e_q, const float* e_v, hipStream_t s);
+int attention_prenorm_max_tokens();
 bool attention_supported(int D);
 int attention_form(int D, int Tq, int Tk);
 
@@ -64,6 +68,8 @@
                               int C, int F, hipStream_t s);
 hipError_t launch_pack_geglu(const float* w, const float* b, uint16_t* wout, float* bout, int half_rows, int K,
                              hipStream_t s);
+hipError_t launch_pack_proj_fold(const float* W, const float* gamma, const float* beta, const float* Wp, const float* bp, float* cm,
+                                 int fill_cm, uint16_t* wout, float* d, float* e, int R, int C, hipStream_t s);
 
 hipError_t launch_bcast_rows(const float* src, float* dst, int rows, int n, hipStream_t s);
 hipError_t launch_pack_latent_bcast(const float* x, uint16_t* out, int B, int C, int HW, int cpad, int rep, const float* src,
diff --git a/diff_foley_amd/engine.py b/diff_foley_amd/engine.py
--- a/diff_foley_amd/engine.py
+++ b/diff_foley_amd/engine.py
@@ -29,7 +29,8 @@
         ("sm_valid", C.c_int), ("dup_rows", C.c_int), ("no_c_store", C.c_int), ("store_nchw", C.c_int), ("hw_out", C.c_int),
         ("cfg_out", C.c_void_p), ("cfg_scale", C.c_float), ("defer_reduce", C.c_int), ("slabs_out", C.c_void_p),
         ("ups", C.c_int), ("zstuff", C.c_int), ("A2", C.c_void_p), ("lda2", C.c_int), ("Cin2", C.c_int), ("geglu", C.c_int),
-        ("vt", C.c_void_p), ("vt_col0", C.c_int), ("vt_T", C.c_int), ("ldvt", C.c_int)]
+        ("vt", C.c_void_p), ("vt_col0", C.c_int), ("vt_T", C.c_int), ("ldvt", C.c_int),
+        ("t0", C.c_void_p), ("t0_ld", C.c_int), ("t0_cols", C.c_int)]
 
     def __init__(self, **kw):
         kw.setdefault("alpha", 1.0)
@@ -179,6 +180,10 @@
     "df_test_gemm_tile_info": [C.c_int, C.POINTER(GemmTile)],
     "df_test_xattn_chain": [C.c_void_p] * 10 + [C.c_int] * 6 + [C.c_void_p] * 10 + [C.c_int, C.c_int, C.c_void_p],
     "df_test_pack_ffproj": [C.c_void_p] * 6 + [C.c_int, C.c_int, C.c_void_p],
+    "df_test_attention_prenorm": [C.c_void_p, C.c_int, C.c_void_p, C.c_int, C.c_void_p, C.c_int, C.c_void_p, C.c_int, C.c_int, C.c_int,
+                                  C.c_int, C.c_int, C.c_float, C.c_void_p, C.c_int, C.c_int, C.c_float, C.c_void_p, C.c_void_p,
+                                  C.c_void_p],
+    "df_test_pack_proj_fold": [C.c_void_p] * 9 + [C.c_int, C.c_int, C.c_void_p],
     "df_test_softmax_rows": [C.c_void_p, C.c_void_p, C.c_int, C.c_int, C.c_int, C.c_void_p],
     "df_test_timestep_embedding": [C.c_void_p, C.c_void_p, C.c_int, C.c_int, C.c_void_p],
     "df_test_timestep_embedding_b16": [C.c_void_p, C.c_int, C.c_void_p, C.c_int, C.c_int, C.c_void_p],
diff --git a/include/df_engine.h b/include/df_engine.h
--- a/include/df_engine.h
+++ b/include/df_engine.h
@@ -226,6 +226,7 @@
   const void* A2; int lda2, Cin2;
   int geglu;
   void* vt; int vt_col0, vt_T, ldvt;
+  float* t0; int t0_ld, t0_cols;
 } df_test_gemm_desc;
 int df_test_gemm_ex(const df_test_gemm_desc* d, void* stream);
 int df_test_gemm_valid(const df_test_gemm_desc* d, int tile, int batch, int splitk);
@@ -241,6 +242,11 @@
                         const void* xstats_dev, int NB, int T, int Tc, int Dc, int C, int heads, uint16_t* kv_dev, uint16_t* Kexp_dev,
                         uint16_t* Vexp_dev, uint16_t* WqT_dev, uint16_t* G_dev, float* cs_dev, float* bb_dev, uint16_t* Vo_dev,
                         uint16_t* P_dev, float* out_dev, int tile_xs, int tile_xo, void* stream);
+int df_test_attention_prenorm(const uint16_t* Q_dev, int ldq, const uint16_t* K_dev, int ldk, const uint16_t* Vt_dev, int ldvt,
+                              uint16_t* O_dev, int ldo, int N, int heads, int D, int T, float scale, const void* stats_dev, int slots,
+                              int C, float eps, const float* e_q_dev, const float* e_v_dev, void* stream);
+int df_test_pack_proj_fold(const float* W_dev, const float* gamma_dev, const float* beta_dev, const float* Wp_dev, const float* bp_dev,
+                           float* cm_dev, uint16_t* wout_dev, float* d_dev, float* e_dev, int R, int C, void* stream);
 int df_test_pack_ffproj(const float* Wp_dev, const float* bp_dev, const float* W2_dev, const float* b2_dev, uint16_t* wout_dev,
                         float* bout_dev, int C, int F, void* stream);
 int df_test_peak(int kind, const void* src_dev, void* dst_dev, size_t n, int blocks, void* stream);
```
